# adwardlee/multitask-end-to-end-video-captioning

Measured on AMD Instinct MI355X. Metric: sampled caption tokens/sec (REINFORCE step), higher is better.
Workload: dtype f32

## Files before the change

include/s2vt.h:

```cpp
#ifndef S2VT_H
#define S2VT_H

#include <stddef.h>
#include <stdint.h>

#ifdef __cplusplus
extern "C" {
#endif

#define S2VT_OK 0
#define S2VT_E_BADARG (-1)
#define S2VT_E_ALIGN (-2)
#define S2VT_E_WORKSPACE (-3)
#define S2VT_E_HIP (-4)
#define S2VT_E_CHAIN_TIMEOUT (-5)

typedef void* s2vt_stream;

typedef struct s2vt_dims {
    int32_t dim_image;
    int32_t n_words;
    int32_t word_dim;
    int32_t lstm_dim;
    int32_t n_video_lstm_step;
// ... 138 lines not shown
size_t s2vt_train_workspace_bytes(const s2vt_dims* d, int32_t B, int32_t N);
int s2vt_teacher_forced_fwd(const s2vt_dims* d, const s2vt_params* p, const float* video, int32_t B, int32_t N,
                            const int32_t* caption, float keep, uint64_t seed, const int32_t* video_id,
                            const int32_t* sample_id, float* logits_out, void* workspace, size_t workspace_bytes,
                            s2vt_stream stream);

size_t s2vt_scheduled_scratch_bytes(const s2vt_dims* d, int32_t N);
int s2vt_scheduled_fwd(const s2vt_dims* d, const s2vt_params* p, const float* video, int32_t B, int32_t N, const int32_t* caption, float p_gt,
                       uint64_t coin_seed, float loss_weight, float keep, uint64_t seed, const int32_t* video_id, const int32_t* sample_id,
                       float* logits_out, int32_t* generated, int32_t* fed, float* mask, float* coef_tm, int32_t* target_tm, float* mask_sum,
                       float* mask_sum_copy, void* workspace, size_t workspace_bytes, void* scratch, size_t scratch_bytes, s2vt_stream stream);

int s2vt_teacher_forced_fwd_reuse(const s2vt_dims* d, const s2vt_params* p, const float* video, int32_t B, int32_t N,
                                  const int32_t* caption, float keep, uint64_t seed, const int32_t* video_id,
                                  const int32_t* sample_id, float* logits_out, void* workspace, size_t workspace_bytes,
                                  const void* sampler_workspace, size_t sampler_workspace_bytes, int32_t sampler_rows,
                                  s2vt_stream stream);

int s2vt_teacher_forced_fwd_steps(const s2vt_dims* d, const s2vt_params* p, const float* video, int32_t B, int32_t N,
                                  const int32_t* caption, int32_t caption_steps, float keep, uint64_t seed,
                                  const int32_t* video_id, const int32_t* sample_id, float* logits_out, void* workspace,
                                  size_t workspace_bytes, const void* sampler_workspace, size_t sampler_workspace_bytes,
                                  int32_t sampler_rows, s2vt_stream stream);

int s2vt_teacher_forced_fwd_live(const s2vt_dims* d, const s2vt_params* p, const float* video, int32_t B, int32_t N,
                                 const int32_t* caption, int32_t caption_steps, const int32_t* live_rows, int32_t n_live, float keep,
                                 uint64_t seed, const int32_t* video_id, const int32_t* sample_id, float* logits_out,
                                 void* workspace, size_t workspace_bytes, const void* sampler_workspace,
                                 size_t sampler_workspace_bytes, int32_t sampler_rows, s2vt_stream stream);

int s2vt_softmax_nll_fwd_bwd(float* logits, int32_t ld, int32_t R, int32_t V, const int32_t* target, const float* coef,
                             float smoothing, float* nll, float* lp_target, s2vt_stream stream);
int s2vt_softmax_nll_fwd_bwd_rows(float* logits, int32_t ld, int32_t R, int32_t V, const int32_t* target, const float* coef,
                                  const float* smoothing_rows, float* nll, float* lp_target, s2vt_stream stream);

int s2vt_bptt_bwd(const s2vt_dims* d, const s2vt_params* p, const s2vt_params* grads, const float* video, int32_t B,
                  int32_t N, const float* dlogits, float keep, uint64_t seed, const int32_t* video_id,
                  const int32_t* sample_id, void* workspace, size_t workspace_bytes, s2vt_stream stream);

int s2vt_bptt_bwd_phase(const s2vt_dims* d, const s2vt_params* p, const s2vt_params* grads, const float* video, int32_t B,
                        int32_t N, const float* dlogits, float keep, uint64_t seed, const int32_t* video_id,
                        const int32_t* sample_id, void* workspace, size_t workspace_bytes, int32_t phase, s2vt_stream stream);

int s2vt_bptt_bwd_steps(const s2vt_dims* d, const s2vt_params* p, const s2vt_params* grads, const float* video, int32_t B,
                        int32_t N, const float* dlogits, int32_t caption_steps, float keep, uint64_t seed,
                        const int32_t* video_id, const int32_t* sample_id, void* workspace, size_t workspace_bytes, int32_t phase,
                        s2vt_stream stream);

int s2vt_bptt_bwd_live(const s2vt_dims* d, const s2vt_params* p, const s2vt_params* grads, const float* video, int32_t B,
                       int32_t N, const float* dlogits, int32_t caption_steps, const int32_t* live_rows, int32_t n_live, float keep,
                       uint64_t seed, const int32_t* video_id, const int32_t* sample_id, void* workspace, size_t workspace_bytes,
                       int32_t phase, s2vt_stream stream);

size_t s2vt_bf16_grad_workspace_bytes(const s2vt_dims* d, int32_t B, int32_t N);
int s2vt_bptt_bwd_bf16(const s2vt_dims* d, const s2vt_params* p, const s2vt_params* grads, const float* video, int32_t B,
                       int32_t N, const float* dlogits, int32_t caption_steps, const int32_t* live_rows, int32_t n_live, float keep,
                       uint64_t seed, const int32_t* video_id, const int32_t* sample_id, void* workspace, size_t workspace_bytes,
                       int32_t phase, void* bf16_ws, size_t bf16_ws_bytes, s2vt_stream stream);

int s2vt_cast_bf16(const float* src, int32_t ld, const int32_t* rowidx, int32_t R, int32_t C, int32_t transpose, uint16_t* dst, int32_t ldd,
                   int32_t Rp, float* colsum, uint16_t* row_dst, int32_t row_ldd, void* scratch, size_t scratch_bytes, s2vt_stream stream);
int s2vt_gemm_bf16_nt(const uint16_t* A, int32_t lda, const uint16_t* B, int32_t ldb, float* C, int32_t ldc, int32_t M, int32_t N,
                      int32_t Kp, int32_t accumulate, int32_t mfma, s2vt_stream stream);

size_t s2vt_split_grad_workspace_bytes(const s2vt_dims* d, int32_t B, int32_t N);
int s2vt_bptt_bwd_split(const s2vt_dims* d, const s2vt_params* p, const s2vt_params* grads, const float* video, int32_t B,
                        int32_t N, const float* dlogits, int32_t caption_steps, const int32_t* live_rows, int32_t n_live, float keep,
                        uint64_t seed, const int32_t* video_id, const int32_t* sample_id, void* workspace, size_t workspace_bytes,
                        int32_t phase, void* split_ws, size_t split_ws_bytes, s2vt_stream stream);
int s2vt_cast_bf16_split(const float* src, int32_t ld, const int32_t* rowidx, int32_t R, int32_t C, int32_t transpose, uint16_t* dst,
                         uint16_t* dst_lo, int32_t ldd, int32_t Rp, float* colsum, uint16_t* row_dst, uint16_t* row_dst_lo, int32_t row_ldd,
                         void* scratch, size_t scratch_bytes, s2vt_stream stream);
int s2vt_gemm_bf16x3_nt(const uint16_t* Ah, const uint16_t* Al, int32_t lda, const uint16_t* Bh, const uint16_t* Bl, int32_t ldb, float* C,
                        int32_t ldc, int32_t M, int32_t N, int32_t Kp, int32_t accumulate, void* scratch, size_t scratch_bytes, s2vt_stream stream);

int s2vt_gemm_bf16x3_tn(const uint16_t* Ah, const uint16_t* Al, int32_t lda, const uint16_t* Bh, const uint16_t* Bl, int32_t ldb, float* C,
                        int32_t ldc, int32_t M, int32_t N, int32_t K, int32_t accumulate, float* bias, void* scratch, size_t scratch_bytes,
                        s2vt_stream stream);
int s2vt_split_grad_active(int32_t N);
int s2vt_split_grad_dlogits_planes(const s2vt_dims* d, int32_t B, int32_t N, size_t* hi_offset, size_t* lo_offset, int32_t* ld);
int s2vt_softmax_nll_fwd_bwd_split(float* logits, int32_t ld, int32_t R, int32_t V, const int32_t* target, const float* coef, float smoothing,
                                   const float* smoothing_rows, float* nll, float* lp_target, const s2vt_dims* d, int32_t B, int32_t N,
                                   void* split_ws, size_t split_ws_bytes, s2vt_stream stream);

int s2vt_bptt_dvideo(const s2vt_dims* d, const s2vt_params* p, int32_t B, int32_t N, float* d_video, void* workspace,
                      size_t workspace_bytes, s2vt_stream stream);

int s2vt_embed_scatter_add(const float* dE, int32_t ld, const int32_t* idx, int32_t R, int32_t E, float* dWemb,
                           s2vt_stream stream);

int s2vt_caption_mask(const int32_t* ids, int32_t N, int32_t Tc, float* mask, int32_t* target_tm, float* mask_sum, float* mask_sum_copy, s2vt_stream stream);
int s2vt_pg_coef(const float* mask, const float* rewards, const float* baseline, float scale, int32_t N, int32_t Tc, float* coef_tm,
                 s2vt_stream stream);
int s2vt_step_scalars(const float* coef, const float* nll, int64_t R, const float* mask_sum_local, const float* mask_sum_global, float* loss,
                      float* gscale, float* sumsq, s2vt_stream stream);

int s2vt_xe_prep(const float* mask, const int32_t* caption, int32_t N, int32_t Tc, float loss_weight, float n_global, int32_t q1, float* coef_tm,
                 int32_t* target_tm, float* mask_sum, s2vt_stream stream);
int s2vt_mixed_prep(const float* mask, const float* gt_mask, const float* rewards, const float* baseline, const int32_t* sampled,
                    const int32_t* gt_caption, int32_t Ns, int32_t B, int32_t Tc, double lambda_loss, float loss_weight, int32_t q1,
                    float smoothing, float n_global_b, float* coef_tm, float* smooth_tm, int32_t* caption_all, int32_t* target_tm, float* sums, s2vt_stream stream);
int s2vt_mixed_loss(const float* coef, const float* nll, const int32_t* live_rows, int64_t R, int32_t N, int32_t Ns, float* out3, s2vt_stream stream);

int s2vt_grad_finalize(float* g, const float* theta, int64_t n, const float* gscale, float weight_decay, float* sumsq,
                       s2vt_stream stream);
int s2vt_adam_tf(float* theta, const float* g, float* m, float* v, int64_t n, const float* sumsq, float clip_norm,
                 float lr, int64_t step, float beta1, float beta2, float eps, s2vt_stream stream);
int s2vt_adam_tf_guarded(float* theta, const float* g, float* m, float* v, int64_t n, const float* sumsq, float clip_norm,
                         float lr, int64_t step, float beta1, float beta2, float eps, int32_t* applied_step, s2vt_stream stream);

int s2vt_sgd_guarded(float* theta, const float* g, int64_t n, const float* sumsq, float clip_norm, float lr, int64_t step, int32_t* applied_step,
                     s2vt_stream stream);

int s2vt_attention_fwd(const float* hWa, const float* P, const float* Vt, const float* w, float* scores, float* alpha,
                       float* ctx, int32_t Tv, int32_t B, int32_t H, s2vt_stream stream);
int s2vt_attention_bwd(const float* hWa, const float* P, const float* Vt, const float* w, const float* alpha,
                       const float* dctx, float* de_scratch, float* dhWa, float* dP, float* dVt, float* dw, int32_t Tv,
                       int32_t B, int32_t H, s2vt_stream stream);

int s2vt_attention_fwd_rows(const float* hWa, const float* P, const float* Vt, const float* w, float* scores, float* alpha, float* ctx,
                            int32_t* row_video_scratch, int32_t Tv, int32_t n_video, int32_t samples, int32_t H, s2vt_stream stream);
int s2vt_attention_bwd_rows(const float* hWa, const float* P, const float* Vt, const float* w, const float* alpha, const float* dctx,
                            float* de_scratch, float* dhWa, float* dP, float* dVt, float* dw, int32_t Tv, int32_t n_video,
                            int32_t samples, int32_t H, int32_t acc, s2vt_stream stream);

typedef struct s2vt_attn_params {
    float* Wemb;
    float* encode_image_W;
    float* encode_image_b;
    float* embed_att_w;
    float* embed_att_Wa;
    float* embed_att_Ua;
    float* embed_att_ba;
    float* embed_word_W;
    float* embed_word_b;
    float* embed_nn_Wp;
    float* embed_nn_bp;
    float* lstm3_W;
    float* lstm3_b;
} s2vt_attn_params;

size_t s2vt_attn_workspace_bytes(const s2vt_dims* d, int32_t B);
int s2vt_attn_teacher_forced_fwd(const s2vt_dims* d, const s2vt_attn_params* p, const float* video, int32_t B, const int32_t* caption,
                                 int32_t caption_steps, float keep, uint64_t seed, const int32_t* video_id, const int32_t* sample_id,
                                 float* logits, float* alphas_out, void* workspace, size_t workspace_bytes, s2vt_stream stream);
int s2vt_attn_loss_inputs(const int32_t* caption, const float* mask, int32_t B, int32_t Tc, float beta, int32_t* target_tm, float* coef_tm,
                          float* reg_tm, float* mask_sum, s2vt_stream stream);
int s2vt_attn_step_scalars(const float* coef, const float* nll, int64_t R, const float* reg_coef, float reg_m, const float* mask_sum_local,
                           const float* mask_sum_global, float* loss, float* gscale, float* sumsq, const s2vt_dims* d, int32_t B,
                           void* workspace, size_t workspace_bytes, s2vt_stream stream);
int s2vt_attn_bptt_bwd(const s2vt_dims* d, const s2vt_attn_params* p, const s2vt_attn_params* grads, const float* video, int32_t B,
                       const float* dlogits, int32_t caption_steps, const float* reg_coef, float reg_m, float keep, uint64_t seed,
                       const int32_t* video_id, const int32_t* sample_id, void* workspace, size_t workspace_bytes, s2vt_stream stream);
int s2vt_attn_decode_greedy(const s2vt_dims* d, const s2vt_attn_params* p, const float* video, int32_t B, int32_t video_base, int32_t* ids_out,
                            float* alphas_out, void* workspace, size_t workspace_bytes, s2vt_stream stream);

size_t s2vt_attn_sample_workspace_bytes(const s2vt_dims* d, int32_t B, int32_t K, int32_t with_greedy);
int s2vt_attn_sample(const s2vt_dims* d, const s2vt_attn_params* p, const float* video, int32_t B, int32_t K, int32_t with_greedy, uint64_t seed,
                     int32_t video_base, int32_t* ids_out, int32_t* greedy_out, void* workspace, size_t workspace_bytes, s2vt_stream stream);
int s2vt_attn_sample_ex(const s2vt_dims* d, const s2vt_attn_params* p, const float* video, int32_t B, int32_t K, int32_t with_greedy, uint64_t seed,
                        int32_t video_base, int32_t flags, int32_t* ids_out, int32_t* greedy_out, void* workspace, size_t workspace_bytes,
                        s2vt_stream stream);
size_t s2vt_attn_rows_workspace_bytes(const s2vt_dims* d, int32_t n_video, int32_t samples);
int s2vt_attn_teacher_forced_fwd_rows(const s2vt_dims* d, const s2vt_attn_params* p, const float* video, int32_t n_video, int32_t samples,
                                      const int32_t* caption, int32_t caption_steps, float keep, uint64_t seed, const int32_t* video_id,
                                      const int32_t* sample_id, float* logits, float* alphas_out, void* workspace, size_t workspace_bytes,
// ... 141 lines not shown
```

multitask-end-to-end-video-captioning_amd/_lib.py:

```python
from __future__ import annotations

import ctypes as C
import os

_HERE = os.path.dirname(os.path.abspath(__file__))
_LIB = None


class S2VTLibraryError(RuntimeError):
    pass


class S2VTChainTimeout(S2VTLibraryError):
    """A persistent recurrence (csrc/chain.hip) was starved of CUs and gave up a grid-wide wait (S2VT_E_CHAIN_TIMEOUT):
    activations computed since are suspect, variable updates queued behind it were skipped on the device.  Recover with
    Video_Caption_Generator.recover() (synchronise, acknowledge, fall back to per-step launches) and repeat the step."""


MODEL_RESIDUAL = 1


class Dims(C.Structure):
    _fields_ = [(n, C.c_int32) for n in ("dim_image", "n_words", "word_dim", "lstm_dim", "n_video_lstm_step",
                                         "n_caption_lstm_step", "label_dim", "reserved")]
# ... 30 lines not shown

class Operand(C.Structure):
    _fields_ = [("ptr", C.c_void_p), ("rowidx", C.c_void_p), ("ld", C.c_int32), ("k", C.c_int32), ("rowmod", C.c_int32),
                ("reserved", C.c_int32)]


class LstmDir(C.Structure):
    _fields_ = [("W", C.c_void_p), ("kw0", C.c_int32), ("b", C.c_void_p), ("cinit", C.c_void_p), ("cinit_tstride", C.c_int64),
                ("ldcinit", C.c_int32), ("cinit_t0", C.c_int32), ("cinit_steps", C.c_int32), ("C_hist", C.c_void_p),
                ("H_hist", C.c_void_p), ("gates", C.c_void_p)]


BIDIR_PARAM_FIELDS = ("Wemb", "encode_image_W", "encode_image_b", "lstm1_fw_W", "lstm1_fw_b", "lstm1_bw_W", "lstm1_bw_b", "lstm2_W", "lstm2_b",
                      "embed_word_W", "embed_word_b")


class BidirParams(C.Structure):
    _fields_ = [(n, C.c_void_p) for n in BIDIR_PARAM_FIELDS]


def lib_path() -> str:
    return os.environ.get("S2VT_LIB") or os.path.join(_HERE, "libs2vt_hip.so")


_vp, _i32, _i64, _u32, _u64, _f32, _sz = C.c_void_p, C.c_int32, C.c_int64, C.c_uint32, C.c_uint64, C.c_float, C.c_size_t
_DP, _PP, _OP = C.POINTER(Dims), C.POINTER(Params), C.POINTER(Operand)
_AP = C.POINTER(AttnParams)
_LD = C.POINTER(LstmDir)
_BP = C.POINTER(BidirParams)

SIGNATURES = {
    "s2vt_version": (C.c_int, []),
    "s2vt_build_flags": (C.c_int, []),
    "s2vt_last_hip_error": (C.c_int, []),
    "s2vt_zero_regions": (C.c_int, [C.POINTER(C.c_void_p), C.POINTER(C.c_size_t), _i32, _vp]),
    "s2vt_error_string": (C.c_char_p, [C.c_int]),
    "s2vt_prof_enable": (C.c_int, [C.c_int]),
    "s2vt_prof_filter": (C.c_int, [C.c_int, C.c_int]),
    "s2vt_prof_collect": (C.c_int, [C.POINTER(ProfRow), C.c_int]),
    "s2vt_math_eval": (C.c_int, [C.c_int, _vp, _vp, _i64, _vp]),
    "s2vt_gumbel_eval": (C.c_int, [_u64, _i32, _i32, _i32, _vp, _i32, _vp]),
    "s2vt_gemm": (C.c_int, [_OP, _i32, _vp, _i32, _vp, _vp, _i32, _vp, _i32, _i32, _i32, _i32, _i32, _vp]),
    "s2vt_gemm_nt": (C.c_int, [_OP, _i32, _vp, _i32, _vp, _vp, _i32, _vp, _i32, _i32, _i32, _i32, _i32, _vp]),
    "s2vt_lstm_cell_fwd": (C.c_int, [_OP, _OP, _vp, _vp, _i32, _vp, _vp, _vp, _vp, _vp, _vp, _i32, _i32, _f32, _u64, _vp,
                                     _vp, _u32, _i32, _vp]),
    "s2vt_lstm_cell_fwd_res": (C.c_int, [_OP, _OP, _vp, _vp, _i32, _vp, _vp, _OP, _vp, _vp, _vp, _vp, _i32, _i32, _f32, _u64, _vp,
                                         _vp, _u32, _i32, _vp]),
    "s2vt_vocab_pick": (C.c_int, [_vp, _i32, _vp, _vp, _i32, _i32, _i32, _vp, _vp, _i32, _u64, _vp, _vp, _vp, _i32, _vp]),
    "s2vt_tile_count": (C.c_int, [C.c_int]),
    "s2vt_tile_info": (C.c_int, [C.c_int, C.c_int, C.POINTER(TileDesc)]),
    "s2vt_gemm_live": (C.c_int, [_OP, _i32, _vp, _i32, _vp, _vp, _i32, _vp, _i32, _i32, _i32, _i32, _vp, _vp, _i32, _vp]),
    "s2vt_lstm_cell_fwd_live": (C.c_int, [_OP, _OP, _vp, _vp, _i32, _vp, _vp, _OP, _vp, _vp, _vp, _vp, _i32, _i32, _f32, _u64, _vp,
                                          _vp, _u32, _vp, _vp, _i32, _vp]),
    "s2vt_lstm_cell_fwd_gather": (C.c_int, [_OP, _OP, _vp, _vp, _vp, _vp, _i32, _vp, _vp, _vp, _vp, _vp, _vp, _i32, _i32, _i32, _vp]),
    "s2vt_vocab_pick_live": (C.c_int, [_vp, _i32, _vp, _vp, _i32, _i32, _i32, _vp, _vp, _i32, _u64, _vp, _i32, _vp, _vp, _vp, _i32, _vp]),
    "s2vt_frame_embed_fwd": (C.c_int, [_DP, _PP, _vp, _i32, _vp, _vp]),
    "s2vt_sample_workspace_bytes": (_sz, [_DP, _i32, _i32, _i32]),
    "s2vt_sample": (C.c_int, [_DP, _PP, _vp, _i32, _i32, _i32, _u64, _i32, _vp, _vp, _sz, _vp]),
    "s2vt_sample_ex": (C.c_int, [_DP, _PP, _vp, _i32, _i32, _i32, _u64, _i32, _i32, _vp, _vp, _sz, _vp]),
    "s2vt_sample_screen_workspace_bytes": (_sz, [_DP, _i32, _i32, _i32]),
    "s2vt_sample_screened": (C.c_int, [_DP, _PP, _vp, _i32, _i32, _i32, _u64, _i32, _vp, _vp, _sz, _vp, _sz, _vp]),
    "s2vt_sample_mix_workspace_bytes": (_sz, [_DP, _i32, _i32]),
    "s2vt_sample_mix": (C.c_int, [_DP, _PP, _vp, _i32, _vp, _f32, _i32, _u64, _i32, _vp, _vp, _sz, _vp]),
    "s2vt_vocab_topk": (C.c_int, [_vp, _i32, _i32, _i32, _i32, _vp, _vp, _vp]),
    "s2vt_beam_workspace_bytes": (_sz, [_DP, _i32, _i32]),
    "s2vt_beam_encode": (C.c_int, [_DP, _PP, _vp, _i32, _i32, _vp, _sz, _vp]),
    "s2vt_beam_step": (C.c_int, [_DP, _PP, _i32, _i32, _i32, _i32, _vp, _vp, _vp, _i32, _vp, _vp, _vp, _vp, _sz, _vp]),
    "s2vt_train_workspace_bytes": (_sz, [_DP, _i32, _i32]),
    "s2vt_teacher_forced_fwd": (C.c_int, [_DP, _PP, _vp, _i32, _i32, _vp, _f32, _u64, _vp, _vp, _vp, _vp, _sz, _vp]),
    "s2vt_teacher_forced_fwd_reuse": (C.c_int, [_DP, _PP, _vp, _i32, _i32, _vp, _f32, _u64, _vp, _vp, _vp, _vp, _sz, _vp, _sz, _i32, _vp]),
    "s2vt_gemm_nt_splitk": (C.c_int, [_vp, _i32, _vp, _i32, _vp, _i32, _i32, _i32, _i32, _i32, _i32, _vp, _sz, _vp]),
    "s2vt_teacher_forced_fwd_steps": (C.c_int, [_DP, _PP, _vp, _i32, _i32, _vp, _i32, _f32, _u64, _vp, _vp, _vp, _vp, _sz, _vp, _sz, _i32, _vp]),
    "s2vt_teacher_forced_fwd_live": (C.c_int, [_DP, _PP, _vp, _i32, _i32, _vp, _i32, _vp, _i32, _f32, _u64, _vp, _vp, _vp, _vp, _sz, _vp, _sz, _i32, _vp]),
    "s2vt_bptt_bwd_live": (C.c_int, [_DP, _PP, _PP, _vp, _i32, _i32, _vp, _i32, _vp, _i32, _f32, _u64, _vp, _vp, _vp, _sz, _i32, _vp]),
    "s2vt_bf16_grad_workspace_bytes": (_sz, [_DP, _i32, _i32]),
    "s2vt_bptt_bwd_bf16": (C.c_int, [_DP, _PP, _PP, _vp, _i32, _i32, _vp, _i32, _vp, _i32, _f32, _u64, _vp, _vp, _vp, _sz, _i32, _vp, _sz, _vp]),
    "s2vt_cast_bf16": (C.c_int, [_vp, _i32, _vp, _i32, _i32, _i32, _vp, _i32, _i32, _vp, _vp, _i32, _vp, _sz, _vp]),
    "s2vt_gemm_bf16_nt": (C.c_int, [_vp, _i32, _vp, _i32, _vp, _i32, _i32, _i32, _i32, _i32, _i32, _vp]),
    "s2vt_split_grad_workspace_bytes": (_sz, [_DP, _i32, _i32]),
    "s2vt_bptt_bwd_split": (C.c_int, [_DP, _PP, _PP, _vp, _i32, _i32, _vp, _i32, _vp, _i32, _f32, _u64, _vp, _vp, _vp, _sz, _i32, _vp, _sz, _vp]),
    "s2vt_cast_bf16_split": (C.c_int, [_vp, _i32, _vp, _i32, _i32, _i32, _vp, _vp, _i32, _i32, _vp, _vp, _vp, _i32, _vp, _sz, _vp]),
    "s2vt_gemm_bf16x3_nt": (C.c_int, [_vp, _vp, _i32, _vp, _vp, _i32, _vp, _i32, _i32, _i32, _i32, _i32, _vp, _sz, _vp]),
    "s2vt_gemm_bf16x3_tn": (C.c_int, [_vp, _vp, _i32, _vp, _vp, _i32, _vp, _i32, _i32, _i32, _i32, _i32, _vp, _vp, _sz, _vp]),
    "s2vt_split_grad_active": (C.c_int, [_i32]),
    "s2vt_train_workspace_dz2": (C.c_int, [_DP, _i32, _i32, C.POINTER(_sz), C.POINTER(_sz)]),
    "s2vt_split_grad_dlogits_planes": (C.c_int, [_DP, _i32, _i32, C.POINTER(_sz), C.POINTER(_sz), C.POINTER(_i32)]),
    "s2vt_softmax_nll_fwd_bwd_split": (C.c_int, [_vp, _i32, _i32, _i32, _vp, _vp, _f32, _vp, _vp, _vp, _DP, _i32, _i32, _vp, _sz, _vp]),
    "s2vt_bptt_bwd_steps": (C.c_int, [_DP, _PP, _PP, _vp, _i32, _i32, _vp, _i32, _f32, _u64, _vp, _vp, _vp, _sz, _i32, _vp]),
    "s2vt_softmax_nll_fwd_bwd": (C.c_int, [_vp, _i32, _i32, _i32, _vp, _vp, _f32, _vp, _vp, _vp]),
    "s2vt_softmax_unshifted_argmax": (C.c_int, [_vp, _i32, _i32, _i32, _vp, _vp, _vp]),
    "s2vt_softmax_nll_fwd_bwd_rows": (C.c_int, [_vp, _i32, _i32, _i32, _vp, _vp, _vp, _vp, _vp, _vp]),
    "s2vt_bptt_bwd": (C.c_int, [_DP, _PP, _PP, _vp, _i32, _i32, _vp, _f32, _u64, _vp, _vp, _vp, _sz, _vp]),
    "s2vt_bptt_bwd_phase": (C.c_int, [_DP, _PP, _PP, _vp, _i32, _i32, _vp, _f32, _u64, _vp, _vp, _vp, _sz, _i32, _vp]),
    "s2vt_bptt_dvideo": (C.c_int, [_DP, _PP, _i32, _i32, _vp, _vp, _sz, _vp]),
    "s2vt_embed_scatter_add": (C.c_int, [_vp, _i32, _vp, _i32, _i32, _vp, _vp]),
    "s2vt_caption_mask": (C.c_int, [_vp, _i32, _i32, _vp, _vp, _vp, _vp, _vp]),
    "s2vt_pg_coef": (C.c_int, [_vp, _vp, _vp, _f32, _i32, _i32, _vp, _vp]),
    "s2vt_xe_prep": (C.c_int, [_vp, _vp, _i32, _i32, _f32, _f32, _i32, _vp, _vp, _vp, _vp]),
    "s2vt_mixed_prep": (C.c_int, [_vp, _vp, _vp, _vp, _vp, _vp, _i32, _i32, _i32, C.c_double, _f32, _i32, _f32, _f32, _vp, _vp, _vp, _vp, _vp, _vp]),
    "s2vt_mixed_loss": (C.c_int, [_vp, _vp, _vp, _i64, _i32, _i32, _vp, _vp]),
    "s2vt_step_scalars": (C.c_int, [_vp, _vp, _i64, _vp, _vp, _vp, _vp, _vp, _vp]),
    "s2vt_grad_finalize": (C.c_int, [_vp, _vp, _i64, _vp, _f32, _vp, _vp]),
    "s2vt_adam_tf": (C.c_int, [_vp, _vp, _vp, _vp, _i64, _vp, _f32, _f32, _i64, _f32, _f32, _f32, _vp]),
    "s2vt_attention_fwd": (C.c_int, [_vp, _vp, _vp, _vp, _vp, _vp, _vp, _i32, _i32, _i32, _vp]),
    "s2vt_attention_bwd": (C.c_int, [_vp, _vp, _vp, _vp, _vp, _vp, _vp, _vp, _vp, _vp, _vp, _i32, _i32, _i32, _vp]),
    "s2vt_attention_fwd_rows": (C.c_int, [_vp, _vp, _vp, _vp, _vp, _vp, _vp, _vp, _i32, _i32, _i32, _i32, _vp]),
    "s2vt_attention_bwd_rows": (C.c_int, [_vp, _vp, _vp, _vp, _vp, _vp, _vp, _vp, _vp, _vp, _vp, _i32, _i32, _i32, _i32, _i32, _vp]),
    "s2vt_attn_sample_workspace_bytes": (_sz, [_DP, _i32, _i32, _i32]),
    "s2vt_attn_sample": (C.c_int, [_DP, _AP, _vp, _i32, _i32, _i32, _u64, _i32, _vp, _vp, _vp, _sz, _vp]),
    "s2vt_attn_sample_ex": (C.c_int, [_DP, _AP, _vp, _i32, _i32, _i32, _u64, _i32, _i32, _vp, _vp, _vp, _sz, _vp]),
    "s2vt_attn_rows_workspace_bytes": (_sz, [_DP, _i32, _i32]),
    "s2vt_attn_teacher_forced_fwd_rows": (C.c_int, [_DP, _AP, _vp, _i32, _i32, _vp, _i32, _f32, _u64, _vp, _vp, _vp, _vp, _vp, _sz, _vp]),
    "s2vt_attn_step_scalars_rows": (C.c_int, [_vp, _vp, _i64, _vp, _f32, _vp, _vp, _vp, _vp, _vp, _DP, _i32, _i32, _vp, _sz, _vp]),
    "s2vt_attn_bptt_bwd_rows": (C.c_int, [_DP, _AP, _AP, _vp, _i32, _i32, _vp, _i32, _vp, _f32, _f32, _u64, _vp, _vp, _vp, _sz, _vp]),
    "s2vt_attn_workspace_bytes": (_sz, [_DP, _i32]),
    "s2vt_attn_teacher_forced_fwd": (C.c_int, [_DP, _AP, _vp, _i32, _vp, _i32, _f32, _u64, _vp, _vp, _vp, _vp, _vp, _sz, _vp]),
    "s2vt_attn_loss_inputs": (C.c_int, [_vp, _vp, _i32, _i32, _f32, _vp, _vp, _vp, _vp, _vp]),
    "s2vt_attn_step_scalars": (C.c_int, [_vp, _vp, _i64, _vp, _f32, _vp, _vp, _vp, _vp, _vp, _DP, _i32, _vp, _sz, _vp]),
    "s2vt_attn_bptt_bwd": (C.c_int, [_DP, _AP, _AP, _vp, _i32, _vp, _i32, _vp, _f32, _f32, _u64, _vp, _vp, _vp, _sz, _vp]),
    "s2vt_attn_decode_greedy": (C.c_int, [_DP, _AP, _vp, _i32, _i32, _vp, _vp, _vp, _sz, _vp]),
    "s2vt_attn_beam_workspace_bytes": (_sz, [_DP, _i32, _i32]),
    "s2vt_attn_beam_encode": (C.c_int, [_DP, _AP, _vp, _i32, _i32, _vp, _sz, _vp]),
    "s2vt_attn_beam_step": (C.c_int, [_DP, _AP, _i32, _i32, _i32, _i32, _vp, _vp, _vp, _i32, _vp, _vp, _vp, _vp, _vp, _sz, _vp]),
    "s2vt_attr_head_fwd": (C.c_int, [_vp, _i32, _i32, _i32, _vp, _vp, _i32, _vp, _vp, _vp, _vp, _vp]),
    "s2vt_attr_head_bwd": (C.c_int, [_vp, _vp, _vp, _i32, _i32, _i32, _f32, _vp, _vp, _vp, _vp]),
    "s2vt_attr_head_scores": (C.c_int, [_vp, _i32, _i32, _i32, _vp, _vp, _i32, _vp, _vp, _vp, _vp]),
    "s2vt_create": (C.c_int, [_DP, _i32, _i32, C.POINTER(_vp)]),
    "s2vt_destroy": (C.c_int, [_vp]),
    "s2vt_encode_fwd": (C.c_int, [_vp, _PP, _vp, _i32, _vp]),
    "s2vt_decode_greedy": (C.c_int, [_vp, _PP, _vp, _vp]),
    "s2vt_decode_multinomial": (C.c_int, [_vp, _PP, _i32, _u64, _i32, _vp, _vp]),
    "s2vt_pack_weights": (C.c_int, [_vp, _i32, _i32, _vp, _vp, _vp]),
    "s2vt_unpack_weights": (C.c_int, [_vp, _vp, _i32, _i32, _vp, _vp]),
    "s2vt_frame_embed_bwd": (C.c_int, [_DP, _vp, _vp, _i32, _vp, _vp, _vp]),
    "s2vt_lstm_cell_bwd": (C.c_int, [_vp, _vp, _vp, _vp, _vp, _vp, _vp, _i32, _i32, _vp]),
    "s2vt_xent_smooth_fwd_bwd": (C.c_int, [_vp, _i32, _i32, _i32, _vp, _vp, _f32, _vp, _vp]),
    "s2vt_pg_nll_fwd_bwd": (C.c_int, [_vp, _i32, _i32, _i32, _i32, _vp, _vp, _vp, _vp, _vp, _vp, _vp]),
    "s2vt_embed_gather": (C.c_int, [_vp, _i32, _vp, _i32, _i32, _vp, _i32, _vp]),
    "s2vt_global_norm_clip": (C.c_int, [_vp, _i64, _f32, _vp, _vp]),
    "s2vt_gemm_tn": (C.c_int, [_vp, _i32, _vp, _vp, _i32, _vp, _i32, _i32, _i32, _i32, _i32, _vp]),
    "s2vt_transpose": (C.c_int, [_vp, _i32, _vp, _i32, _i32, _i32, _vp]),
    "s2vt_colsum": (C.c_int, [_vp, _i32, _i32, _i32, _vp, _vp]),
    "s2vt_tanh_bwd": (C.c_int, [_vp, _vp, _vp, _i64, _vp]),
    "s2vt_dropout_bwd": (C.c_int, [_vp, _i32, _vp, _i32, _i32, _f32, _u64, _u32, _vp, _vp, _vp]),
    "s2vt_lstm_recurrence_scratch_bytes": (_sz, [_i32]),
    "s2vt_lstm_recurrence_fwd": (C.c_int, [_vp, _i32, _vp, _vp, _i64, _i32, _i32, _vp, _vp, _vp, _vp, _i32, _i32, _i32, _f32, _u64, _vp, _vp,
                                           _u32, _i32, _vp, _sz, _vp]),
    "s2vt_lstm_birecurrence_scratch_bytes": (_sz, [_i32]),
    "s2vt_lstm_birecurrence_fwd": (C.c_int, [_LD, _LD, _i32, _i32, _i32, _i32, _vp, _sz, _vp]),
    "s2vt_bidir_workspace_bytes": (_sz, [_DP, _i32]),
    "s2vt_bidir_teacher_forced_fwd": (C.c_int, [_DP, _BP, _vp, _i32, _vp, _f32, _u64, _vp, _vp, _i32, _vp, _vp, _sz, _vp]),
    "s2vt_bidir_bptt_bwd": (C.c_int, [_DP, _BP, _BP, _vp, _i32, _vp, _f32, _u64, _vp, _vp, _vp, _sz, _vp]),
    "s2vt_bidir_decode_workspace_bytes": (_sz, [_DP, _i32]),
    "s2vt_bidir_decode_greedy": (C.c_int, [_DP, _BP, _vp, _i32, _i32, _i32, _i32, _vp, _vp, _vp, _sz, _vp]),
    "s2vt_bidir_sample_workspace_bytes": (_sz, [_DP, _i32, _i32, _i32]),
    "s2vt_bidir_sample": (C.c_int, [_DP, _BP, _vp, _i32, _i32, _i32, _u64, _i32, _i32, _vp, _vp, _vp, _sz, _vp]),
    "s2vt_bidir_beam_workspace_bytes": (_sz, [_DP, _i32, _i32]),
    "s2vt_bidir_beam_encode": (C.c_int, [_DP, _BP, _vp, _i32, _i32, _i32, _vp, _sz, _vp]),
    "s2vt_bidir_beam_step": (C.c_int, [_DP, _BP, _i32, _i32, _i32, _i32, _vp, _vp, _vp, _i32, _vp, _vp, _vp, _vp, _sz, _vp]),
    "s2vt_bidir_sample_sum": (C.c_int, [_vp, _vp, _i32, _i32, _i32, _i32, _vp]),
    "s2vt_bidir_rows_workspace_bytes": (_sz, [_DP, _i32, _i32]),
    "s2vt_bidir_teacher_forced_fwd_rows": (C.c_int, [_DP, _BP, _vp, _i32, _i32, _vp, _f32, _u64, _vp, _vp, _i32, _vp, _vp, _sz, _vp]),
    "s2vt_bidir_bptt_bwd_rows": (C.c_int, [_DP, _BP, _BP, _vp, _i32, _i32, _vp, _f32, _u64, _vp, _vp, _vp, _sz, _vp]),
    "s2vt_lstm_recurrence_bwd_scratch_bytes": (_sz, [_i32, _i32]),
    "s2vt_lstm_recurrence_bwd": (C.c_int, [_vp, _i32, _vp, _vp, _vp, _i64, _i32, _i32, _vp, _i32, _i32, _i32, _f32, _u64, _vp, _vp, _u32, _i32,
                                           _vp, _sz, _vp]),
    "s2vt_lstm_recurrence_bwd_split": (C.c_int, [_vp, _i32, _vp, _vp, _vp, _i64, _i32, _i32, _vp, _i32, _i32, _i32, _f32, _u64, _vp, _vp, _u32,
# ... 47 lines not shown
```

multitask-end-to-end-video-captioning_amd/csrc/bwd_bf16.hip:

```cpp
#include <hip/hip_runtime.h>

#include <cstdlib>
#include <type_traits>

#include "internal.h"

namespace s2vt {
namespace {

typedef __bf16 bf16x8 __attribute__((ext_vector_type(8)));
typedef float f32x4 __attribute__((ext_vector_type(4)));
typedef float f32x16 __attribute__((ext_vector_type(16)));

template <bool SPLIT>
__global__ __launch_bounds__(256) void cast_rows_bf16_kernel(const float* __restrict__ src, int ld, const int32_t* __restrict__ rowidx,
                                                             int R, int K, uint16_t* __restrict__ dst, int ldd, int vec,
                                                             uint16_t* __restrict__ dst_lo, int ones)
{
    const int cpr = bf16_pad(K + ones) / 8;
    const long total = (long)R * cpr;
    for (long i = (long)blockIdx.x * 256 + threadIdx.x; i < total; i += (long)gridDim.x * 256) {
        const int r = (int)(i / cpr), k0 = (int)(i % cpr) * 8;
        const float* s = src + (size_t)(rowidx ? rowidx[r] : r) * ld + k0;
        float v[8];
        if (vec && k0 + 8 <= K) {
            const float4 a = *reinterpret_cast<const float4*>(s), b = *reinterpret_cast<const float4*>(s + 4);
            v[0] = a.x; v[1] = a.y; v[2] = a.z; v[3] = a.w; v[4] = b.x; v[5] = b.y; v[6] = b.z; v[7] = b.w;
        } else {
#pragma unroll
            for (int j = 0; j < 8; ++j) v[j] = k0 + j < K ? s[j] : ones && k0 + j == K ? 1.0f : 0.0f;
        }
        uint4 o;
        if constexpr (SPLIT) {
            uint4 l;
            split2(v[0], v[1], o.x, l.x); split2(v[2], v[3], o.y, l.y); split2(v[4], v[5], o.z, l.z); split2(v[6], v[7], o.w, l.w);
            *reinterpret_cast<uint4*>(dst_lo + (size_t)r * ldd + k0) = l;
        } else {
            o.x = pack2(v[0], v[1]); o.y = pack2(v[2], v[3]); o.z = pack2(v[4], v[5]); o.w = pack2(v[6], v[7]);
        }
        *reinterpret_cast<uint4*>(dst + (size_t)r * ldd + k0) = o;
    }
}

constexpr int kTrRows = 256;

template <bool SPLIT>
__global__ __launch_bounds__(256) void cast_tr_bf16_kernel(CastTrArgs a, int vec)
{
    __shared__ float t[64][65];
    __shared__ float cs[4][64];
    const int tid = threadIdx.x, c0 = blockIdx.x * 64;
    const int rbeg = blockIdx.y * kTrRows, rend = min(rbeg + kTrRows, a.Rp);
    float csum = 0.0f;
    for (int r0 = rbeg; r0 < rend; r0 += 64) {
#pragma unroll
        for (int p = 0; p < 4; ++p) {
            const int rr = p * 16 + (tid >> 4), cc = (tid & 15) * 4;
            const int r = r0 + rr, c = c0 + cc;
            float v[4] = {0.0f, 0.0f, 0.0f, 0.0f};
            if (r < a.R) {
                const float* s = a.src + (size_t)(a.rowidx ? a.rowidx[r] : r) * a.ld + c;
                if (vec && c + 4 <= a.C) {
                    const float4 x = *reinterpret_cast<const float4*>(s);
                    v[0] = x.x; v[1] = x.y; v[2] = x.z; v[3] = x.w;
                } else {
#pragma unroll
                    for (int j = 0; j < 4; ++j) v[j] = c + j < a.C ? s[j] : 0.0f;
                }
                if (a.rdst) {
                    uint2 o;
                    if constexpr (SPLIT) {
                        uint2 l;
                        split2(v[0], v[1], o.x, l.x); split2(v[2], v[3], o.y, l.y);
                        *reinterpret_cast<uint2*>(a.rdst_lo + (size_t)r * a.rldd + c) = l;
                    } else {
                        o.x = pack2(v[0], v[1]); o.y = pack2(v[2], v[3]);
                    }
                    *reinterpret_cast<uint2*>(a.rdst + (size_t)r * a.rldd + c) = o;
                }
            }
#pragma unroll
            for (int j = 0; j < 4; ++j) t[rr][cc + j] = v[j];
        }
        __syncthreads();
        for (int i = tid >> 6; i < 64; i += 4) csum += t[i][tid & 63];
#pragma unroll
        for (int p = 0; p < 2; ++p) {
            const int cc = p * 32 + (tid >> 3), rr = (tid & 7) * 8;
            if (c0 + cc < a.C) {
                uint4 o;
                if constexpr (SPLIT) {
                    uint4 l;
                    split2(t[rr][cc], t[rr + 1][cc], o.x, l.x); split2(t[rr + 2][cc], t[rr + 3][cc], o.y, l.y);
                    split2(t[rr + 4][cc], t[rr + 5][cc], o.z, l.z); split2(t[rr + 6][cc], t[rr + 7][cc], o.w, l.w);
                    *reinterpret_cast<uint4*>(a.dst_lo + (size_t)(c0 + cc) * a.ldd + r0 + rr) = l;
                } else {
                    o.x = pack2(t[rr][cc], t[rr + 1][cc]); o.y = pack2(t[rr + 2][cc], t[rr + 3][cc]);
                    o.z = pack2(t[rr + 4][cc], t[rr + 5][cc]); o.w = pack2(t[rr + 6][cc], t[rr + 7][cc]);
                }
                *reinterpret_cast<uint4*>(a.dst + (size_t)(c0 + cc) * a.ldd + r0 + rr) = o;
            }
        }
// ... 57 lines not shown
    constexpr int RM = MF == 16 ? 4 : 2;
    typedef typename std::conditional<MF == 16, f32x4, f32x16>::type acc_t;
    constexpr int NACC = MF == 16 ? 4 : 16;
    acc_t acc[RM][RM];
#pragma unroll
    for (int i = 0; i < RM; ++i)
#pragma unroll
        for (int j = 0; j < RM; ++j)
#pragma unroll
            for (int e = 0; e < NACC; ++e) acc[i][j][e] = 0.0f;

    const int nk = g.Kp / kBK;
    if (nk > 0) { load(0); store(0); }
    __syncthreads();
    for (int kt = 0; kt < nk; ++kt) {
        const int cur = kt & 1;
        if (kt + 1 < nk) load((kt + 1) * kBK);
        const uint16_t* As = lds[cur][0];
        const uint16_t* Bs = lds[cur][1];
        if constexpr (MF == 16) {
#pragma unroll
            for (int kk = 0; kk < 2; ++kk) {
                const int ch = kk * 4 + (lane >> 4);
                bf16x8 af[4], bfr[4];
#pragma unroll
                for (int i = 0; i < 4; ++i) {
                    const int ra_ = wr * 64 + i * 16 + (lane & 15), rb_ = wc * 64 + i * 16 + (lane & 15);
                    af[i] = *reinterpret_cast<const bf16x8*>(As + swz(ra_, ch));
                    bfr[i] = *reinterpret_cast<const bf16x8*>(Bs + swz(rb_, ch));
                }
#pragma unroll
                for (int i = 0; i < 4; ++i)
#pragma unroll
                    for (int j = 0; j < 4; ++j) acc[i][j] = __builtin_amdgcn_mfma_f32_16x16x32_bf16(af[i], bfr[j], acc[i][j], 0, 0, 0);
            }
        } else {
#pragma unroll
            for (int kk = 0; kk < 4; ++kk) {
                const int ch = kk * 2 + (lane >> 5);
                bf16x8 af[2], bfr[2];
#pragma unroll
                for (int i = 0; i < 2; ++i) {
                    const int ra_ = wr * 64 + i * 32 + (lane & 31), rb_ = wc * 64 + i * 32 + (lane & 31);
                    af[i] = *reinterpret_cast<const bf16x8*>(As + swz(ra_, ch));
                    bfr[i] = *reinterpret_cast<const bf16x8*>(Bs + swz(rb_, ch));
                }
#pragma unroll
                for (int i = 0; i < 2; ++i)
#pragma unroll
                    for (int j = 0; j < 2; ++j) acc[i][j] = __builtin_amdgcn_mfma_f32_32x32x16_bf16(af[i], bfr[j], acc[i][j], 0, 0, 0);
            }
        }
        if (kt + 1 < nk) store(cur ^ 1);
        __syncthreads();
    }
#pragma unroll
    for (int i = 0; i < RM; ++i)
#pragma unroll
        for (int j = 0; j < RM; ++j)
#pragma unroll
            for (int e = 0; e < NACC; ++e) {
                int row, col;
                if constexpr (MF == 16) {
                    row = m0 + wr * 64 + i * 16 + (lane >> 4) * 4 + e;
                    col = n0 + wc * 64 + j * 16 + (lane & 15);
                } else {
                    row = m0 + wr * 64 + i * 32 + (e & 3) + 8 * (e >> 2) + 4 * (lane >> 5);
                    col = n0 + wc * 64 + j * 32 + (lane & 31);
                }
                if (row < g.M && col < g.N) {
                    float* c = g.C + (size_t)row * g.ldc + col;
                    *c = g.accumulate ? *c + acc[i][j][e] : acc[i][j][e];
                }
            }
}


struct GemmX3Args {
    const uint16_t *Ah, *Al; int lda; const uint16_t *Bh, *Bl; int ldb; float* C; int ldc;
    int M, N, nk, nk_slab, accumulate, tiles_m, tiles_n;
    float* part;
    int K;
    float* bias; int Mo;
};

constexpr int kX3BK = 32, kX3Slots = 4, kX3Plane = kTile * kX3BK;
constexpr int kX3Lds = kX3Slots * 4 * kX3Plane * 2;
constexpr int kX3Dma = kTile / 16;
typedef __attribute__((address_space(3))) void* x3_lds_ptr;
typedef short i16x4 __attribute__((ext_vector_type(4)));
typedef __attribute__((address_space(3))) i16x4* x3_tr_ptr;

template <bool TN>
__global__ __launch_bounds__(512) void gemm_bf16x3_kernel(GemmX3Args g)
{
    extern __shared__ __attribute__((aligned(16))) uint16_t x3lds[];
    const int nwg = g.tiles_m * g.tiles_n, orig = blockIdx.x;
    const int xcd = orig & 7, q = nwg >> 3, rem = nwg & 7;
    const int wgid = (xcd < rem ? xcd * (q + 1) : rem * (q + 1) + (xcd - rem) * q) + (orig >> 3);
    const int tm = wgid % g.tiles_m, tn = wgid / g.tiles_m;
    const int m0 = tm * kTile, n0 = tn * kTile;
    const int kbeg = blockIdx.y * g.nk_slab, nk = min(g.nk_slab, g.nk - kbeg);
    const int tid = threadIdx.x, lane = tid & 63, w = __builtin_amdgcn_readfirstlane(tid >> 6);

    if (w >= 4) {
        const int p = w - 4;
        const uint16_t* const plane = p == 0 ? g.Ah : p == 1 ? g.Al : p == 2 ? g.Bh : g.Bl;
        const int r0 = p < 2 ? m0 : n0, rows = p < 2 ? g.M : g.N, ld = p < 2 ? g.lda : g.ldb;
        const __amdgpu_buffer_rsrc_t rs = __builtin_amdgcn_make_buffer_rsrc(const_cast<uint16_t*>(plane + (TN ? (size_t)r0 : (size_t)r0 * ld)), 0,
                                                                            TN ? (int)(((uint32_t)g.K * (uint32_t)ld - (uint32_t)r0) * 2u) : (int)kOob, 0x00020000);
        uint32_t voff[kX3Dma];
        if constexpr (TN) {
            const int kr = lane >> 4, s = lane & 15;
#pragma unroll
            for (int b = 0; b < kX3Dma; ++b)
                voff[b] = (uint32_t)((b * 4 + kr) * ld + ((((s >> 1) ^ (kr | ((b & 2) << 1))) << 1) | (s & 1)) * 8) * 2u;
        } else {
            const int rr = lane >> 2, kg = (lane & 3) ^ ((rr >> 2) & 3);
#pragma unroll
            for (int b = 0; b < kX3Dma; ++b) {
                const int r = b * 16 + rr;
                voff[b] = r0 + r < rows ? (uint32_t)(r * ld + kg * 8) * 2u : kOob;
            }
        }
        auto issue = [&](int ks) __attribute__((always_inline)) {
            uint16_t* const dst = x3lds + ((ks % kX3Slots) * 4 + p) * kX3Plane;
            if constexpr (TN) {
                const uint32_t koff = (uint32_t)(kbeg + ks) * kX3BK * (uint32_t)ld * 2u;
#pragma unroll
                for (int b = 0; b < kX3Dma; ++b)
                    __builtin_amdgcn_raw_ptr_buffer_load_lds(rs, (x3_lds_ptr)(dst + b * 4 * kTile), 16, voff[b] + koff, 0, 0, 0);
            } else {
                const uint32_t soff = (uint32_t)(kbeg + ks) * kX3BK * 2u;
#pragma unroll
                for (int b = 0; b < kX3Dma; ++b)
                    __builtin_amdgcn_raw_ptr_buffer_load_lds(rs, (x3_lds_ptr)(dst + b * 16 * kX3BK), 16, voff[b], soff, 0, 0);
            }
        };
        auto wait_younger = [](int n) __attribute__((always_inline)) {
            if (n >= 2) wait_vmcnt<2 * kX3Dma>();
            else if (n == 1) wait_vmcnt<kX3Dma>();
            else wait_vmcnt<0>();
        };
        const int pro = min(kX3Slots, nk);
        for (int ks = 0; ks < pro; ++ks) issue(ks);
        if (pro - 1 >= 3) wait_vmcnt<3 * kX3Dma>();
        else wait_younger(pro - 1);
        asm volatile("" ::: "memory");
        __builtin_amdgcn_s_barrier();
        asm volatile("" ::: "memory");
        for (int k = 0; k < nk; ++k) {
            wait_younger(min(k + 3, nk - 1) - (k + 1));
            asm volatile("" ::: "memory");
            __builtin_amdgcn_s_barrier();
            asm volatile("" ::: "memory");
            if (k + kX3Slots < nk) issue(k + kX3Slots);
        }
        return;
    }

    const int wr = w >> 1, wc = w & 1;
    const int fofs = (lane & 15) * kX3BK + (((lane >> 4) ^ ((lane >> 2) & 3)) << 3);
    const int gq = lane >> 4, tq = (lane >> 2) & 3, tswz = tq | ((gq & 1) << 2);
    const int tofs = (gq * 8 + tq) * kTile + (lane & 3) * 4;
    f32x4 acc[4][4];
#pragma unroll
    for (int i = 0; i < 4; ++i)
#pragma unroll
        for (int j = 0; j < 4; ++j) acc[i][j] = f32x4{0.0f, 0.0f, 0.0f, 0.0f};
    auto read = [&](int ks, bf16x8 (&f)[4][4]) __attribute__((always_inline)) {
        const uint16_t* const s = x3lds + (ks % kX3Slots) * 4 * kX3Plane;
#pragma unroll
        for (int pl = 0; pl < 4; ++pl)
#pragma unroll
            for (int i = 0; i < 4; ++i)
                if constexpr (TN) {
                    const uint16_t* const a = s + pl * kX3Plane + tofs + ((((pl < 2 ? wr : wc) * 4 + i) ^ tswz) << 4);
                    const i16x4 lo4 = __builtin_amdgcn_ds_read_tr16_b64_v4i16((x3_tr_ptr)a);
                    const i16x4 hi4 = __builtin_amdgcn_ds_read_tr16_b64_v4i16((x3_tr_ptr)(a + 4 * kTile));
                    f[pl][i] = __builtin_bit_cast(bf16x8, __builtin_shufflevector(lo4, hi4, 0, 1, 2, 3, 4, 5, 6, 7));
                } else {
                    f[pl][i] = *reinterpret_cast<const bf16x8*>(s + pl * kX3Plane + ((pl < 2 ? wr : wc) * 64 + i * 16) * kX3BK + fofs);
                }
    };
    auto mul = [&](const bf16x8 (&f)[4][4]) __attribute__((always_inline)) {
#pragma unroll
        for (int i = 0; i < 4; ++i)
#pragma unroll
            for (int j = 0; j < 4; ++j) acc[i][j] = __builtin_amdgcn_mfma_f32_16x16x32_bf16(f[0][i], f[3][j], acc[i][j], 0, 0, 0);
#pragma unroll
        for (int i = 0; i < 4; ++i)
#pragma unroll
            for (int j = 0; j < 4; ++j) acc[i][j] = __builtin_amdgcn_mfma_f32_16x16x32_bf16(f[1][i], f[2][j], acc[i][j], 0, 0, 0);
#pragma unroll
        for (int i = 0; i < 4; ++i)
#pragma unroll
            for (int j = 0; j < 4; ++j) acc[i][j] = __builtin_amdgcn_mfma_f32_16x16x32_bf16(f[0][i], f[2][j], acc[i][j], 0, 0, 0);
    };
    bf16x8 fa[4][4], fb[4][4];
    __syncthreads();
    if (nk > 0) read(0, fa);
    auto step = [&](int k, bf16x8 (&cur)[4][4], bf16x8 (&nxt)[4][4]) __attribute__((always_inline)) {
        asm volatile("s_waitcnt lgkmcnt(0)" ::: "memory");
        __syncthreads();
        if (k + 1 < nk) read(k + 1, nxt);
        mul(cur);
    };
    for (int k = 0; k < nk; k += 2) {
        step(k, fa, fb);
        step(k + 1, fb, fa);
    }
    float* const out = g.part ? g.part + (size_t)blockIdx.y * g.Mo * g.N : g.C;
    const int ldo = g.part ? g.N : g.ldc;
    const bool add = !g.part && g.accumulate;
#pragma unroll
    for (int i = 0; i < 4; ++i)
#pragma unroll
        for (int j = 0; j < 4; ++j)
#pragma unroll
            for (int e = 0; e < 4; ++e) {
                const int row = m0 + wr * 64 + i * 16 + (lane >> 4) * 4 + e, col = n0 + wc * 64 + j * 16 + (lane & 15);
                if (row < g.M && col < g.N) {
                    float* c = out + (size_t)row * ldo + col;
                    *c = add ? *c + acc[i][j][e] : acc[i][j][e];
                } else if (TN && row == g.M && g.bias && col < g.N) {
                    if (g.part) out[(size_t)row * ldo + col] = acc[i][j][e];
                    else g.bias[col] += acc[i][j][e];
                }
            }
}

__global__ __launch_bounds__(256) void reduce_slabs_kernel(const float* __restrict__ part, int slabs, int M, int N, float* __restrict__ C, int ldc,
                                                           int accumulate, int Mo, float* __restrict__ bias)
{
    const size_t MN = (size_t)Mo * N;
    for (size_t i = (size_t)blockIdx.x * 256 + threadIdx.x; i < MN; i += (size_t)gridDim.x * 256) {
        float s = part[i];
        for (int k = 1; k < slabs; ++k) s += part[(size_t)k * MN + i];
        const size_t r = i / N;
        if (r < (size_t)M) {
            float* c = C + r * ldc + i % N;
            *c = accumulate ? *c + s : s;
        } else {
            bias[i % N] += s;
        }
    }
}
}

hipError_t launch_cast_rows_bf16(const float* src, int ld, const int32_t* rowidx, int R, int K, uint16_t* dst, int ldd, hipStream_t st,
                                 uint16_t* dst_lo, int ones)
{
    if (R <= 0 || K <= 0) return hipSuccess;
    ones = ones ? 1 : 0;
    const int vec = !((reinterpret_cast<uintptr_t>(src) & 15) || (ld & 3));
    const long chunks = (long)R * (bf16_pad(K + ones) / 8);
    const long blocks = (chunks + 255) / 256;
    const dim3 grid((unsigned)(blocks < 8192 ? blocks : 8192));
    if (dst_lo) hipLaunchKernelGGL(cast_rows_bf16_kernel<true>, grid, dim3(256), 0, st, src, ld, rowidx, R, K, dst, ldd, vec, dst_lo, ones);
    else hipLaunchKernelGGL(cast_rows_bf16_kernel<false>, grid, dim3(256), 0, st, src, ld, rowidx, R, K, dst, ldd, vec, dst_lo, ones);
    return hipGetLastError();
}

size_t cast_tr_part_floats(int Rp, int C)
{
    return (size_t)((Rp + kTrRows - 1) / kTrRows) * (size_t)C;
}

hipError_t launch_cast_tr_bf16(const CastTrArgs& a, hipStream_t st)
{
    if (a.C <= 0 || a.Rp <= 0) return hipSuccess;
    const int vec = !((reinterpret_cast<uintptr_t>(a.src) & 15) || (a.ld & 3));
    const int ny = (a.Rp + kTrRows - 1) / kTrRows;
    if (a.dst_lo) hipLaunchKernelGGL(cast_tr_bf16_kernel<true>, dim3((a.C + 63) / 64, ny), dim3(256), 0, st, a, vec);
    else hipLaunchKernelGGL(cast_tr_bf16_kernel<false>, dim3((a.C + 63) / 64, ny), dim3(256), 0, st, a, vec);
    hipError_t e = hipGetLastError();
    if (e != hipSuccess || !a.colsum) return e;
    hipLaunchKernelGGL(colsum_parts_kernel, dim3((a.C + 255) / 256), dim3(256), 0, st, (const float*)a.part, ny, a.C, a.colsum);
    return hipGetLastError();
}

int gemm_bf16_default_mfma()
{
    static const int v = [] { const char* e = getenv("S2VT_BF16_MFMA"); const int x = e ? atoi(e) : 16; return x == 32 ? 32 : 16; }();
    return v;
}

hipError_t launch_gemm_bf16_nt(const uint16_t* A, int lda, const uint16_t* B, int ldb, float* C, int ldc, int M, int N, int Kp, int accumulate,
                               int mfma, hipStream_t st)
{
    if (M <= 0 || N <= 0) return hipSuccess;
    GemmBf16Args g;
    g.A = A; g.lda = lda; g.B = B; g.ldb = ldb; g.C = C; g.ldc = ldc; g.M = M; g.N = N; g.Kp = Kp; g.accumulate = accumulate;
    g.tiles_m = (M + kTile - 1) / kTile; g.tiles_n = (N + kTile - 1) / kTile;
    const dim3 grid((unsigned)(g.tiles_m * g.tiles_n));
    if ((mfma ? mfma : gemm_bf16_default_mfma()) == 32) hipLaunchKernelGGL(gemm_bf16_nt_kernel<32>, grid, dim3(256), 0, st, g);
    else hipLaunchKernelGGL(gemm_bf16_nt_kernel<16>, grid, dim3(256), 0, st, g);
    return hipGetLastError();
}

int gemm_bf16x3_slabs(int M, int N, int Kp)
{
    const int tiles = ((M + kTile - 1) / kTile) * ((N + kTile - 1) / kTile), nk = Kp / kX3BK;
    static const int cus = [] {
        int dev = 0, n = 256;
        if (hipGetDevice(&dev) == hipSuccess) (void)hipDeviceGetAttribute(&n, hipDeviceAttributeMultiprocessorCount, dev);
        return n > 0 ? n : 256;
    }();
    int s = 1;
    while (s < 8 && tiles * (s * 2) <= cus && nk / (s * 2) >= 16) s *= 2;
    return s;
}

size_t gemm_bf16x3_part_floats(int M, int N, int Kp)
{
    const int s = gemm_bf16x3_slabs(M, N, Kp);
    return s > 1 ? (size_t)s * M * N : 0;
}

namespace {
template <bool TN>
hipError_t launch_x3(const uint16_t* Ah, const uint16_t* Al, int lda, const uint16_t* Bh, const uint16_t* Bl, int ldb, float* C, int ldc, int M, int N,
                     int Kp, int accumulate, float* bias, float* part, size_t part_floats, int cls, hipStream_t st)
{
    if (M <= 0 || N <= 0) return hipSuccess;
    static const hipError_t attr = hipFuncSetAttribute(reinterpret_cast<const void*>(gemm_bf16x3_kernel<TN>), hipFuncAttributeMaxDynamicSharedMemorySize, kX3Lds);
    if (attr != hipSuccess) return attr;
    GemmX3Args g;
    g.Ah = Ah; g.Al = Al; g.lda = lda; g.Bh = Bh; g.Bl = Bl; g.ldb = ldb; g.C = C; g.ldc = ldc; g.M = M; g.N = N;
    g.K = Kp; g.bias = bias; g.Mo = M + (bias ? 1 : 0);
    const int Kr = bf16_pad(Kp);
    g.nk = Kr / kX3BK; g.accumulate = accumulate;
    g.tiles_m = (g.Mo + kTile - 1) / kTile; g.tiles_n = (N + kTile - 1) / kTile;
    int slabs = part ? gemm_bf16x3_slabs(g.Mo, N, Kr) : 1;
    if ((size_t)slabs * g.Mo * N > part_floats) slabs = 1;
    g.nk_slab = ((g.nk + slabs - 1) / slabs + 1) & ~1;
    slabs = g.nk_slab ? (g.nk + g.nk_slab - 1) / g.nk_slab : 1;
    g.part = slabs > 1 ? part : nullptr;
    const dim3 grid((unsigned)(g.tiles_m * g.tiles_n), (unsigned)slabs);
    const bool prof = prof_wants(cls, 16);
    hipEvent_t e0 = nullptr, e1 = nullptr;
    if (prof) {
        hipError_t pe = prof_events(&e0, &e1);
        if (pe != hipSuccess) return pe;
        (void)hipEventRecord(e0, st);
    }
    hipLaunchKernelGGL(gemm_bf16x3_kernel<TN>, grid, dim3(512), kX3Lds, st, g);
    if (slabs > 1) {
        const size_t MN = (size_t)g.Mo * N, blocks = (MN + 255) / 256;
        hipLaunchKernelGGL(reduce_slabs_kernel, dim3((unsigned)(blocks < 4096 ? blocks : 4096)), dim3(256), 0, st, (const float*)part, slabs, M, N, C, ldc,
                           accumulate, g.Mo, bias);
    }
    if (prof) {
        (void)hipEventRecord(e1, st);
        prof_record(cls, 16, cls == 2 ? "x3_128x128(dma) pick screen" : cls == 3 ? "x3_128x128(dma) wgrad" : "x3_128x128(dma) dgrad",
                    2.0 * M * (double)N * Kp, e0, e1);
    }
    return hipGetLastError();
}
}

hipError_t launch_gemm_bf16x3_nt(const uint16_t* Ah, const uint16_t* Al, int lda, const uint16_t* Bh, const uint16_t* Bl, int ldb, float* C, int ldc,
                                 int M, int N, int Kp, int accumulate, float* part, size_t part_floats, int cls, hipStream_t st)
{
    return launch_x3<false>(Ah, Al, lda, Bh, Bl, ldb, C, ldc, M, N, Kp, accumulate, nullptr, part, part_floats, cls, st);
}

bool gemm_bf16x3_tn_ok(int lda, int ldb, int K)
{
    const unsigned long long ld = (unsigned long long)(lda > ldb ? lda : ldb);
    return K >= 0 && lda > 0 && ldb > 0 && ((unsigned long long)bf16_pad(K) + 1) * ld * 2ull + 512ull < (1ull << 31);
}

hipError_t launch_gemm_bf16x3_tn(const uint16_t* Ah, const uint16_t* Al, int lda, const uint16_t* Bh, const uint16_t* Bl, int ldb, float* C, int ldc,
                                 int M, int N, int K, int accumulate, float* bias, float* part, size_t part_floats, int cls, hipStream_t st)
{
    if (!gemm_bf16x3_tn_ok(lda, ldb, K)) return hipErrorInvalidValue;
    return launch_x3<true>(Ah, Al, lda, Bh, Bl, ldb, C, ldc, M, N, K, accumulate, bias, part, part_floats, cls, st);
}

}
```

multitask-end-to-end-video-captioning_amd/csrc/internal.h:

```cpp
#pragma once
#include <hip/hip_runtime.h>
#include <stdint.h>

#include "gemm_mfma.h"

namespace s2vt {

hipError_t launch_gemm(const GemmArgs& a, int epi, int cfg, hipStream_t st);

struct ProfRow { int cls, cfg; long launches; double ms, flops; const char* name; };
void prof_enable(bool on);
bool prof_on();
bool prof_wants(int cls, int cfg);
void prof_filter(int cls, int cfg);
void prof_record(int cls, int cfg, const char* name, double flops, hipEvent_t e0, hipEvent_t e1);
hipError_t prof_events(hipEvent_t* e0, hipEvent_t* e1);
int prof_collect(ProfRow* rows, int max_rows);
int gemm_num_cfgs(int epi);
const char* gemm_cfg_name(int epi, int cfg);
struct GemmCfgInfo { const char* name; int BM, CG, fallback; bool has_scalar, has_live; };
bool gemm_cfg_info(int epi, int cfg, GemmCfgInfo* out);

struct TnArgs {
    const float* A; const int* rowidx; int lda;
// ... 166 lines not shown
    int n_video;
    const int32_t* live;
    const int32_t* n_live;
};
hipError_t launch_attn_fwd(const AttnFwdArgs& a, hipStream_t st);
struct AttnBwdArgs {
    const float* hWa; const float* P; const float* Vt; const float* w; const float* alpha;
    const float* dctx; int ld_dctx;
    const float* slabs; int nslab; size_t slab_stride; int ld_slab;
    int ctx_col0, emb_col0;
    const float* demb_dense; int ld_demb; float* demb_out;
    const float* reg_coef;
    const float* asum; float reg_m;
    float* dhWa;
    float* dP; float* dVt; int acc;
    float* dw;
    int Tv, B, H;
    int vec;
};
hipError_t launch_attn_bwd(const AttnBwdArgs& a, hipStream_t st);
struct AttnBwdRowsArgs {
    AttnBwdArgs a;
    int n_video, samples;
    float* de_rows;
    float* dctx_rows;
};
hipError_t launch_attn_bwd_rows(const AttnBwdRowsArgs& r, hipStream_t st);
hipError_t launch_attn_row_video(int32_t* row_video, int rows, int n_video, hipStream_t st);

hipError_t launch_vocab_topk(const float* logits, int ld, int R, int V, int k, int32_t* ids, float* logp, hipStream_t st);

struct AttnChainLaunch {
    const float* W3; int ldw; const float* b3;
    const float* cinit; size_t cinit_tstride; int ldcinit;
    float* C; float* Hh; float* Out; size_t state_tstride;
    float* gates; size_t gates_tstride;
    const float* Wa; int ldwa; const float* P; const float* Vt; const float* w;
    float* hWa; size_t hwa_tstride;
    float* alpha; float* asum; float* ctx;
    int B, H, T, Tv;
    float keep; uint32_t seed_lo, seed_hi, drop_code0; const int32_t* video_id; const int32_t* sample_id;
    float* img;
    unsigned* sync;
};
constexpr size_t kAttnChainSyncBytes = 3 * kChainSyncBytes;
bool attn_chain_eligible(int B, int H, int Tv);
size_t attn_chain_scratch_floats(int H);
hipError_t launch_attn_chain(const AttnChainLaunch& a, hipStream_t st);

struct AttnBwdChainLaunch {
    const float* W3; int ldw; const float* Wa; int ldwa;
    const float* gates; size_t gates_tstride; const float* C; size_t state_tstride;
    float* dcat; size_t dcat_tstride; int ld_cat;
    float* deh;
    float* dZ; size_t dz_tstride;
    const float* hWa; size_t hwa_tstride; const float* P; const float* Vt; const float* w; const float* alpha;
    const float* reg_coef; const float* asum; float reg_m;
    float* dhWa; size_t dhwa_tstride;
    float* dP; float* dVt; float* dw;
    int B, H, T, Tv;
    float keep; uint32_t seed_lo, seed_hi, drop_code0; const int32_t* video_id; const int32_t* sample_id;
    float* img; float* ex; float* dctxs; unsigned* sync;
};
bool attn_bwd_chain_eligible(int B, int H, int Tv);
void attn_bwd_chain_scratch(int H, size_t* img_floats, size_t* ex_floats, size_t* row_floats, size_t* sync_bytes);
hipError_t launch_attn_bwd_chain(const AttnBwdChainLaunch& a, hipStream_t st);

constexpr int kBf16K = 64;
__host__ __device__ inline int bf16_pad(int k) { return (k + kBf16K - 1) / kBf16K * kBf16K; }
typedef float f32x2 __attribute__((ext_vector_type(2)));
typedef __bf16 bf16x2 __attribute__((ext_vector_type(2)));
__device__ __forceinline__ uint32_t pack2(float a, float b)
{
    const f32x2 v = {a, b};
    return __builtin_bit_cast(uint32_t, __builtin_convertvector(v, bf16x2));
}

__device__ __forceinline__ void split2(float a, float b, uint32_t& hi, uint32_t& lo)
{
    hi = pack2(a, b);
    lo = pack2(a - __uint_as_float(hi << 16), b - __uint_as_float(hi & 0xffff0000u));
}
hipError_t launch_cast_rows_bf16(const float* src, int ld, const int32_t* rowidx, int R, int K, uint16_t* dst, int ldd, hipStream_t st,
                                 uint16_t* dst_lo = nullptr, int ones = 0);
struct CastTrArgs {
    const float* src; int ld; const int32_t* rowidx; int R, C;
    uint16_t* dst; int ldd; int Rp;
    float* colsum; float* part;
    uint16_t* rdst; int rldd;
    uint16_t* dst_lo; uint16_t* rdst_lo;
};
hipError_t launch_cast_tr_bf16(const CastTrArgs& a, hipStream_t st);
size_t cast_tr_part_floats(int Rp, int C);
hipError_t launch_gemm_bf16_nt(const uint16_t* A, int lda, const uint16_t* B, int ldb, float* C, int ldc, int M, int N, int Kp, int accumulate,
                               int mfma, hipStream_t st);
hipError_t launch_gemm_bf16x3_nt(const uint16_t* Ah, const uint16_t* Al, int lda, const uint16_t* Bh, const uint16_t* Bl, int ldb, float* C, int ldc,
                                 int M, int N, int Kp, int accumulate, float* part, size_t part_floats, int cls, hipStream_t st);
size_t gemm_bf16x3_part_floats(int M, int N, int Kp);
bool gemm_bf16x3_tn_ok(int lda, int ldb, int K);
hipError_t launch_gemm_bf16x3_tn(const uint16_t* Ah, const uint16_t* Al, int lda, const uint16_t* Bh, const uint16_t* Bl, int ldb, float* C, int ldc,
                                 int M, int N, int K, int accumulate, float* bias, float* part, size_t part_floats, int cls, hipStream_t st);
bool softmax_nll_split_ok(const float* logits, int ld, int V, const uint16_t* hi, const uint16_t* lo, int ldp);
hipError_t launch_softmax_nll_split(const float* logits, int ld, int R, int V, const int32_t* target, const float* coef, float smoothing, float* nll,
                                    float* lp_t, uint16_t* hi, uint16_t* lo, int ldp, hipStream_t st, const float* smooth_rows = nullptr);

constexpr int kPickScreenMaxH = 2048;
constexpr size_t kPickScreenHeadBytes = 256;
struct PickScreenWs {
    unsigned long long* counters;
    float* nwmax;
    uint16_t *Wh, *Wl;
    float* Wt;
    uint16_t *hh, *hl;
    float* L;
    int Hp, ldl, ldt;
};
hipError_t launch_pick_screen_prepare(const float* W, int H, int V, const PickScreenWs& s, hipStream_t st);
hipError_t launch_pick_screen_step(const float* h, int ldh, const float* W, const float* bias, int R, int H, int V, const int32_t* vid,
                                   const int32_t* sid, uint64_t seed, int step, unsigned long long* pick, int pick_stride, const PickScreenWs& s,
                                   hipStream_t st);

struct NnBwdArgs {
    const float* A; int lda;
    const float* W; int ldw;
    float* C; int ldc;
    int M, N, K;
    int splits; size_t slab_stride;
};
hipError_t launch_gemm_nn_bwd(const NnBwdArgs& a, hipStream_t st);

}
```

multitask-end-to-end-video-captioning_amd/csrc/train.hip:

```cpp
#include <hip/hip_runtime.h>

#include <mutex>

#include <cstdlib>

#include "api_util.h"

using namespace s2vt_api;

namespace s2vt_api {
SideStream& side_stream()
{
    constexpr int kMaxDev = 32;
    static SideStream table[kMaxDev];
    static bool made[kMaxDev] = {};
    static SideStream none;
    static const int mode = [] {
        const char* on = getenv("S2VT_OVERLAP");
        const int m = on ? atoi(on) : 2;
        return (m < 1 || m > 2) ? 0 : m;
    }();
    int dev = -1;
    if (mode == 0 || hipGetDevice(&dev) != hipSuccess || dev < 0 || dev >= kMaxDev) return none;
    std::lock_guard<std::mutex> lk(side_stream_mutex());
// ... 157 lines not shown
    const size_t ke1 = bf16_pad((int)(Tv * B)), K1 = ke1 + bf16_pad((int)(Tc * B));
    auto mx = [](std::initializer_list<size_t> l) { size_t m = 0; for (size_t v : l) m = v > m ? v : m; return m; };
    Bf16Ws w;
    const size_t off0 = c.off;
    w.L = c.take<uint16_t>(mx({Tc * N * Kv, T * N * K4, Tv * B * K4}));
    w.W = c.take<uint16_t>(mx({H * Kv, (H + E) * K4, E * K4}));
    const bool fused = split && split_fused();
    const size_t Hp1 = bf16_pad((int)H + 1), Ep = bf16_pad((int)E);
    w.BT = c.take<uint16_t>(mx({V * Kr, 4 * H * Kt, 4 * H * K1, E * ke1}));
    w.AT = c.take<uint16_t>(mx({H * Kr, H * Kt, E * Kr, E * ke1, H * K1, D * ke1, fused ? T * N * Hp1 : 0, fused ? Tc * N * Ep : 0}));
    w.lo_delta = 0; w.kpart = nullptr; w.kpart_floats = 0;
    if (split) {
        const size_t hi_bytes = c.off - off0;
        c.take<char>(hi_bytes);
        w.lo_delta = hi_bytes / sizeof(uint16_t);
        const int Re = (int)(Tv * N), Rr = (int)(Tc * N), Re1 = (int)(Tv * B);
        if (fused)
            w.kpart_floats = mx({gemm_bf16x3_part_floats((int)H + 1, (int)V, (int)Kr), gemm_bf16x3_part_floats(Rr, (int)H, (int)Kv),
                                 gemm_bf16x3_part_floats((int)H + 1, (int)(4 * H), bf16_pad((int)(T * N))),
                                 gemm_bf16x3_part_floats((int)E, (int)(4 * H), (int)Kr),
                                 gemm_bf16x3_part_floats((int)(T * N), (int)(H + E), (int)K4), gemm_bf16x3_part_floats(Re, (int)(H + E), (int)K4),
                                 gemm_bf16x3_part_floats(Rr, (int)(H + E), (int)K4)});
        else
        w.kpart_floats = mx({gemm_bf16x3_part_floats((int)H, (int)V, (int)Kr), gemm_bf16x3_part_floats(Rr, (int)H, (int)Kv),
                             gemm_bf16x3_part_floats((int)H, (int)(4 * H), (int)Kt), gemm_bf16x3_part_floats((int)E, (int)(4 * H), (int)Kr),
                             gemm_bf16x3_part_floats((int)(T * N), (int)(H + E), (int)K4), gemm_bf16x3_part_floats(Re, (int)(H + E), (int)K4),
                             gemm_bf16x3_part_floats(Rr, (int)(H + E), (int)K4), gemm_bf16x3_part_floats(Re1, (int)E, (int)K4),
                             gemm_bf16x3_part_floats((int)E, (int)(4 * H), (int)ke1), gemm_bf16x3_part_floats((int)H, (int)(4 * H), (int)K1),
                             gemm_bf16x3_part_floats((int)D, (int)E, (int)ke1)});
        w.kpart = c.take<float>(w.kpart_floats);
    }
    w.part = c.take<float>(mx({cast_tr_part_floats((int)Kr, (int)V), cast_tr_part_floats((int)(ke > Kr ? ke : Kr), (int)(4 * H)),
                               cast_tr_part_floats((int)(K1 - ke1 > ke1 ? K1 - ke1 : ke1), (int)(4 * H)), cast_tr_part_floats((int)ke1, (int)E)}));
    if (out) *out = w;
    return c.off;
}

bool params_ok(const s2vt_params* p)
{
    return p && p->Wemb && p->encode_image_W && p->encode_image_b && p->lstm1_W && p->lstm1_b && p->lstm2_W && p->lstm2_b &&
           p->embed_word_W && p->embed_word_b;
}

struct BwdScratch { float* slab; float* dc; float* bimg; float* bex; unsigned* bsync; };
hipError_t lstm_recurrence_bwd(const float* W, int kw0, const float* gates, const float* C, const float* dext, size_t dext_tstride,
                               int ld_ext, int dext_t0, float* dZ, int M, int H, int T, float keep, uint64_t seed, uint32_t drop_code0,
                               const int32_t* video_id, const int32_t* sample_id, const BwdScratch& sc, int persistent, hipStream_t st,
                               const int32_t* perm = nullptr, const int32_t* nlive = nullptr, bool split = false)
{
    const size_t MH = (size_t)M * H;
    const bool can = sc.bimg && sc.bex && sc.bsync && bwd_chain_eligible(M, H) && !(reinterpret_cast<uintptr_t>(W) & 15);
    if (persistent == 1 && !can) return hipErrorInvalidValue;
    if (persistent == 1 || (persistent == -1 && can && bwd_chain_auto(M, H))) {
        BwdChainLaunch a;
        std::memset(&a, 0, sizeof(a));
        a.W = W; a.ldw = 4 * H; a.kw0 = kw0; a.gates = gates; a.gates_tstride = 4 * MH; a.C = C; a.state_tstride = MH;
        a.dext = dext; a.dext_tstride = dext_tstride; a.ld_ext = ld_ext; a.dext_t0 = dext_t0;
        a.dZ = dZ; a.dz_tstride = 4 * MH; a.M = M; a.H = H; a.T = T;
        a.keep = keep; a.seed_lo = (uint32_t)seed; a.seed_hi = (uint32_t)(seed >> 32); a.drop_code0 = drop_code0;
        a.video_id = video_id; a.sample_id = sample_id;
        a.img = sc.bimg; a.ex = sc.bex; a.sync = sc.bsync;
        a.perm = perm; a.nlive = nlive;
        a.split = split && bwd_chain_split_serves(M, H);
        return launch_lstm_bwd_chain(a, st);
    }
    const SlabPlan sp = slab_plan(M, H);
    for (int t = T - 1; t >= 0; --t) {
        hipError_t e = launch_lstm_bwd_pointwise(gates + (size_t)t * 4 * MH, C + (t + 1) * MH, C + t * MH, t == T - 1 ? nullptr : sc.slab, sp.nslab, MH,
                                                 (dext && t >= dext_t0) ? dext + (size_t)(t - dext_t0) * dext_tstride : nullptr, ld_ext,
                                                 t == T - 1 ? nullptr : sc.dc, sc.dc, dZ + (size_t)t * 4 * MH, M, H, keep, seed, drop_code0 + (uint32_t)t,
                                                 video_id, sample_id, st);
        if (e != hipSuccess) return e;
        if (t > 0) {
            e = nn_bwd(dZ + (size_t)t * 4 * MH, 4 * H, W + (size_t)kw0 * 4 * H, 4 * H, sc.slab, H, M, H, 4 * H, sp.splits, MH, st);
            if (e != hipSuccess) return e;
        }
    }
    return hipSuccess;
}


int unroll_front(const s2vt_dims* d, const s2vt_params* p, const float* video, int B, int N, int T, float keep, uint64_t seed,
                 const int32_t* video_id, const int32_t* sample_id, const TrainWs& w, const void* sampler_workspace,
                 size_t sampler_workspace_bytes, int sampler_rows, s2vt_stream stream)
{
    const int H = d->lstm_dim, E = d->word_dim, Tv = d->n_video_lstm_step;
    const size_t NH = (size_t)N * H, BH = (size_t)B * H;
    hipStream_t st = S(stream);
    hipLaunchKernelGGL(enc_index_kernel, dim3((B * Tv + 255) / 256), dim3(256), 0, st, w.encidx, B, Tv);
    HIP_TRY(hipGetLastError());
    {
        ZeroList z;
        if (!sampler_workspace) { z.add(w.C1, BH * 4); z.add(w.H1, BH * 4); }
        z.add(w.C2, NH * 4); z.add(w.H2, NH * 4);
        HIP_TRY(launch_zero_regions(z, st));
    }
    if (!sampler_workspace) {
        int rc = s2vt_frame_embed_fwd(d, p, video, B, w.emb, stream);
        if (rc != S2VT_OK) return rc;
    }

    NoiseIds none{nullptr, nullptr, 0};
    if (sampler_workspace) {
        Carver sc(const_cast<void*>(sampler_workspace), sampler_workspace_bytes);
        SampleWs sw;
        carve_sample(sc, d, B, sampler_rows, &sw);
        if (!sc.ok() || sampler_rows <= 0) return S2VT_E_WORKSPACE;
        CopyList cl;
        if (cl.add(w.C1, sw.c1, (size_t)(T + 1) * BH * 4) && cl.add(w.H1, sw.h1, (size_t)(T + 1) * BH * 4) && cl.add(w.G1, sw.G1, (size_t)T * 4 * BH * 4) &&
            cl.add(w.emb, sw.emb, (size_t)B * Tv * E * 4)) {
            HIP_TRY(launch_copy_regions(cl, st));
        } else {
            HIP_TRY(hipMemcpyAsync(w.emb, sw.emb, (size_t)B * Tv * E * 4, hipMemcpyDeviceToDevice, st));
            HIP_TRY(hipMemcpyAsync(w.C1, sw.c1, (size_t)(T + 1) * BH * 4, hipMemcpyDeviceToDevice, st));
            HIP_TRY(hipMemcpyAsync(w.H1, sw.h1, (size_t)(T + 1) * BH * 4, hipMemcpyDeviceToDevice, st));
            HIP_TRY(hipMemcpyAsync(w.G1, sw.G1, (size_t)T * 4 * BH * 4, hipMemcpyDeviceToDevice, st));
        }
    } else {
        {
            ASeg sx = make_seg(w.emb, E, E, 0);
            HIP_TRY(store_call(&sx, 1, p->lstm1_W, 4 * H, nullptr, w.Xp1, 4 * H, B * Tv, 4 * H, 0, -1, st));
        }
        HIP_TRY(lstm_recurrence(p->lstm1_W, E, p->lstm1_b, w.Xp1, (size_t)4 * H, Tv * 4 * H, Tv, w.C1, w.H1, BH, w.G1, (size_t)4 * BH,
                                nullptr, 0, B, H, T, 1.0f, none, 0, w.chain_abuf, w.chain_sync, st));
    }
    HIP_TRY(launch_expand_dropout(w.H1 + BH, w.O1, T, B, N, H, keep, seed, 256u, video_id, sample_id, st));
    {
        ASeg se = make_seg(w.O1, H, H, 0);
        HIP_TRY(store_call(&se, 1, p->lstm2_W, 4 * H, nullptr, w.G2, 4 * H, Tv * N, 4 * H, 0, -1, st));
    }
    return S2VT_OK;
}

__device__ __forceinline__ int32_t clamp_word(int32_t c, int V) { return c < 0 ? 0 : c >= V ? V - 1 : c; }

__global__ __launch_bounds__(256) void sched_open_kernel(const int32_t* caption, int N, int Tc, int V, int32_t* prev, int32_t* tgt, int32_t* fed,
                                                         int32_t* argmax_sid)
{
    const int i = blockIdx.x * 256 + threadIdx.x;
    if (i >= N * Tc) return;
    const int t = i / N, n = i - t * N;
    tgt[i] = clamp_word(caption[(size_t)n * Tc + t], V);
    if (t == 0) { prev[n] = 1; fed[(size_t)n * Tc] = 1; argmax_sid[n] = -1; }
}

__global__ __launch_bounds__(256) void sched_step_kernel(const unsigned long long* picked, int stride, const int32_t* caption, int N, int Tc, int t,
                                                         int V, const int32_t* video_id, const int32_t* sample_id, uint32_t seed_lo,
                                                         uint32_t seed_hi, float p_gt, float loss_weight, float* running, int32_t* generated,
                                                         int32_t* fed, float* mask, float* coef_tm, int32_t* target_tm, int32_t* prev)
{
    const int n = blockIdx.x * 256 + threadIdx.x;
    if (n >= N) return;
    const unsigned long long w = picked[(size_t)n * stride];
    const int32_t g = w ? (int32_t)(~(uint32_t)w) : 0;
    const float m = (t == 0 ? 1.0f : running[n]) * (g != 0 ? 1.0f : 0.0f);
    running[n] = m;
    const int32_t truth = clamp_word(caption[(size_t)n * Tc + t], V);
    generated[(size_t)n * Tc + t] = g;
    mask[(size_t)n * Tc + t] = m;
    coef_tm[(size_t)t * N + n] = loss_weight * m;
    target_tm[(size_t)t * N + n] = truth;
    if (t + 1 < Tc) {
        const int32_t word = mix_feeds_truth(seed_lo, seed_hi, (uint32_t)video_id[n], (uint32_t)sample_id[n], (uint32_t)(t + 1), p_gt) ? truth : g;
        fed[(size_t)n * Tc + t + 1] = word;
        prev[(size_t)(t + 1) * N + n] = word;
    }
}

__global__ __launch_bounds__(256) void sched_mask_sum_kernel(const float* mask, int n, float* mask_sum, float* mask_sum_copy)
{
    __shared__ float sh[4];
    float local = 0.f;
    for (int i = threadIdx.x; i < n; i += 256) local += mask[i];
    for (int off = 32; off > 0; off >>= 1) local += __shfl_down(local, off, 64);
    if ((threadIdx.x & 63) == 0) sh[threadIdx.x >> 6] = local;
    __syncthreads();
    if (threadIdx.x == 0) {
        const float total = (sh[0] + sh[1]) + (sh[2] + sh[3]);
        if (mask_sum) *mask_sum = total;
        if (mask_sum_copy) *mask_sum_copy = total;
    }
}

struct SchedScratch { unsigned long long* packed; float* running; int32_t* argmax_sid; };
size_t carve_sched(Carver& c, const s2vt_dims* d, int N, SchedScratch* out)
{
    SchedScratch s;
    s.packed = c.take<unsigned long long>((size_t)d->n_caption_lstm_step * N * kPickStride);
    s.running = c.take<float>(N);
    s.argmax_sid = c.take<int32_t>(N);
    if (out) *out = s;
    return c.off;
}

#define HIP_CHECK(expr) do { const hipError_t _e = (expr); if (_e != hipSuccess) return _e; } while (0)

struct SchedDecode {
    const s2vt_params* p; const TrainWs& w; const SchedScratch& x;
    int N, H, E, V, Tv, Tc; float keep; NoiseIds ids; hipStream_t st;
    const int32_t* caption; float p_gt, loss_weight; uint64_t coin_seed;
    float* logits; int32_t *generated, *fed; float *mask, *coef_tm; int32_t* target_tm;
    size_t NH;

    unsigned long long* picks(int t) const { return x.packed + (size_t)t * N * kPickStride; }

    hipError_t open()
    {
        ZeroList z;
        z.add(x.packed, (size_t)Tc * N * kPickStride * 8);
        HIP_CHECK(launch_zero_regions(z, st));
// ... 57 lines not shown
    if (reinterpret_cast<uintptr_t>(scratch) & 255u) return S2VT_E_ALIGN;
    if (chain_fault()) return S2VT_E_CHAIN_TIMEOUT;
    Carver c(scratch, scratch_bytes);
    size_t imgf, exf, syncb;
    bwd_scratch_max(H, M, &imgf, &exf, &syncb);
    BwdScratch sc;
    sc.slab = c.take<float>((size_t)kMaxSlabs * M * H); sc.dc = c.take<float>((size_t)M * H);
    sc.bimg = c.take<float>(imgf); sc.bex = c.take<float>(exf); sc.bsync = c.take<unsigned>(syncb / 4);
    if (!c.ok()) return S2VT_E_WORKSPACE;
    if (persistent == 1 && !bwd_chain_eligible(M, H)) return S2VT_E_BADARG;
    if (split && (persistent != 1 || !bwd_chain_split_serves(M, H) || (reinterpret_cast<uintptr_t>(W) & 15))) return S2VT_E_BADARG;
    HIP_TRY(lstm_recurrence_bwd(W, kw0, gates, C_hist, dext, (size_t)dext_tstride, ld_ext, dext_t0, dZ, M, H, T, keep, seed, drop_code0, video_id,
                                sample_id, sc, persistent, S(stream), nullptr, nullptr, split));
    return S2VT_OK;
}

int s2vt_lstm_recurrence_bwd(const float* W, int32_t kw0, const float* gates, const float* C_hist, const float* dext, int64_t dext_tstride,
                             int32_t ld_ext, int32_t dext_t0, float* dZ, int32_t M, int32_t H, int32_t T, float keep, uint64_t seed,
                             const int32_t* video_id, const int32_t* sample_id, uint32_t drop_code0, int32_t persistent, void* scratch,
                             size_t scratch_bytes, s2vt_stream stream)
{
    return recurrence_bwd_entry(W, kw0, gates, C_hist, dext, dext_tstride, ld_ext, dext_t0, dZ, M, H, T, keep, seed, video_id, sample_id, drop_code0,
                                persistent, scratch, scratch_bytes, stream, false);
}

int s2vt_lstm_recurrence_bwd_split(const float* W, int32_t kw0, const float* gates, const float* C_hist, const float* dext, int64_t dext_tstride,
                                   int32_t ld_ext, int32_t dext_t0, float* dZ, int32_t M, int32_t H, int32_t T, float keep, uint64_t seed,
                                   const int32_t* video_id, const int32_t* sample_id, uint32_t drop_code0, int32_t persistent, void* scratch,
                                   size_t scratch_bytes, s2vt_stream stream)
{
    return recurrence_bwd_entry(W, kw0, gates, C_hist, dext, dext_tstride, ld_ext, dext_t0, dZ, M, H, T, keep, seed, video_id, sample_id, drop_code0,
                                persistent, scratch, scratch_bytes, stream, true);
}

size_t s2vt_train_workspace_bytes(const s2vt_dims* d, int32_t B, int32_t N)
{
    if (!dims_ok_res(d) || B <= 0 || N <= 0 || N % B) return 0;
    Carver c(nullptr, 0);
    return carve_train(c, d, B, N, nullptr);
}

int s2vt_train_workspace_dz2(const s2vt_dims* d, int32_t B, int32_t N, size_t* offset, size_t* floats)
{
    if (!dims_ok_res(d) || B <= 0 || N <= 0 || N % B || !offset || !floats) return S2VT_E_BADARG;
    alignas(256) static char origin[256];
    Carver c(origin, 0);
    TrainWs w;
    carve_train(c, d, B, N, &w);
    *offset = (size_t)(reinterpret_cast<const char*>(w.dZ2) - origin);
    *floats = (size_t)(d->n_video_lstm_step + d->n_caption_lstm_step) * N * 4 * d->lstm_dim;
    return S2VT_OK;
}

int s2vt_teacher_forced_fwd(const s2vt_dims* d, const s2vt_params* p, const float* video, int32_t B, int32_t N,
                            const int32_t* caption, float keep, uint64_t seed, const int32_t* video_id,
                            const int32_t* sample_id, float* logits, void* workspace, size_t workspace_bytes,
                            s2vt_stream stream)
{
    return s2vt_teacher_forced_fwd_reuse(d, p, video, B, N, caption, keep, seed, video_id, sample_id, logits, workspace,
                                         workspace_bytes, nullptr, 0, 0, stream);
}

int s2vt_teacher_forced_fwd_reuse(const s2vt_dims* d, const s2vt_params* p, const float* video, int32_t B, int32_t N,
                                  const int32_t* caption, float keep, uint64_t seed, const int32_t* video_id,
                                  const int32_t* sample_id, float* logits, void* workspace, size_t workspace_bytes,
                                  const void* sampler_workspace, size_t sampler_workspace_bytes, int32_t sampler_rows,
                                  s2vt_stream stream)
{
    return s2vt_teacher_forced_fwd_steps(d, p, video, B, N, caption, d ? d->n_caption_lstm_step : 0, keep, seed, video_id, sample_id,
                                         logits, workspace, workspace_bytes, sampler_workspace, sampler_workspace_bytes, sampler_rows,
                                         stream);
}

int s2vt_teacher_forced_fwd_steps(const s2vt_dims* d, const s2vt_params* p, const float* video, int32_t B, int32_t N,
                                  const int32_t* caption, int32_t caption_steps, float keep, uint64_t seed,
                                  const int32_t* video_id, const int32_t* sample_id, float* logits, void* workspace,
                                  size_t workspace_bytes, const void* sampler_workspace, size_t sampler_workspace_bytes,
                                  int32_t sampler_rows, s2vt_stream stream)
{
    return s2vt_teacher_forced_fwd_live(d, p, video, B, N, caption, caption_steps, nullptr, 0, keep, seed, video_id, sample_id, logits,
                                        workspace, workspace_bytes, sampler_workspace, sampler_workspace_bytes, sampler_rows, stream);
}

int s2vt_teacher_forced_fwd_live(const s2vt_dims* d, const s2vt_params* p, const float* video, int32_t B, int32_t N,
                                 const int32_t* caption, int32_t caption_steps, const int32_t* live_rows, int32_t n_live, float keep,
                                 uint64_t seed, const int32_t* video_id, const int32_t* sample_id, float* logits, void* workspace,
                                 size_t workspace_bytes, const void* sampler_workspace, size_t sampler_workspace_bytes,
                                 int32_t sampler_rows, s2vt_stream stream)
{
    if ((live_rows == nullptr) != (n_live == 0) || n_live < 0) return S2VT_E_BADARG;
    if (!dims_ok_res(d) || !params_ok(p) || !video || !caption || !logits || !workspace || B <= 0 || N <= 0 || N % B)
        return S2VT_E_BADARG;
    if (!(keep > 0.0f) || (keep < 1.0f && (!video_id || !sample_id))) return S2VT_E_BADARG;
    if (reinterpret_cast<uintptr_t>(workspace) & 255u) return S2VT_E_ALIGN;
    if (chain_fault()) return S2VT_E_CHAIN_TIMEOUT;
    if (caption_steps < 1 || caption_steps > d->n_caption_lstm_step) return S2VT_E_BADARG;
    if (live_rows && (n_live > caption_steps * N || ((d->lstm_dim | d->word_dim) & 3))) return S2VT_E_BADARG;
    const int H = d->lstm_dim, E = d->word_dim, V = d->n_words, Tv = d->n_video_lstm_step, Tc = caption_steps;
    const int T = Tv + Tc;
    Carver c(workspace, workspace_bytes);
    TrainWs w;
    carve_train(c, d, B, N, &w);
    if (!c.ok()) return S2VT_E_WORKSPACE;
    hipStream_t st = S(stream);

    HIP_TRY(launch_prep_caption(caption, w.prev, w.tgt, N, d->n_caption_lstm_step, st));
    {
        const int rc = unroll_front(d, p, video, B, N, T, keep, seed, video_id, sample_id, w, sampler_workspace, sampler_workspace_bytes,
                                    sampler_rows, stream);
        if (rc != S2VT_OK) return rc;
    }
    const size_t NH = (size_t)N * H;
    NoiseIds ids{video_id, sample_id, seed};
    {
        if (!live_rows) {
            ASeg sd[2] = {make_seg(w.O1 + (size_t)Tv * NH, H, H, 0), make_seg(p->Wemb, E, E, H, 0, w.prev)};
            HIP_TRY(store_call(sd, 2, p->lstm2_W, 4 * H, nullptr, w.G2 + (size_t)Tv * 4 * NH, 4 * H, Tc * N, 4 * H, 0, -1, st));
        } else {
            HIP_TRY(launch_gather_i32(w.prev, live_rows, n_live, w.prevp, st));
            ASeg sd[2] = {make_seg(w.O1 + (size_t)Tv * NH, H, H, 0, 0, live_rows), make_seg(p->Wemb, E, E, H, 0, w.prevp)};
            HIP_TRY(store_call(sd, 2, p->lstm2_W, 4 * H, nullptr, w.dZ2p, 4 * H, n_live, 4 * H, 0, -1, st));
            float* const dec = w.G2 + (size_t)Tv * 4 * NH;
            ZeroList z;
            z.add(dec, (size_t)Tc * N * 4 * H * 4);
            if (live_rows && Tc <= 128 && chain_live_capable(N, H)) z.add(w.C2 + (size_t)(Tv + 1) * NH, (size_t)Tc * NH * 4);
            HIP_TRY(launch_zero_regions(z, st));
            HIP_TRY(launch_scatter_rows(w.dZ2p, 4 * H, live_rows, n_live, 4 * H, dec, 4 * H, st));
        }
    }
    const bool rec_live = live_rows && Tc <= 128 && chain_live_capable(N, H);
    if (live_rows && Tc <= 128 && N <= 1024) HIP_TRY(launch_row_order(live_rows, n_live, N, Tv, Tc, w.perm, w.nlive, st));
    HIP_TRY(lstm_recurrence(p->lstm2_W, H + E, p->lstm2_b, w.G2, (size_t)4 * NH, 4 * H, T, w.C2, w.H2, NH, w.G2, (size_t)4 * NH,
                            w.O2, NH, N, H, T, keep, ids, 512u, w.chain_abuf, w.chain_sync, st, rec_live ? w.perm : nullptr,
                            rec_live ? w.nlive : nullptr));
    if (is_residual(d)) HIP_TRY(launch_add_inplace(w.O2 + (size_t)Tv * NH, w.O1 + (size_t)Tv * NH, (size_t)Tc * NH, st));
    ASeg so = make_seg(w.O2 + (size_t)Tv * NH, H, H, 0, 0, live_rows);
    HIP_TRY(store_call(&so, 1, p->embed_word_W, V, p->embed_word_b, logits, V, live_rows ? n_live : Tc * N, V, 0, -1, st));
    return S2VT_OK;
}

size_t s2vt_scheduled_scratch_bytes(const s2vt_dims* d, int32_t N)
{
    if (!dims_ok(d) || N <= 0) return 0;
    Carver c(nullptr, 0);
    return carve_sched(c, d, N, nullptr);
}

int s2vt_scheduled_fwd(const s2vt_dims* d, const s2vt_params* p, const float* video, int32_t B, int32_t N, const int32_t* caption, float p_gt,
                       uint64_t coin_seed, float loss_weight, float keep, uint64_t seed, const int32_t* video_id, const int32_t* sample_id,
                       float* logits_out, int32_t* generated, int32_t* fed, float* mask, float* coef_tm, int32_t* target_tm, float* mask_sum,
                       float* mask_sum_copy, void* workspace, size_t workspace_bytes, void* scratch, size_t scratch_bytes, s2vt_stream stream)
{
    if (!dims_ok(d) || !params_ok(p) || !video || !caption || !video_id || !sample_id || !logits_out || !generated || !fed || !mask || !coef_tm ||
        !target_tm || !workspace || !scratch || B <= 0 || N <= 0 || N % B)
        return S2VT_E_BADARG;
    if (!(p_gt >= 0.0f && p_gt <= 1.0f) || !(keep > 0.0f)) return S2VT_E_BADARG;
    if ((reinterpret_cast<uintptr_t>(workspace) | reinterpret_cast<uintptr_t>(scratch)) & 255u) return S2VT_E_ALIGN;
    if (chain_fault()) return S2VT_E_CHAIN_TIMEOUT;
    const int H = d->lstm_dim, E = d->word_dim, V = d->n_words, Tv = d->n_video_lstm_step, Tc = d->n_caption_lstm_step;
    Carver c(workspace, workspace_bytes);
    TrainWs w;
    carve_train(c, d, B, N, &w);
    Carver cs(scratch, scratch_bytes);
    SchedScratch x;
    carve_sched(cs, d, N, &x);
    if (!c.ok() || !cs.ok()) return S2VT_E_WORKSPACE;
    hipStream_t st = S(stream);
    SchedDecode s{p, w, x, N, H, E, V, Tv, Tc, keep, NoiseIds{video_id, sample_id, seed}, st, caption, p_gt, loss_weight, coin_seed,
                  logits_out, generated, fed, mask, coef_tm, target_tm, (size_t)N * H};
    HIP_TRY(s.open());
    {
        const int rc = unroll_front(d, p, video, B, N, Tv + Tc, keep, seed, video_id, sample_id, w, nullptr, 0, 0, stream);
        if (rc != S2VT_OK) return rc;
    }
    HIP_TRY(s.decode_partials());
    HIP_TRY(s.encode());
    for (int t = 0; t < Tc; ++t) HIP_TRY(s.step(t));
    HIP_TRY(s.close(mask_sum, mask_sum_copy));
    return S2VT_OK;
}

int s2vt_caption_mask(const int32_t* ids, int32_t N, int32_t Tc, float* mask, int32_t* target_tm, float* mask_sum, float* mask_sum_copy, s2vt_stream stream)
{
    if (!ids || N <= 0 || Tc <= 0) return S2VT_E_BADARG;
    HIP_TRY(launch_caption_mask(ids, N, Tc, mask, target_tm, mask_sum, mask_sum_copy, S(stream)));
    return S2VT_OK;
}

int s2vt_pg_coef(const float* mask, const float* rewards, const float* baseline, float scale, int32_t N, int32_t Tc, float* coef_tm,
                 s2vt_stream stream)
{
    if (!mask || !coef_tm || N <= 0 || Tc <= 0) return S2VT_E_BADARG;
    HIP_TRY(launch_pg_coef(mask, rewards, baseline, scale, N, Tc, coef_tm, S(stream)));
    return S2VT_OK;
}

int s2vt_xe_prep(const float* mask, const int32_t* caption, int32_t N, int32_t Tc, float loss_weight, float n_global, int32_t q1, float* coef_tm,
                 int32_t* target_tm, float* mask_sum, s2vt_stream stream)
{
    if (!mask || !coef_tm || (target_tm && !caption) || N <= 0 || Tc <= 0 || Tc > 128 || !(n_global > 0.0f)) return S2VT_E_BADARG;
    HIP_TRY(launch_xe_prep(mask, caption, N, Tc, loss_weight, n_global, q1, coef_tm, target_tm, mask_sum, S(stream)));
    return S2VT_OK;
}

int s2vt_mixed_prep(const float* mask, const float* gt_mask, const float* rewards, const float* baseline, const int32_t* sampled,
                    const int32_t* gt_caption, int32_t Ns, int32_t B, int32_t Tc, double lambda_loss, float loss_weight, int32_t q1,
                    float smoothing, float n_global_b, float* coef_tm, float* smooth_tm, int32_t* caption_all, int32_t* target_tm, float* sums, s2vt_stream stream)
{
    if (!mask || !gt_mask || !rewards || !baseline || !sampled || !gt_caption || !coef_tm || !smooth_tm || !caption_all || !target_tm || !sums) return S2VT_E_BADARG;
    if (Ns <= 0 || B <= 0 || Tc <= 0 || Tc > 128 || !(n_global_b > 0.0f)) return S2VT_E_BADARG;
    HIP_TRY(launch_mixed_prep(mask, gt_mask, rewards, baseline, sampled, gt_caption, Ns, B, Tc, (float)(1.0 - lambda_loss), (float)lambda_loss,
                              loss_weight, q1, smoothing, n_global_b, coef_tm, smooth_tm, caption_all, target_tm, sums, S(stream)));
    return S2VT_OK;
}

int s2vt_mixed_loss(const float* coef, const float* nll, const int32_t* live_rows, int64_t R, int32_t N, int32_t Ns, float* out3, s2vt_stream stream)
{
    if (!coef || !nll || !out3 || R < 0 || R > 0x7fffffff || N <= 0 || Ns < 0 || Ns > N) return S2VT_E_BADARG;
    HIP_TRY(launch_mixed_loss(coef, nll, live_rows, (int)R, N, Ns, out3, S(stream)));
    return S2VT_OK;
}

int s2vt_gemm_nt_splitk(const float* A, int32_t lda, const float* Wt, int32_t ldw, float* C, int32_t ldc, int32_t M, int32_t N,
                        int32_t K, int32_t splits, int32_t tile_cfg, float* slabs, size_t slab_floats, s2vt_stream stream)
{
    if (!A || !Wt || !C || M < 0 || N <= 0 || K <= 0 || lda < K || ldw < K || ldc < N || splits < 0 || splits > 64) return S2VT_E_BADARG;
    if (M == 0) return S2VT_OK;
    hipStream_t st = S(stream);
    int s = splits == 0 ? dx_splits(M, N, K) : splits;
    if (s > 1 && (ldc != N || !slabs)) { if (splits) return S2VT_E_BADARG; s = 1; }
    if (s <= 1) { HIP_TRY(nn_bwd(A, lda, Wt, ldw, C, ldc, M, N, K, 1, 0, st, tile_cfg)); return S2VT_OK; }
    const size_t stride = (size_t)M * N;
    const int kper = ((K + s - 1) / s + BK - 1) / BK * BK, nslab = (K + kper - 1) / kper;
    if ((size_t)nslab * stride > slab_floats) return S2VT_E_WORKSPACE;
    HIP_TRY(nn_bwd(A, lda, Wt, ldw, slabs, N, M, N, K, s, stride, st, tile_cfg >= 0 ? tile_cfg : kSlabTileCfg));
    HIP_TRY(launch_sum_slabs(C, slabs, nslab, stride, stride, st));
    return S2VT_OK;
}

int s2vt_step_scalars(const float* coef, const float* nll, int64_t R, const float* mask_sum_local, const float* mask_sum_global, float* loss,
                      float* gscale, float* sumsq, s2vt_stream stream)
{
    if (R < 0 || ((coef == nullptr) != (nll == nullptr))) return S2VT_E_BADARG;
    HIP_TRY(launch_step_scalars(coef, nll, R, mask_sum_local, mask_sum_global, loss, gscale, sumsq, S(stream)));
    return S2VT_OK;
}

int s2vt_softmax_nll_fwd_bwd(float* logits, int32_t ld, int32_t R, int32_t V, const int32_t* target, const float* coef,
                             float smoothing, float* nll, float* lp_target, s2vt_stream stream)
{
    if (!logits || !target || !coef || R < 0 || V <= 0 || ld < V) return S2VT_E_BADARG;
    HIP_TRY(launch_softmax_nll(logits, ld, R, V, target, coef, smoothing, nll, lp_target, S(stream)));
    return S2VT_OK;
}

int s2vt_softmax_unshifted_argmax(const float* logits, int32_t ld, int32_t R, int32_t V, int32_t* ids, float* probs,
                                  s2vt_stream stream)
{
    if (!logits || !ids || R < 0 || V <= 0 || ld < V) return S2VT_E_BADARG;
    HIP_TRY(launch_softmax_unshifted_argmax(logits, ld, R, V, ids, probs, S(stream)));
    return S2VT_OK;
}

int s2vt_softmax_nll_fwd_bwd_rows(float* logits, int32_t ld, int32_t R, int32_t V, const int32_t* target, const float* coef,
                                  const float* smoothing_rows, float* nll, float* lp_target, s2vt_stream stream)
{
    if (!logits || !target || !coef || !smoothing_rows || R < 0 || V <= 0 || ld < V) return S2VT_E_BADARG;
    HIP_TRY(launch_softmax_nll(logits, ld, R, V, target, coef, 0.0f, nll, lp_target, S(stream), smoothing_rows));
    return S2VT_OK;
}

int s2vt_bptt_bwd(const s2vt_dims* d, const s2vt_params* p, const s2vt_params* grads, const float* video, int32_t B,
                  int32_t N, const float* dlogits, float keep, uint64_t seed, const int32_t* video_id,
                  const int32_t* sample_id, void* workspace, size_t workspace_bytes, s2vt_stream stream)
{
    return s2vt_bptt_bwd_phase(d, p, grads, video, B, N, dlogits, keep, seed, video_id, sample_id, workspace, workspace_bytes, 0,
                               stream);
}

int s2vt_bptt_bwd_phase(const s2vt_dims* d, const s2vt_params* p, const s2vt_params* grads, const float* video, int32_t B,
                        int32_t N, const float* dlogits, float keep, uint64_t seed, const int32_t* video_id,
                        const int32_t* sample_id, void* workspace, size_t workspace_bytes, int32_t phase, s2vt_stream stream)
{
    return s2vt_bptt_bwd_steps(d, p, grads, video, B, N, dlogits, d ? d->n_caption_lstm_step : 0, keep, seed, video_id, sample_id,
                               workspace, workspace_bytes, phase, stream);
}

int s2vt_bptt_bwd_steps(const s2vt_dims* d, const s2vt_params* p, const s2vt_params* grads, const float* video, int32_t B,
                        int32_t N, const float* dlogits, int32_t caption_steps, float keep, uint64_t seed,
                        const int32_t* video_id, const int32_t* sample_id, void* workspace, size_t workspace_bytes, int32_t phase,
                        s2vt_stream stream)
{
    return s2vt_bptt_bwd_live(d, p, grads, video, B, N, dlogits, caption_steps, nullptr, 0, keep, seed, video_id, sample_id, workspace,
                              workspace_bytes, phase, stream);
}

enum GradMode { kGradFp32 = 0, kGradBf16 = 1, kGradSplit = 2 };

static int split_grad_mode(int N)
{
    static const int on = [] { const char* e = getenv("S2VT_SPLIT_GRADS"); return e ? atoi(e) : 1; }();
    return on && N > 256 ? kGradSplit : kGradFp32;
}
static bool split_recurrence()
{
    static const bool on = [] { const char* e = getenv("S2VT_BCHAIN_SPLIT"); return !(e && e[0] == '0'); }();
    return on;
}

enum BwdPhase { kAll = 0, kVocab = 1, kLstm2AndRest = 2, kLstm2 = 3, kRest = 4 };

static TnArgs tn(const float* A, const int32_t* idx, int gather_rows, int lda, const float* B, int ldb, float* C, int ldc, int rows, int M, int N,
                 float* colsum = nullptr)
{
    return TnArgs{A, idx, lda, B, ldb, C, ldc, rows, M, N, 1, colsum, gather_rows};
}

struct BpttBwd {
    SideStream& ss;
    int H, E, V, D, Tv, Tc, T, B, N;
    int K4, Re, Rd;
    size_t NH; TrainWs w; Bf16Ws bw;
    const s2vt_params *p, *grads; const float *video, *dlogits; const int32_t* live_rows; int n_live;
    float keep; uint64_t seed; const int32_t *video_id, *sample_id;
    bool bf16, split, fused;
    hipStream_t st, sd, sv;
    bool gate1, gate2;

    const float* dzd() const { return live_rows ? w.dZ2p : w.dZ2 + (size_t)Tv * 4 * NH; }

    uint16_t* lo(uint16_t* hi) const { return split && hi ? hi + bw.lo_delta : nullptr; }
    hipError_t tr(const float* src, int ld, const int32_t* idx, int R, int C, uint16_t* dst, int ldd, float* colsum = nullptr,
                  uint16_t* rdst = nullptr, int rldd = 0) const
    {
        CastTrArgs a{src, ld, idx, R, C, dst, ldd, bf16_pad(R), colsum, bw.part, rdst, rldd, lo(dst), lo(rdst)};
        return launch_cast_tr_bf16(a, st);
    }
    hipError_t rows(const float* src, int ld, const int32_t* idx, int R, int K, uint16_t* dst, int ldd) const
    {
        return launch_cast_rows_bf16(src, ld, idx, R, K, dst, ldd, st, lo(dst));
    }
    hipError_t mm(uint16_t* A, int lda, uint16_t* Bm, int ldb, float* Cm, int ldc, int M, int Nn, int Kp, int acc) const
    {
        if (split)
            return launch_gemm_bf16x3_nt(A, lo(A), lda, Bm, lo(Bm), ldb, Cm, ldc, M, Nn, Kp, acc, bw.kpart, bw.kpart_floats, acc ? 3 : 4, st);
        return launch_gemm_bf16_nt(A, lda, Bm, ldb, Cm, ldc, M, Nn, Kp, acc, 0, st);
    }
    hipError_t rows1(const float* src, int ld, const int32_t* idx, int R, int K, uint16_t* dst, int ldd) const
    {
        return launch_cast_rows_bf16(src, ld, idx, R, K, dst, ldd, st, lo(dst), 1);
    }
    hipError_t mmt(uint16_t* A, int lda, uint16_t* Bm, int ldb, float* Cm, int ldc, int M, int Nn, int K, float* bias) const
    {
        return launch_gemm_bf16x3_tn(A, lo(A), lda, Bm, lo(Bm), ldb, Cm, ldc, M, Nn, K, 1, bias, bw.kpart, bw.kpart_floats, 3, st);
    }

    hipError_t scatter_into_zeroed(const float* packed, int ld, int n, float* dst, size_t bytes) const
    {
        ZeroList z;
        z.add(dst, bytes);
        const hipError_t e = launch_zero_regions(z, st);
        return e != hipSuccess ? e : launch_scatter_rows(packed, ld, live_rows, n, ld, dst, ld, st);
    }
    hipError_t wemb_scatter_add() const
    {
        if (live_rows) return launch_scatter_add_rows(w.dX2p + H, H + E, w.prevp, n_live, E, grads->Wemb, E, st);
        return launch_scatter_add_rows(w.dX2 + (size_t)Tv * N * (H + E) + H, H + E, w.prev, Tc * N, E, grads->Wemb, E, st);
    }
    hipError_t cast_dz2_rows() const
    {
        HIP_CHECK(rows(w.dZ2, 4 * H, nullptr, Re, 4 * H, bw.L, K4));
        return rows(dzd(), 4 * H, nullptr, Rd, 4 * H, bw.L + (size_t)Re * K4, K4);
    }

    hipError_t vocab_fused(int R, float* dO2t) const
    {
        const int Kv = bf16_pad(V), Hp1 = bf16_pad(H + 1);
        if (dlogits) HIP_CHECK(rows(dlogits, V, nullptr, R, V, bw.L, Kv));
        HIP_CHECK(rows1(w.O2 + (size_t)Tv * NH, H, live_rows, R, H, bw.AT, Hp1));
        HIP_CHECK(mmt(bw.AT, Hp1, bw.L, Kv, grads->embed_word_W, V, H, V, R, grads->embed_word_b));
        HIP_CHECK(rows(p->embed_word_W, V, nullptr, H, V, bw.W, Kv));
        return mm(bw.L, Kv, bw.W, Kv, dO2t, H, R, H, Kv, 0);
    }
    hipError_t vocab_tr(int R, float* dO2t) const
    {
        const int Kr = bf16_pad(R), Kv = bf16_pad(V);
// ... 254 lines not shown
{
    return split_grad_mode(N) == kGradSplit && split_fused();
}

int s2vt_softmax_nll_fwd_bwd_split(float* logits, int32_t ld, int32_t R, int32_t V, const int32_t* target, const float* coef, float smoothing,
                                   const float* smoothing_rows, float* nll, float* lp_target, const s2vt_dims* d, int32_t B, int32_t N,
                                   void* split_ws, size_t split_ws_bytes, s2vt_stream stream)
{
    if (!logits || !target || !coef || R < 0 || V <= 0 || ld < V || !dims_ok_res(d) || B <= 0 || N <= 0 || N % B || !split_ws) return S2VT_E_BADARG;
    if (V != d->n_words || (size_t)R > (size_t)d->n_caption_lstm_step * N || !s2vt_split_grad_active(N)) return S2VT_E_BADARG;
    if (reinterpret_cast<uintptr_t>(split_ws) & 255u) return S2VT_E_ALIGN;
    Carver cb(split_ws, split_ws_bytes);
    Bf16Ws bw{};
    carve_bf16(cb, d, B, N, &bw, true);
    if (!cb.ok()) return S2VT_E_WORKSPACE;
    const int Kv = bf16_pad(V);
    if (!softmax_nll_split_ok(logits, ld, V, bw.L, bw.L + bw.lo_delta, Kv) || !gemm_bf16x3_tn_ok(bf16_pad(d->lstm_dim + 1), Kv, R)) {
        HIP_TRY(launch_softmax_nll(logits, ld, R, V, target, coef, smoothing_rows ? 0.0f : smoothing, nll, lp_target, S(stream), smoothing_rows));
        return 1;
    }
    HIP_TRY(launch_softmax_nll_split(logits, ld, R, V, target, coef, smoothing_rows ? 0.0f : smoothing, nll, lp_target, bw.L, bw.L + bw.lo_delta, Kv,
                                     S(stream), smoothing_rows));
    return S2VT_OK;
}

int s2vt_split_grad_dlogits_planes(const s2vt_dims* d, int32_t B, int32_t N, size_t* hi_offset, size_t* lo_offset, int32_t* ld)
{
    if (!dims_ok_res(d) || B <= 0 || N <= 0 || N % B || !hi_offset || !lo_offset || !ld) return S2VT_E_BADARG;
    Carver cb(nullptr, 0);
    Bf16Ws bw{};
    carve_bf16(cb, d, B, N, &bw, true);
    *hi_offset = 0;
    *lo_offset = bw.lo_delta * sizeof(uint16_t);
    *ld = bf16_pad(d->n_words);
    return S2VT_OK;
}

int s2vt_gemm_bf16x3_tn(const uint16_t* Ah, const uint16_t* Al, int32_t lda, const uint16_t* Bh, const uint16_t* Bl, int32_t ldb, float* C,
                        int32_t ldc, int32_t M, int32_t N, int32_t K, int32_t accumulate, float* bias, void* scratch, size_t scratch_bytes,
                        s2vt_stream stream)
{
    if (!Ah || !Al || !Bh || !Bl || !C || M < 0 || N < 0 || K < 0 || lda < M + (bias ? 1 : 0) || ldb < N || ldc < N || (lda & 7) || (ldb & 7))
        return S2VT_E_BADARG;
    if (accumulate < 0 || accumulate > 1 || (scratch_bytes && !scratch) || !gemm_bf16x3_tn_ok(lda, ldb, K)) return S2VT_E_BADARG;
    if ((reinterpret_cast<uintptr_t>(Ah) | reinterpret_cast<uintptr_t>(Al) | reinterpret_cast<uintptr_t>(Bh) | reinterpret_cast<uintptr_t>(Bl)) & 15)
        return S2VT_E_ALIGN;
    HIP_TRY(launch_gemm_bf16x3_tn(Ah, Al, lda, Bh, Bl, ldb, C, ldc, M, N, K, accumulate, bias, static_cast<float*>(scratch), scratch_bytes / 4, 3, S(stream)));
    return S2VT_OK;
}

int s2vt_cast_bf16_split(const float* src, int32_t ld, const int32_t* rowidx, int32_t R, int32_t C, int32_t transpose, uint16_t* dst,
                         uint16_t* dst_lo, int32_t ldd, int32_t Rp, float* colsum, uint16_t* row_dst, uint16_t* row_dst_lo, int32_t row_ldd,
                         void* scratch, size_t scratch_bytes, s2vt_stream stream)
{
    if (!src || !dst || !dst_lo || R < 0 || C <= 0 || ld < C || transpose < 0 || transpose > 1) return S2VT_E_BADARG;
    if ((reinterpret_cast<uintptr_t>(dst) | reinterpret_cast<uintptr_t>(dst_lo)) & 15) return S2VT_E_ALIGN;
    if (!transpose) {
        if (colsum || row_dst || row_dst_lo || ldd < bf16_pad(C) || (ldd & 7)) return S2VT_E_BADARG;
        HIP_TRY(launch_cast_rows_bf16(src, ld, rowidx, R, C, dst, ldd, S(stream), dst_lo));
        return S2VT_OK;
    }
    if (Rp < R || Rp % kBf16K || ldd < Rp || (ldd & 7)) return S2VT_E_BADARG;
    if (!row_dst != !row_dst_lo) return S2VT_E_BADARG;
    if (row_dst && (row_ldd < bf16_pad(C) || (row_ldd & 3))) return S2VT_E_BADARG;
    if (row_dst && ((reinterpret_cast<uintptr_t>(row_dst) | reinterpret_cast<uintptr_t>(row_dst_lo)) & 7)) return S2VT_E_ALIGN;
    if (colsum && (!scratch || scratch_bytes < cast_tr_part_floats(Rp, C) * 4)) return S2VT_E_WORKSPACE;
    CastTrArgs a{src, ld, rowidx, R, C, dst, ldd, Rp, colsum, static_cast<float*>(scratch), row_dst, row_ldd, dst_lo, row_dst_lo};
    HIP_TRY(launch_cast_tr_bf16(a, S(stream)));
    return S2VT_OK;
}

int s2vt_gemm_bf16x3_nt(const uint16_t* Ah, const uint16_t* Al, int32_t lda, const uint16_t* Bh, const uint16_t* Bl, int32_t ldb, float* C,
                        int32_t ldc, int32_t M, int32_t N, int32_t Kp, int32_t accumulate, void* scratch, size_t scratch_bytes, s2vt_stream stream)
{
    if (!Ah || !Al || !Bh || !Bl || !C || M < 0 || N < 0 || Kp < 0 || Kp % kBf16K || lda < Kp || ldb < Kp || ldc < N || (lda & 7) || (ldb & 7))
        return S2VT_E_BADARG;
    if (accumulate < 0 || accumulate > 1 || (scratch_bytes && !scratch)) return S2VT_E_BADARG;
    if ((reinterpret_cast<uintptr_t>(Ah) | reinterpret_cast<uintptr_t>(Al) | reinterpret_cast<uintptr_t>(Bh) | reinterpret_cast<uintptr_t>(Bl)) & 15)
        return S2VT_E_ALIGN;
    HIP_TRY(launch_gemm_bf16x3_nt(Ah, Al, lda, Bh, Bl, ldb, C, ldc, M, N, Kp, accumulate, static_cast<float*>(scratch), scratch_bytes / 4, 3, S(stream)));
    return S2VT_OK;
}

int s2vt_cast_bf16(const float* src, int32_t ld, const int32_t* rowidx, int32_t R, int32_t C, int32_t transpose, uint16_t* dst, int32_t ldd,
                   int32_t Rp, float* colsum, uint16_t* row_dst, int32_t row_ldd, void* scratch, size_t scratch_bytes, s2vt_stream stream)
{
    if (!src || !dst || R < 0 || C <= 0 || ld < C || transpose < 0 || transpose > 1) return S2VT_E_BADARG;
    if (reinterpret_cast<uintptr_t>(dst) & 15) return S2VT_E_ALIGN;
    if (!transpose) {
        if (colsum || row_dst || ldd < bf16_pad(C) || (ldd & 7)) return S2VT_E_BADARG;
        HIP_TRY(launch_cast_rows_bf16(src, ld, rowidx, R, C, dst, ldd, S(stream)));
        return S2VT_OK;
    }
    if (Rp < R || Rp % kBf16K || ldd < Rp || (ldd & 7)) return S2VT_E_BADARG;
    if (row_dst && (row_ldd < bf16_pad(C) || (row_ldd & 3))) return S2VT_E_BADARG;
    if (row_dst && (reinterpret_cast<uintptr_t>(row_dst) & 7)) return S2VT_E_ALIGN;
    if (colsum && (!scratch || scratch_bytes < cast_tr_part_floats(Rp, C) * 4)) return S2VT_E_WORKSPACE;
    CastTrArgs a{src, ld, rowidx, R, C, dst, ldd, Rp, colsum, static_cast<float*>(scratch), row_dst, row_ldd};
    HIP_TRY(launch_cast_tr_bf16(a, S(stream)));
    return S2VT_OK;
}

int s2vt_gemm_bf16_nt(const uint16_t* A, int32_t lda, const uint16_t* Bm, int32_t ldb, float* C, int32_t ldc, int32_t M, int32_t N, int32_t Kp,
                      int32_t accumulate, int32_t mfma, s2vt_stream stream)
{
    if (!A || !Bm || !C || M < 0 || N < 0 || Kp < 0 || Kp % kBf16K || lda < Kp || ldb < Kp || ldc < N || (lda & 7) || (ldb & 7)) return S2VT_E_BADARG;
    if (accumulate < 0 || accumulate > 1 || (mfma != 0 && mfma != 16 && mfma != 32)) return S2VT_E_BADARG;
    if ((reinterpret_cast<uintptr_t>(A) | reinterpret_cast<uintptr_t>(Bm)) & 15) return S2VT_E_ALIGN;
    HIP_TRY(launch_gemm_bf16_nt(A, lda, Bm, ldb, C, ldc, M, N, Kp, accumulate, mfma, S(stream)));
    return S2VT_OK;
}

int s2vt_bptt_dvideo(const s2vt_dims* d, const s2vt_params* p, int32_t B, int32_t N, float* d_video, void* workspace,
                      size_t workspace_bytes, s2vt_stream stream)
{
    if (!dims_ok_res(d) || !p || !p->encode_image_W || !d_video || !workspace || B <= 0 || N <= 0 || N % B) return S2VT_E_BADARG;
    Carver c(workspace, workspace_bytes);
    TrainWs w;
    carve_train(c, d, B, N, &w);
    if (!c.ok()) return S2VT_E_WORKSPACE;
    hipStream_t st = S(stream);
    const int E = d->word_dim, D = d->dim_image, Tv = d->n_video_lstm_step;
    hipLaunchKernelGGL(enc_index_kernel, dim3((B * Tv + 255) / 256), dim3(256), 0, st, w.decidx, Tv, B);
    HIP_TRY(hipGetLastError());
    GemmArgs a;
    std::memset(&a, 0, sizeof(a));
    a.seg[0] = make_seg(w.dX1, E, E, 0, 0, w.decidx);
    a.nseg = 1;
    a.W = p->encode_image_W; a.ldw = E; a.M = B * Tv; a.N = D; a.C = d_video; a.ldc = D;
    HIP_TRY(launch_gemm(a, EPI_STORE_NT, -1, st));
    return S2VT_OK;
}

int s2vt_embed_scatter_add(const float* dE, int32_t ld, const int32_t* idx, int32_t R, int32_t E, float* dWemb,
                           s2vt_stream stream)
{
    if (!dE || !idx || !dWemb || R < 0 || E <= 0 || ld < E) return S2VT_E_BADARG;
    HIP_TRY(launch_scatter_add_rows(dE, ld, idx, R, E, dWemb, E, S(stream)));
    return S2VT_OK;
}

int s2vt_grad_finalize(float* g, const float* theta, int64_t n, const float* gscale, float weight_decay, float* sumsq,
                       s2vt_stream stream)
{
    if (!g || !sumsq || n < 0 || (weight_decay != 0.0f && !theta)) return S2VT_E_BADARG;
    HIP_TRY(launch_grad_finalize(g, theta, n, gscale, weight_decay, sumsq, S(stream)));
    return S2VT_OK;
}

int s2vt_adam_tf(float* theta, const float* g, float* m, float* v, int64_t n, const float* sumsq, float clip_norm,
                 float lr, int64_t step, float beta1, float beta2, float eps, s2vt_stream stream)
{
    return s2vt_adam_tf_guarded(theta, g, m, v, n, sumsq, clip_norm, lr, step, beta1, beta2, eps, nullptr, stream);
}

int s2vt_adam_tf_guarded(float* theta, const float* g, float* m, float* v, int64_t n, const float* sumsq, float clip_norm,
                         float lr, int64_t step, float beta1, float beta2, float eps, int32_t* applied_step, s2vt_stream stream)
{
    if (!theta || !g || !m || !v || n < 0 || step < 1) return S2VT_E_BADARG;
    if (chain_fault()) return S2VT_E_CHAIN_TIMEOUT;
    const double lr_t = (double)lr * sqrt(1.0 - pow((double)beta2, (double)step)) / (1.0 - pow((double)beta1, (double)step));
    HIP_TRY(launch_adam_tf(theta, g, m, v, n, sumsq, clip_norm, (float)lr_t, beta1, beta2, eps, S(stream), chain_fault_word(), applied_step,
                           (int32_t)step));
    return S2VT_OK;
}

// ... 11 lines not shown
```

multitask-end-to-end-video-captioning_amd/model.py:

```python
from __future__ import annotations

import math
from dataclasses import dataclass

import numpy as np
import torch

from . import dist as dp
from . import ops
from ._lib import PARAM_FIELDS

TF_NAMES = {
    "Wemb": "Wemb", "encode_image_W": "encode_image_W", "encode_image_b": "encode_image_b",
    "embed_word_W": "embed_word_W", "embed_word_b": "embed_word_b",
    "lstm1_W": "s2vt/LSTM1/basic_lstm_cell/weights", "lstm1_b": "s2vt/LSTM1/basic_lstm_cell/biases",
    "lstm2_W": "s2vt/LSTM2/basic_lstm_cell/weights", "lstm2_b": "s2vt/LSTM2/basic_lstm_cell/biases",
    "attr_W": "attr_W", "attr_b": "attr_b",
}
DECAYED = ("Wemb", "encode_image_W", "encode_image_b", "lstm1_W", "lstm2_W", "embed_word_W", "embed_word_b", "attr_W", "attr_b")
UNDECAYED = ("lstm1_b", "lstm2_b")


def param_shapes(dim_image, n_words, word_dim, lstm_dim, label_dim=0):
    E, H, V, D = word_dim, lstm_dim, n_words, dim_image
# ... 413 lines not shown
                ids[:len(sent)] = sent[:Tc]
            elif unshifted_softmax:
                from .beam_generator import BeamSearchGenerator
                ids = BeamSearchGenerator(self, 1).generate_unshifted_softmax(v)
            else:
                _, g = self.sample(v, 0, True)
                ids = g.cpu().numpy().astype(np.int64)[0]
            return {f"word_{t}": ids[t] for t in range(Tc)}
        sentence = [Output(f"word_{t}", fn, [video]) for t in range(Tc)]
        return video, sentence, []

    def _beam_decoder(self, B, beam):
        return ops.BeamDecoder(self.dims, B, beam, self.device)

    def beam_search(self, video, beam_size=3, length_normalization_factor=0.0, batch_size=64):
        from .beam_generator import BatchedBeamSearch
        gen = BatchedBeamSearch(self, beam_size, length_normalization_factor)
        n = video.shape[0] if hasattr(video, "shape") else len(video)
        out = []
        for a in range(0, n, batch_size):
            out += gen.generate(self._features(video[a:a + batch_size]))
        return out

    @staticmethod
    def active_steps(mask):
        if isinstance(mask, torch.Tensor):
            if mask.is_cuda:
                return None
            mask = mask.numpy()
        m = np.asarray(mask)
        if m.ndim != 2 or m.size == 0:
            return None
        live = np.flatnonzero(np.asarray(m != 0).any(axis=0))
        return int(live[-1]) + 1 if live.size else 1

    def live_rows(self, mask, steps):
        if isinstance(mask, torch.Tensor):
            if mask.is_cuda:
                return None
            mask = mask.numpy()
        if mask is None or ((self.dims.lstm_dim | self.dims.word_dim) & 3):
            return None
        m = np.asarray(mask)
        if m.ndim != 2 or m.size == 0:
            return None
        on = m[:, :steps] != 0
        if (on[:, 1:] & ~on[:, :-1]).any():
            return None
        tm = np.ascontiguousarray(on.T).reshape(-1)
        live = np.flatnonzero(tm).astype(np.int32)
        if live.size == 0 or live.size > 0.85 * tm.size:
            return None
        return torch.as_tensor(live).to(self.device)

    def _steps(self, active_steps, mask, local_ok=True):
        Tc = self.n_caption_lstm_step
        if active_steps is None or active_steps == 0:
            return Tc
        if isinstance(active_steps, str):
            if active_steps != "auto":
                raise ValueError("active_steps: an int, None or 'auto'")
            s = self.active_steps(mask) if (local_ok or self.world_size == 1) else None
            return Tc if s is None else max(1, min(Tc, s))
        return max(1, min(Tc, int(active_steps)))

    def _forward_loss(self, video, caption, coef_tm, smoothing, rep, video_base, keep, reuse_sampler_state=False, target_tm=None,
                      steps=None, live=None, row_ids=None):
        B = video.shape[0]
        N = caption.shape[0]
        steps = self.n_caption_lstm_step if steps is None else int(steps)
        R = steps * N
        vid, sid = self._row_ids(B, rep, video_base) if row_ids is None else row_ids
        seed = self.dropout_seed + 104729 * self.global_step
        state = None
        if reuse_sampler_state:
            ls = getattr(self, "_sampler_state", None)
            ok = (ls is not None and ls[2] is video and ls[3] == video._version and ls[4] == B and ls[5] == self.global_step
                  and ops.sample.last_state is not None and ops.sample.last_state[4] == ls[6])
            if not ok:
                raise RuntimeError("reuse_sampler_state needs model.sample() on this very video tensor, with the current "
                                   "weights, as the last sampler call before the update")
            state = (ls[0], ls[1])
        logits, ws = ops.teacher_forced_fwd(self.dims, self.store.params, video, caption, N, keep, seed, vid, sid,
                                            sampler_state=state, steps=steps, live=live)
        if callable(coef_tm):
            coef_tm = coef_tm()
        target = caption.t().contiguous().view(-1) if target_tm is None else target_tm
        if isinstance(smoothing, torch.Tensor):
            smoothing = smoothing[:R]
        target, coef = target[:R], coef_tm[:R]
        if live is not None:
            ix = live.long()
            target, coef = target[ix].contiguous(), coef[ix].contiguous()
            if isinstance(smoothing, torch.Tensor):
                smoothing = smoothing[ix].contiguous()
        dlogits = logits
        if self.grad_precision == "fp32" and ops.split_grad_active(N):
            nll, lp, in_planes = ops.softmax_nll_fwd_bwd_split(logits, target, coef, smoothing, self.dims, B, N)
            if in_planes:
                dlogits = _PlanesDlogits(logits, target, coef, smoothing)
        else:
            nll, lp = ops.softmax_nll_fwd_bwd(logits, target, coef, smoothing)
        self._coef_used = coef
        self._ctx = (video, N, dlogits, ws, keep, seed, vid, sid, steps, live)
        return nll, lp

    def backward(self, accumulate=False, overlap=None, keep_tail=False):
        if overlap is None:
            overlap = self.dp_overlap
        video, N, dlogits, ws, keep, seed, vid, sid, steps, live = self._ctx
        if isinstance(dlogits, _PlanesDlogits):
            dlogits = None
        st = self.store
        if not accumulate:
            ops.zero_(st.grad[:st.numel] if keep_tail else st.grad)
        self._pending = []
        self._early = None
        if dp.active() and overlap:
            def span(first, last):
                return st.offsets[first], st.offsets[last] + (int(np.prod(st.shapes[last])) + 63) // 64 * 64
            args = (self.dims, st.params, st.grads, video, N, dlogits, ws, keep, seed, vid, sid)
            ops.bptt_bwd(*args, phase=1, steps=steps, live=live, precision=self.grad_precision)
            lo1, hi1 = span("embed_word_W", "embed_word_b")
            self._pending.append(dp.allreduce_async(st.grad[lo1:hi1]))
            with ops.chain_hold():
                ops.bptt_bwd(*args, phase=3, steps=steps, live=live, precision=self.grad_precision)
                lo2, hi2 = span("lstm2_W", "lstm2_W")
                assert hi2 == lo1, "bucket layout: lstm2_W sits right below embed_word_W"
                self._pending.append(dp.allreduce_async(st.grad[lo2:hi2]))
                self._early = (lo2, hi1)
                ops.bptt_bwd(*args, phase=4, steps=steps, live=live, precision=self.grad_precision)
        else:
            ops.bptt_bwd(self.dims, st.params, st.grads, video, N, dlogits, ws, keep, seed, vid, sid, steps=steps, live=live,
                         precision=self.grad_precision)

    def video_grad(self):
        video, N, _, ws, *_ = self._ctx
        return ops.bptt_dvideo(self.dims, self.store.params, video.shape[0], N, ws)

    def apply_gradients(self, mask_sum, lr, clip_norm, weight_decay=0.0, attr_scale=None, extra_sumsq=None, decay_all=False, loss_terms=None,
                        optimizer="adam"):
        if optimizer not in ("adam", "sgd"):
            raise ValueError(f"optimizer must be 'adam' or 'sgd', got {optimizer!r}")
        st = self.store
        early = getattr(self, "_early", None)
        if early is not None and dp.active():
            lo, hi = early
            if mask_sum is not None:
                st.grad[st.numel] = mask_sum
            pend = getattr(self, "_pending", [])
            pend.append(dp.allreduce_async(st.grad[:lo]))
            pend.append(dp.allreduce_async(st.grad[hi:]))
            dp.wait_all(pend, st.grad)
            self._pending, self._early = [], None
            gsum = st.grad[st.numel:st.numel + 1]
        else:
            gsum = dp.allreduce_bucket(st.grad, st.numel, mask_sum)
        self._sumsq = torch.empty(1, dtype=torch.float32, device=self.device)
        self._loss = torch.empty(1, dtype=torch.float32, device=self.device) if loss_terms is not None else None
        coef_, nll_, msum_ = loss_terms if loss_terms is not None else (None, None, None)
        ops.step_scalars(coef_, nll_, msum_, gsum, self._loss, self._gscale, self._sumsq)
        nd = st.n_decayed
        a0 = st.offsets.get("attr_W", nd)
        ops.grad_finalize(st.grad[:a0], st.theta[:a0], self._gscale, weight_decay, self._sumsq)
        if a0 < nd:
            want = 1.0 if attr_scale is None else float(attr_scale)
            if getattr(self, "_ascale_val", None) != want:
# ... 518 lines not shown
```

multitask-end-to-end-video-captioning_amd/ops.py:

```python
from __future__ import annotations

import ctypes as C

import torch

from . import _lib
from ._lib import AttnParams, Dims, Operand, Params, check, lib


def _stream():
    return C.c_void_p(torch.cuda.current_stream().cuda_stream)


def _ptr(t):
    return None if t is None else C.c_void_p(t.data_ptr())


def _chk_f32(*ts):
    for t in ts:
        if t is not None:
            assert t.is_cuda and t.dtype == torch.float32, "expected a CUDA float32 tensor"


def make_dims(dim_image, n_words, word_dim, lstm_dim, n_video_lstm_step, n_caption_lstm_step, label_dim=0, residual=False) -> Dims:
# ... 366 lines not shown
    emb = torch.empty((B * dims.n_video_lstm_step, dims.word_dim), dtype=torch.float32, device=video.device)
    check(lib().s2vt_frame_embed_fwd(C.byref(dims), C.byref(params), _ptr(video), B, _ptr(emb), _stream()),
          "s2vt_frame_embed_fwd")
    return emb


def zero_(*tensors):
    ts = [t for t in tensors if t is not None and t.numel()]
    for i in range(0, len(ts), 8):
        grp = ts[i:i + 8]
        for t in grp:
            assert t.is_cuda and t.is_contiguous() and (t.numel() * t.element_size()) % 4 == 0
        ptrs = (C.c_void_p * len(grp))(*[t.data_ptr() for t in grp])
        nb = (C.c_size_t * len(grp))(*[t.numel() * t.element_size() for t in grp])
        check(lib().s2vt_zero_regions(ptrs, nb, len(grp), _stream()), "s2vt_zero_regions")


_ws_cache = {}


def workspace(nbytes: int, device, tag="default"):
    key = (tag, str(device))
    t = _ws_cache.get(key)
    if t is None or t.numel() < nbytes:
        t = torch.empty(max(nbytes, 256), dtype=torch.uint8, device=device)
        assert t.data_ptr() % 256 == 0
        _ws_cache[key] = t
    return t


def sample(dims: Dims, params: Params, video, K: int, seed: int, video_base: int = 0, with_greedy: bool = True, stop_at_eos: bool = False):
    _chk_f32(video)
    assert video.is_contiguous()
    B = video.shape[0]
    g = 1 if with_greedy else 0
    L = lib()
    nbytes = L.s2vt_sample_workspace_bytes(C.byref(dims), B, K, g)
    ws = workspace(nbytes, video.device, "sample")
    ids = torch.empty(((K + g) * B, dims.n_caption_lstm_step), dtype=torch.int32, device=video.device)
    if stop_at_eos:
        check(L.s2vt_sample_ex(C.byref(dims), C.byref(params), _ptr(video), B, K, g, seed, video_base, 1, _ptr(ids), _ptr(ws),
                               ws.numel(), _stream()), "s2vt_sample_ex")
    else:
        sbytes = L.s2vt_sample_screen_workspace_bytes(C.byref(dims), B, K, g)
        if sbytes > 0:
            sws = workspace(sbytes, video.device, "sample_screen")
            check(L.s2vt_sample_screened(C.byref(dims), C.byref(params), _ptr(video), B, K, g, seed, video_base, _ptr(ids), _ptr(ws),
                                         ws.numel(), _ptr(sws), sws.numel(), _stream()), "s2vt_sample_screened")
        else:
            check(L.s2vt_sample(C.byref(dims), C.byref(params), _ptr(video), B, K, g, seed, video_base, _ptr(ids), _ptr(ws),
                                ws.numel(), _stream()), "s2vt_sample")
    sample.serial += 1
    sample.last_state = (ws, (K + g) * B, video.data_ptr(), B, sample.serial)
    return ids[:K * B], (ids[K * B:] if with_greedy else None)


sample.last_state = None
sample.serial = 0


def sample_mix(dims: Dims, params: Params, video, caption, p_gt: float, seed: int, video_base: int = 0, with_greedy: bool = True):
    _chk_f32(video)
    assert video.is_contiguous()
    B = video.shape[0]
    assert caption.is_cuda and caption.dtype == torch.int32 and caption.is_contiguous()
    assert tuple(caption.shape) == (B, dims.n_caption_lstm_step)
    g = 1 if with_greedy else 0
    L = lib()
    nbytes = L.s2vt_sample_mix_workspace_bytes(C.byref(dims), B, g)
    ws = workspace(nbytes, video.device, "sample_mix")
    ids = torch.empty(((1 + g) * B, dims.n_caption_lstm_step), dtype=torch.int32, device=video.device)
    check(L.s2vt_sample_mix(C.byref(dims), C.byref(params), _ptr(video), B, _ptr(caption), float(p_gt), g, seed, video_base, _ptr(ids),
                            _ptr(ws), ws.numel(), _stream()), "s2vt_sample_mix")
    return ids[:B], (ids[B:] if with_greedy else None)


def train_workspace(dims: Dims, B: int, N: int, device):
    nbytes = lib().s2vt_train_workspace_bytes(C.byref(dims), B, N)
    assert nbytes > 0, "bad dims / B / N (N must be a multiple of B)"
    return workspace(nbytes, device, "train")


def teacher_forced_fwd(dims: Dims, params: Params, video, caption, N: int, keep=1.0, seed=0, video_id=None,
                       sample_id=None, ws=None, logits=None, sampler_state=None, steps=None, live=None):
    _chk_f32(video)
    assert caption.is_cuda and caption.dtype == torch.int32 and caption.is_contiguous() and caption.shape[0] == N
    assert caption.shape[1] == dims.n_caption_lstm_step
    B = video.shape[0]
    steps = dims.n_caption_lstm_step if steps is None else int(steps)
    if ws is None:
        ws = train_workspace(dims, B, N, video.device)
    R = steps * N
    if live is not None:
        assert live.is_cuda and live.dtype == torch.int32 and live.is_contiguous() and live.dim() == 1
        R = live.numel()
    if logits is None:
        logits = torch.empty((R, dims.n_words), dtype=torch.float32, device=video.device)
    assert logits.shape[0] == R
    sws, srows = sampler_state if sampler_state is not None else (None, 0)
    check(lib().s2vt_teacher_forced_fwd_live(C.byref(dims), C.byref(params), _ptr(video), B, N, _ptr(caption), steps,
                                             _ptr(live), 0 if live is None else live.numel(), float(keep), seed,
                                              _ptr(video_id), _ptr(sample_id), _ptr(logits), _ptr(ws), ws.numel(), _ptr(sws),
                                              0 if sws is None else sws.numel(), srows, _stream()),
          "s2vt_teacher_forced_fwd")
    return logits, ws


def scheduled_fwd(dims: Dims, params: Params, video, caption, N: int, p_gt: float, coin_seed: int, loss_weight=1.0, keep=1.0, seed=0,
                  video_id=None, sample_id=None, ws=None, mask_sum=None, mask_sum_copy=None):
    _chk_f32(video, mask_sum, mask_sum_copy)
    assert video.is_contiguous()
    assert caption.is_cuda and caption.dtype == torch.int32 and caption.is_contiguous()
    Tc = dims.n_caption_lstm_step
    assert tuple(caption.shape) == (N, Tc)
    for t in (video_id, sample_id):
        assert t is not None and t.is_cuda and t.dtype == torch.int32 and t.is_contiguous() and t.numel() == N, "video_id / sample_id: int32 [N]"
    B = video.shape[0]
    dev = video.device
    L = lib()
    if ws is None:
        ws = train_workspace(dims, B, N, dev)
    nb = L.s2vt_scheduled_scratch_bytes(C.byref(dims), N)
    assert nb > 0, "bad dims / N"
    scratch = workspace(nb, dev, "scheduled")
    out = dict(logits=torch.empty((Tc * N, dims.n_words), dtype=torch.float32, device=dev),
               generated=torch.empty((N, Tc), dtype=torch.int32, device=dev), fed=torch.empty((N, Tc), dtype=torch.int32, device=dev),
               mask=torch.empty((N, Tc), dtype=torch.float32, device=dev), coef_tm=torch.empty(Tc * N, dtype=torch.float32, device=dev),
               target_tm=torch.empty(Tc * N, dtype=torch.int32, device=dev),
               mask_sum=torch.empty(1, dtype=torch.float32, device=dev) if mask_sum is None else mask_sum, ws=ws)
    check(L.s2vt_scheduled_fwd(C.byref(dims), C.byref(params), _ptr(video), B, N, _ptr(caption), float(p_gt), int(coin_seed) & (2 ** 64 - 1),
                               float(loss_weight), float(keep), seed, _ptr(video_id), _ptr(sample_id), _ptr(out["logits"]), _ptr(out["generated"]),
                               _ptr(out["fed"]), _ptr(out["mask"]), _ptr(out["coef_tm"]), _ptr(out["target_tm"]), _ptr(out["mask_sum"]),
                               _ptr(mask_sum_copy), _ptr(ws), ws.numel(), _ptr(scratch), scratch.numel(), _stream()), "s2vt_scheduled_fwd")
    return out


def softmax_nll_fwd_bwd(logits, target, coef, smoothing=0.0):
    _chk_f32(logits, coef)
    R, V = logits.shape
    assert target.dtype == torch.int32 and target.is_cuda and target.numel() == R and coef.numel() == R
    nll = torch.empty(R, dtype=torch.float32, device=logits.device)
    lp = torch.empty_like(nll)
    if isinstance(smoothing, torch.Tensor):
        _chk_f32(smoothing)
        assert smoothing.numel() == R and smoothing.is_contiguous()
        check(lib().s2vt_softmax_nll_fwd_bwd_rows(_ptr(logits), logits.stride(0), R, V, _ptr(target), _ptr(coef), _ptr(smoothing),
                                                  _ptr(nll), _ptr(lp), _stream()), "s2vt_softmax_nll_fwd_bwd_rows")
        return nll, lp
    check(lib().s2vt_softmax_nll_fwd_bwd(_ptr(logits), logits.stride(0), R, V, _ptr(target), _ptr(coef), float(smoothing),
                                         _ptr(nll), _ptr(lp), _stream()), "s2vt_softmax_nll_fwd_bwd")
    return nll, lp


def split_grad_active(N: int) -> bool:
    return bool(lib().s2vt_split_grad_active(int(N)))


def softmax_nll_fwd_bwd_split(logits, target, coef, smoothing, dims: Dims, B: int, N: int):
    _chk_f32(logits, coef)
    R, V = logits.shape
    assert target.dtype == torch.int32 and target.is_cuda and target.numel() == R and coef.numel() == R
    nll = torch.empty(R, dtype=torch.float32, device=logits.device)
    lp = torch.empty_like(nll)
    rows = None
    if isinstance(smoothing, torch.Tensor):
        _chk_f32(smoothing)
        assert smoothing.numel() == R and smoothing.is_contiguous()
        rows, smoothing = smoothing, 0.0
    sws = split_grad_workspace(dims, B, N, logits.device)
    rc = lib().s2vt_softmax_nll_fwd_bwd_split(_ptr(logits), logits.stride(0), R, V, _ptr(target), _ptr(coef), float(smoothing), _ptr(rows),
                                              _ptr(nll), _ptr(lp), C.byref(dims), B, N, _ptr(sws), sws.numel(), _stream())
    if rc != 1:
        check(rc, "s2vt_softmax_nll_fwd_bwd_split")
    return nll, lp, rc == 0


def train_workspace_dz2(dims: Dims, B: int, N: int, ws):
    off, n = C.c_size_t(), C.c_size_t()
    check(lib().s2vt_train_workspace_dz2(C.byref(dims), B, N, C.byref(off), C.byref(n)), "s2vt_train_workspace_dz2")
    return ws[off.value:off.value + 4 * n.value].view(torch.float32).view(-1, N, 4 * dims.lstm_dim)


def split_grad_dlogits_planes(dims: Dims, B: int, N: int, R: int, device):
    hi_off, lo_off, ld = C.c_size_t(), C.c_size_t(), C.c_int32()
    check(lib().s2vt_split_grad_dlogits_planes(C.byref(dims), B, N, C.byref(hi_off), C.byref(lo_off), C.byref(ld)), "s2vt_split_grad_dlogits_planes")
    sws = split_grad_workspace(dims, B, N, device)
    n = R * ld.value * 2
    return tuple(sws[o.value:o.value + n].view(torch.bfloat16).view(R, ld.value) for o in (hi_off, lo_off))


def softmax_unshifted_argmax(logits, want_probs=False):
    _chk_f32(logits)
    R, V = logits.shape
    ids = torch.empty(R, dtype=torch.int32, device=logits.device)
    probs = torch.empty((R, V), dtype=torch.float32, device=logits.device) if want_probs else None
    check(lib().s2vt_softmax_unshifted_argmax(_ptr(logits), logits.stride(0), R, V, _ptr(ids), _ptr(probs), _stream()),
          "s2vt_softmax_unshifted_argmax")
    return ids, probs


GRAD_PRECISIONS = ("fp32", "bf16")


def bf16_grad_workspace(dims: Dims, B: int, N: int, device):
    nbytes = lib().s2vt_bf16_grad_workspace_bytes(C.byref(dims), B, N)
    assert nbytes > 0, "bad dims / B / N (N must be a multiple of B)"
    return workspace(nbytes, device, "bf16_grad")


def split_grad_workspace(dims: Dims, B: int, N: int, device):
    nbytes = lib().s2vt_split_grad_workspace_bytes(C.byref(dims), B, N)
    assert nbytes > 0, "bad dims / B / N (N must be a multiple of B)"
    return workspace(nbytes, device, "split_grad")


def bptt_bwd(dims: Dims, params: Params, grads: Params, video, N: int, dlogits, ws, keep=1.0, seed=0, video_id=None,
             sample_id=None, phase=0, steps=None, live=None, precision="fp32"):
    _chk_f32(video, dlogits)
    if precision not in GRAD_PRECISIONS:
        raise ValueError(f"precision must be one of {GRAD_PRECISIONS}, got {precision!r}")
    steps = dims.n_caption_lstm_step if steps is None else int(steps)
    assert dlogits is None or dlogits.shape[0] == (steps * N if live is None else live.numel())
    assert dlogits is not None or precision == "fp32"
    if precision == "bf16":
        bws = bf16_grad_workspace(dims, video.shape[0], N, video.device)
        check(lib().s2vt_bptt_bwd_bf16(C.byref(dims), C.byref(params), C.byref(grads), _ptr(video), video.shape[0], N, _ptr(dlogits),
                                       steps, _ptr(live), 0 if live is None else live.numel(), float(keep), seed, _ptr(video_id),
                                       _ptr(sample_id), _ptr(ws), ws.numel(), phase, _ptr(bws), bws.numel(), _stream()),
              "s2vt_bptt_bwd_bf16")
        return
    sws = split_grad_workspace(dims, video.shape[0], N, video.device)
    check(lib().s2vt_bptt_bwd_split(C.byref(dims), C.byref(params), C.byref(grads), _ptr(video), video.shape[0], N, _ptr(dlogits),
                                    steps, _ptr(live), 0 if live is None else live.numel(), float(keep), seed, _ptr(video_id),
                                    _ptr(sample_id), _ptr(ws), ws.numel(), phase, _ptr(sws), sws.numel(), _stream()),
          "s2vt_bptt_bwd_split")


def cast_bf16(src, rowidx=None, transpose=False, pad_rows=None, colsum=None, row_copy=False):
    _chk_f32(src, colsum)
    assert src.dim() == 2 and src.stride(1) == 1
    if rowidx is not None:
        assert rowidx.is_cuda and rowidx.dtype == torch.int32 and rowidx.is_contiguous()
    R = src.shape[0] if rowidx is None else rowidx.numel()
    Cc = src.shape[1]
    Kp = (Cc + 63) // 64 * 64
    dev = src.device
    if not transpose:
        out = torch.empty((R, Kp), dtype=torch.bfloat16, device=dev)
        check(lib().s2vt_cast_bf16(_ptr(src), src.stride(0), _ptr(rowidx), R, Cc, 0, _ptr(out), Kp, 0, None, None, 0, None, 0, _stream()),
              "s2vt_cast_bf16")
        return out
    Rp = (R + 63) // 64 * 64 if pad_rows is None else int(pad_rows)
    out = torch.empty((Cc, Rp), dtype=torch.bfloat16, device=dev)
    rows = torch.empty((R, Kp), dtype=torch.bfloat16, device=dev) if row_copy else None
    scratch = workspace(4 * ((Rp + 255) // 256) * Cc, dev, "cast_bf16") if colsum is not None else None
    check(lib().s2vt_cast_bf16(_ptr(src), src.stride(0), _ptr(rowidx), R, Cc, 1, _ptr(out), Rp, Rp, _ptr(colsum), _ptr(rows), Kp,
                               _ptr(scratch), 0 if scratch is None else scratch.numel(), _stream()), "s2vt_cast_bf16")
    return (out, rows) if row_copy else out


def gemm_bf16x3_tn(Ah, Al, Bh, Bl, M=None, N=None, out=None, accumulate=False, split_k=True, bias=None):
    for t in (Ah, Al, Bh, Bl):
        assert t.is_cuda and t.dtype == torch.bfloat16 and t.stride(1) == 1
    assert Ah.shape == Al.shape and Bh.shape == Bl.shape and Ah.stride(0) == Al.stride(0) and Bh.stride(0) == Bl.stride(0)
    K = Ah.shape[0]
    assert Bh.shape[0] == K
    M = Ah.shape[1] if M is None else int(M)
    N = Bh.shape[1] if N is None else int(N)
    if out is None:
        assert not accumulate
        out = torch.empty((M, N), dtype=torch.float32, device=Ah.device)
    _chk_f32(out, bias)
    assert out.shape[0] == M and out.shape[1] == N and out.stride(1) == 1
    scratch = workspace(32 * (M + 1) * N, Ah.device, "gemm_bf16x3") if split_k and M * N else None
    check(lib().s2vt_gemm_bf16x3_tn(_ptr(Ah), _ptr(Al), Ah.stride(0), _ptr(Bh), _ptr(Bl), Bh.stride(0), _ptr(out), out.stride(0), M, N, K,
                                    int(bool(accumulate)), _ptr(bias), _ptr(scratch), 0 if scratch is None else scratch.numel(), _stream()),
          "s2vt_gemm_bf16x3_tn")
    return out


def cast_bf16_split(src, rowidx=None, transpose=False, pad_rows=None, colsum=None, row_copy=False):
    _chk_f32(src, colsum)
    assert src.dim() == 2 and src.stride(1) == 1
    if rowidx is not None:
        assert rowidx.is_cuda and rowidx.dtype == torch.int32 and rowidx.is_contiguous()
    R = src.shape[0] if rowidx is None else rowidx.numel()
    Cc = src.shape[1]
    Kp = (Cc + 63) // 64 * 64
    dev = src.device
    if not transpose:
        hi = torch.empty((R, Kp), dtype=torch.bfloat16, device=dev)
        lo = torch.empty_like(hi)
        check(lib().s2vt_cast_bf16_split(_ptr(src), src.stride(0), _ptr(rowidx), R, Cc, 0, _ptr(hi), _ptr(lo), Kp, 0, None, None, None, 0,
                                         None, 0, _stream()), "s2vt_cast_bf16_split")
        return hi, lo
    Rp = (R + 63) // 64 * 64 if pad_rows is None else int(pad_rows)
    hi = torch.empty((Cc, Rp), dtype=torch.bfloat16, device=dev)
    lo = torch.empty_like(hi)
    rh = torch.empty((R, Kp), dtype=torch.bfloat16, device=dev) if row_copy else None
    rl = torch.empty((R, Kp), dtype=torch.bfloat16, device=dev) if row_copy else None
    scratch = workspace(4 * ((Rp + 255) // 256) * Cc, dev, "cast_bf16") if colsum is not None else None
    check(lib().s2vt_cast_bf16_split(_ptr(src), src.stride(0), _ptr(rowidx), R, Cc, 1, _ptr(hi), _ptr(lo), Rp, Rp, _ptr(colsum), _ptr(rh),
                                     _ptr(rl), Kp, _ptr(scratch), 0 if scratch is None else scratch.numel(), _stream()), "s2vt_cast_bf16_split")
    return ((hi, lo), (rh, rl)) if row_copy else (hi, lo)


def gemm_bf16x3_nt(Ah, Al, Bh, Bl, out=None, accumulate=False, split_k=True):
    for t in (Ah, Al, Bh, Bl):
        assert t.is_cuda and t.dtype == torch.bfloat16 and t.stride(1) == 1
    assert Ah.shape == Al.shape and Bh.shape == Bl.shape and Ah.stride(0) == Al.stride(0) and Bh.stride(0) == Bl.stride(0)
    M, Kp = Ah.shape
    N = Bh.shape[0]
    if out is None:
        assert not accumulate
        out = torch.empty((M, N), dtype=torch.float32, device=Ah.device)
    _chk_f32(out)
    assert out.shape[0] == M and out.shape[1] == N and out.stride(1) == 1
    scratch = workspace(32 * M * N, Ah.device, "gemm_bf16x3") if split_k and M * N else None
    check(lib().s2vt_gemm_bf16x3_nt(_ptr(Ah), _ptr(Al), Ah.stride(0), _ptr(Bh), _ptr(Bl), Bh.stride(0), _ptr(out), out.stride(0), M, N, Kp,
                                    int(bool(accumulate)), _ptr(scratch), 0 if scratch is None else scratch.numel(), _stream()),
          "s2vt_gemm_bf16x3_nt")
    return out


def gemm_bf16_nt(A, B, out=None, accumulate=False, mfma=0, n=None):
    assert A.is_cuda and B.is_cuda and A.dtype == torch.bfloat16 and B.dtype == torch.bfloat16
    assert A.stride(1) == 1 and B.stride(1) == 1 and A.shape[1] == B.shape[1]
    M, Kp = A.shape
    N = B.shape[0] if n is None else int(n)
    if out is None:
        assert not accumulate
        out = torch.empty((M, N), dtype=torch.float32, device=A.device)
    _chk_f32(out)
    assert out.shape[0] == M and out.shape[1] == N and out.stride(1) == 1
    check(lib().s2vt_gemm_bf16_nt(_ptr(A), A.stride(0), _ptr(B), B.stride(0), _ptr(out), out.stride(0), M, N, Kp, int(bool(accumulate)),
                                  int(mfma), _stream()), "s2vt_gemm_bf16_nt")
    return out


def bptt_dvideo(dims: Dims, params: Params, B: int, N: int, ws):
    import torch
    out = torch.empty(B, dims.n_video_lstm_step, dims.dim_image, device=ws.device, dtype=torch.float32)
    check(lib().s2vt_bptt_dvideo(C.byref(dims), C.byref(params), B, N, _ptr(out), _ptr(ws), ws.numel(), _stream()), "s2vt_bptt_dvideo")
    return out


def caption_mask(ids, mask_sum=None, want_mask=True, want_target=True, mask_sum_copy=None):
    assert ids.is_cuda and ids.dtype == torch.int32 and ids.is_contiguous()
    N, Tc = ids.shape
    mask = torch.empty((N, Tc), dtype=torch.float32, device=ids.device) if want_mask else None
    tgt = torch.empty(N * Tc, dtype=torch.int32, device=ids.device) if want_target else None
    if mask_sum is None:
        mask_sum = torch.empty(1, dtype=torch.float32, device=ids.device)
    check(lib().s2vt_caption_mask(_ptr(ids), N, Tc, _ptr(mask), _ptr(tgt), _ptr(mask_sum), _ptr(mask_sum_copy), _stream()), "s2vt_caption_mask")
    return mask, tgt, mask_sum


def pg_coef(mask, rewards, baseline, scale=1.0):
    _chk_f32(mask, rewards, baseline)
    N, Tc = mask.shape
# ... 599 lines not shown
```

Baseline: 679,700.

## Route teacher-forced forward GEMMs through split-bf16x3 matrix kernels with fused bias

Adds an NN form of the bf16x3 (hi/lo split) GEMM kernel, with mixed transpose handling in the LDS reads and a column-bias epilogue in both the direct-store and split-K reduce paths. Adds a split teacher-forced forward entry point that casts activations to hi/lo bf16 planes and runs the vocabulary projection on matrix cores instead of the fp32 path. The Python model enables it when grad precision is fp32 and split mode is active for the batch size, staged by an environment variable. The intent is to replace the fp32 forward logits GEMM with emulated-fp32 bf16 matrix-core work, at the cost of extra cast passes and a small precision difference.

New measurement: 714,900, median of 6. 5.2% higher.

```diff
diff --git a/include/s2vt.h b/include/s2vt.h
--- a/include/s2vt.h
+++ b/include/s2vt.h
@@ -244,6 +244,19 @@
 int s2vt_softmax_nll_fwd_bwd_split(float* logits, int32_t ld, int32_t R, int32_t V, const int32_t* target, const float* coef, float smoothing,
                                    const float* smoothing_rows, float* nll, float* lp_target, const s2vt_dims* d, int32_t B, int32_t N,
                                    void* split_ws, size_t split_ws_bytes, s2vt_stream stream);
+
+int s2vt_gemm_bf16x3_nn(const uint16_t* Ah, const uint16_t* Al, int32_t lda, const uint16_t* Bh, const uint16_t* Bl, int32_t ldb, float* C,
+                        int32_t ldc, int32_t M, int32_t N, int32_t K, int32_t accumulate, const float* bias, void* scratch, size_t scratch_bytes,
+                        s2vt_stream stream);
+
+int s2vt_split_fwd_stage(void);
+int s2vt_split_fwd_active(int32_t N);
+int s2vt_teacher_forced_fwd_split(const s2vt_dims* d, const s2vt_params* p, const float* video, int32_t B, int32_t N,
+                                  const int32_t* caption, int32_t caption_steps, const int32_t* live_rows, int32_t n_live, float keep,
+                                  uint64_t seed, const int32_t* video_id, const int32_t* sample_id, float* logits_out,
+                                  void* workspace, size_t workspace_bytes, const void* sampler_workspace,
+                                  size_t sampler_workspace_bytes, int32_t sampler_rows, void* split_ws, size_t split_ws_bytes,
+                                  s2vt_stream stream);
 
 int s2vt_bptt_dvideo(const s2vt_dims* d, const s2vt_params* p, int32_t B, int32_t N, float* d_video, void* workspace,
                       size_t workspace_bytes, s2vt_stream stream);
diff --git a/multitask-end-to-end-video-captioning_amd/_lib.py b/multitask-end-to-end-video-captioning_amd/_lib.py
--- a/multitask-end-to-end-video-captioning_amd/_lib.py
+++ b/multitask-end-to-end-video-captioning_amd/_lib.py
@@ -136,7 +136,12 @@
     "s2vt_cast_bf16_split": (C.c_int, [_vp, _i32, _vp, _i32, _i32, _i32, _vp, _vp, _i32, _i32, _vp, _vp, _vp, _i32, _vp, _sz, _vp]),
     "s2vt_gemm_bf16x3_nt": (C.c_int, [_vp, _vp, _i32, _vp, _vp, _i32, _vp, _i32, _i32, _i32, _i32, _i32, _vp, _sz, _vp]),
     "s2vt_gemm_bf16x3_tn": (C.c_int, [_vp, _vp, _i32, _vp, _vp, _i32, _vp, _i32, _i32, _i32, _i32, _i32, _vp, _vp, _sz, _vp]),
+    "s2vt_gemm_bf16x3_nn": (C.c_int, [_vp, _vp, _i32, _vp, _vp, _i32, _vp, _i32, _i32, _i32, _i32, _i32, _vp, _vp, _sz, _vp]),
     "s2vt_split_grad_active": (C.c_int, [_i32]),
+    "s2vt_split_fwd_stage": (C.c_int, []),
+    "s2vt_split_fwd_active": (C.c_int, [_i32]),
+    "s2vt_teacher_forced_fwd_split": (C.c_int, [_DP, _PP, _vp, _i32, _i32, _vp, _i32, _vp, _i32, _f32, _u64, _vp, _vp, _vp, _vp, _sz, _vp, _sz, _i32,
+                                                _vp, _sz, _vp]),
     "s2vt_train_workspace_dz2": (C.c_int, [_DP, _i32, _i32, C.POINTER(_sz), C.POINTER(_sz)]),
     "s2vt_split_grad_dlogits_planes": (C.c_int, [_DP, _i32, _i32, C.POINTER(_sz), C.POINTER(_sz), C.POINTER(_i32)]),
     "s2vt_softmax_nll_fwd_bwd_split": (C.c_int, [_vp, _i32, _i32, _i32, _vp, _vp, _f32, _vp, _vp, _vp, _DP, _i32, _i32, _vp, _sz, _vp]),
diff --git a/multitask-end-to-end-video-captioning_amd/csrc/bwd_bf16.hip b/multitask-end-to-end-video-captioning_amd/csrc/bwd_bf16.hip
--- a/multitask-end-to-end-video-captioning_amd/csrc/bwd_bf16.hip
+++ b/multitask-end-to-end-video-captioning_amd/csrc/bwd_bf16.hip
@@ -15,9 +15,9 @@
 template <bool SPLIT>
 __global__ __launch_bounds__(256) void cast_rows_bf16_kernel(const float* __restrict__ src, int ld, const int32_t* __restrict__ rowidx,
                                                              int R, int K, uint16_t* __restrict__ dst, int ldd, int vec,
-                                                             uint16_t* __restrict__ dst_lo, int ones)
-{
-    const int cpr = bf16_pad(K + ones) / 8;
+                                                             uint16_t* __restrict__ dst_lo, int ones, int width)
+{
+    const int cpr = width / 8;
     const long total = (long)R * cpr;
     for (long i = (long)blockIdx.x * 256 + threadIdx.x; i < total; i += (long)gridDim.x * 256) {
         const int r = (int)(i / cpr), k0 = (int)(i % cpr) * 8;
@@ -241,7 +241,10 @@
     float* part;
     int K;
     float* bias; int Mo;
+    const float* cbias;
 };
+
+enum : int { kX3NT = 0, kX3TN = 1, kX3NN = 2 };
 
 constexpr int kX3BK = 32, kX3Slots = 4, kX3Plane = kTile * kX3BK;
 constexpr int kX3Lds = kX3Slots * 4 * kX3Plane * 2;
@@ -250,9 +253,10 @@
 typedef short i16x4 __attribute__((ext_vector_type(4)));
 typedef __attribute__((address_space(3))) i16x4* x3_tr_ptr;
 
-template <bool TN>
+template <int FORM>
 __global__ __launch_bounds__(512) void gemm_bf16x3_kernel(GemmX3Args g)
 {
+    constexpr bool ATN = FORM == kX3TN, BTN = FORM != kX3NT;
     extern __shared__ __attribute__((aligned(16))) uint16_t x3lds[];
     const int nwg = g.tiles_m * g.tiles_n, orig = blockIdx.x;
     const int xcd = orig & 7, q = nwg >> 3, rem = nwg & 7;
@@ -264,12 +268,13 @@
 
     if (w >= 4) {
         const int p = w - 4;
+        const bool TN = ATN == BTN ? ATN : p >= 2;
         const uint16_t* const plane = p == 0 ? g.Ah : p == 1 ? g.Al : p == 2 ? g.Bh : g.Bl;
         const int r0 = p < 2 ? m0 : n0, rows = p < 2 ? g.M : g.N, ld = p < 2 ? g.lda : g.ldb;
         const __amdgpu_buffer_rsrc_t rs = __builtin_amdgcn_make_buffer_rsrc(const_cast<uint16_t*>(plane + (TN ? (size_t)r0 : (size_t)r0 * ld)), 0,
                                                                             TN ? (int)(((uint32_t)g.K * (uint32_t)ld - (uint32_t)r0) * 2u) : (int)kOob, 0x00020000);
         uint32_t voff[kX3Dma];
-        if constexpr (TN) {
+        if (TN) {
             const int kr = lane >> 4, s = lane & 15;
 #pragma unroll
             for (int b = 0; b < kX3Dma; ++b)
@@ -284,7 +289,7 @@
         }
         auto issue = [&](int ks) __attribute__((always_inline)) {
             uint16_t* const dst = x3lds + ((ks % kX3Slots) * 4 + p) * kX3Plane;
-            if constexpr (TN) {
+            if (TN) {
                 const uint32_t koff = (uint32_t)(kbeg + ks) * kX3BK * (uint32_t)ld * 2u;
 #pragma unroll
                 for (int b = 0; b < kX3Dma; ++b)
@@ -333,7 +338,16 @@
         for (int pl = 0; pl < 4; ++pl)
 #pragma unroll
             for (int i = 0; i < 4; ++i)
-                if constexpr (TN) {
+                if constexpr (ATN != BTN) {
+                    if (pl < 2) {
+                        f[pl][i] = *reinterpret_cast<const bf16x8*>(s + pl * kX3Plane + (wr * 64 + i * 16) * kX3BK + fofs);
+                    } else {
+                        const uint16_t* const a = s + pl * kX3Plane + tofs + (((wc * 4 + i) ^ tswz) << 4);
+                        const i16x4 lo4 = __builtin_amdgcn_ds_read_tr16_b64_v4i16((x3_tr_ptr)a);
+                        const i16x4 hi4 = __builtin_amdgcn_ds_read_tr16_b64_v4i16((x3_tr_ptr)(a + 4 * kTile));
+                        f[pl][i] = __builtin_bit_cast(bf16x8, __builtin_shufflevector(lo4, hi4, 0, 1, 2, 3, 4, 5, 6, 7));
+                    }
+                } else if constexpr (ATN) {
                     const uint16_t* const a = s + pl * kX3Plane + tofs + ((((pl < 2 ? wr : wc) * 4 + i) ^ tswz) << 4);
                     const i16x4 lo4 = __builtin_amdgcn_ds_read_tr16_b64_v4i16((x3_tr_ptr)a);
                     const i16x4 hi4 = __builtin_amdgcn_ds_read_tr16_b64_v4i16((x3_tr_ptr)(a + 4 * kTile));
@@ -381,8 +395,13 @@
                 const int row = m0 + wr * 64 + i * 16 + (lane >> 4) * 4 + e, col = n0 + wc * 64 + j * 16 + (lane & 15);
                 if (row < g.M && col < g.N) {
                     float* c = out + (size_t)row * ldo + col;
-                    *c = add ? *c + acc[i][j][e] : acc[i][j][e];
-                } else if (TN && row == g.M && g.bias && col < g.N) {
+                    if constexpr (FORM == kX3NN) {
+                        const float v = !g.part && g.cbias ? acc[i][j][e] + g.cbias[col] : acc[i][j][e];
+                        *c = add ? *c + v : v;
+                    } else {
+                        *c = add ? *c + acc[i][j][e] : acc[i][j][e];
+                    }
+                } else if (FORM == kX3TN && row == g.M && g.bias && col < g.N) {
                     if (g.part) out[(size_t)row * ldo + col] = acc[i][j][e];
                     else g.bias[col] += acc[i][j][e];
                 }
@@ -390,7 +409,7 @@
 }
 
 __global__ __launch_bounds__(256) void reduce_slabs_kernel(const float* __restrict__ part, int slabs, int M, int N, float* __restrict__ C, int ldc,
-                                                           int accumulate, int Mo, float* __restrict__ bias)
+                                                           int accumulate, int Mo, float* __restrict__ bias, const float* __restrict__ cbias)
 {
     const size_t MN = (size_t)Mo * N;
     for (size_t i = (size_t)blockIdx.x * 256 + threadIdx.x; i < MN; i += (size_t)gridDim.x * 256) {
@@ -399,6 +418,7 @@
         const size_t r = i / N;
         if (r < (size_t)M) {
             float* c = C + r * ldc + i % N;
+            if (cbias) s = s + cbias[i % N];
             *c = accumulate ? *c + s : s;
         } else {
             bias[i % N] += s;
@@ -408,16 +428,18 @@
 }
 
 hipError_t launch_cast_rows_bf16(const float* src, int ld, const int32_t* rowidx, int R, int K, uint16_t* dst, int ldd, hipStream_t st,
-                                 uint16_t* dst_lo, int ones)
+                                 uint16_t* dst_lo, int ones, int width)
 {
     if (R <= 0 || K <= 0) return hipSuccess;
     ones = ones ? 1 : 0;
+    if (width <= 0) width = bf16_pad(K + ones);
+    if ((width & 7) || width < K + ones) return hipErrorInvalidValue;
     const int vec = !((reinterpret_cast<uintptr_t>(src) & 15) || (ld & 3));
-    const long chunks = (long)R * (bf16_pad(K + ones) / 8);
+    const long chunks = (long)R * (width / 8);
     const long blocks = (chunks + 255) / 256;
     const dim3 grid((unsigned)(blocks < 8192 ? blocks : 8192));
-    if (dst_lo) hipLaunchKernelGGL(cast_rows_bf16_kernel<true>, grid, dim3(256), 0, st, src, ld, rowidx, R, K, dst, ldd, vec, dst_lo, ones);
-    else hipLaunchKernelGGL(cast_rows_bf16_kernel<false>, grid, dim3(256), 0, st, src, ld, rowidx, R, K, dst, ldd, vec, dst_lo, ones);
+    if (dst_lo) hipLaunchKernelGGL(cast_rows_bf16_kernel<true>, grid, dim3(256), 0, st, src, ld, rowidx, R, K, dst, ldd, vec, dst_lo, ones, width);
+    else hipLaunchKernelGGL(cast_rows_bf16_kernel<false>, grid, dim3(256), 0, st, src, ld, rowidx, R, K, dst, ldd, vec, dst_lo, ones, width);
     return hipGetLastError();
 }
 
@@ -478,16 +500,16 @@
 }
 
 namespace {
-template <bool TN>
+template <int FORM>
 hipError_t launch_x3(const uint16_t* Ah, const uint16_t* Al, int lda, const uint16_t* Bh, const uint16_t* Bl, int ldb, float* C, int ldc, int M, int N,
-                     int Kp, int accumulate, float* bias, float* part, size_t part_floats, int cls, hipStream_t st)
+                     int Kp, int accumulate, float* bias, float* part, size_t part_floats, int cls, hipStream_t st, const float* cbias = nullptr)
 {
     if (M <= 0 || N <= 0) return hipSuccess;
-    static const hipError_t attr = hipFuncSetAttribute(reinterpret_cast<const void*>(gemm_bf16x3_kernel<TN>), hipFuncAttributeMaxDynamicSharedMemorySize, kX3Lds);
+    static const hipError_t attr = hipFuncSetAttribute(reinterpret_cast<const void*>(gemm_bf16x3_kernel<FORM>), hipFuncAttributeMaxDynamicSharedMemorySize, kX3Lds);
     if (attr != hipSuccess) return attr;
     GemmX3Args g;
     g.Ah = Ah; g.Al = Al; g.lda = lda; g.Bh = Bh; g.Bl = Bl; g.ldb = ldb; g.C = C; g.ldc = ldc; g.M = M; g.N = N;
-    g.K = Kp; g.bias = bias; g.Mo = M + (bias ? 1 : 0);
+    g.K = Kp; g.bias = bias; g.Mo = M + (bias ? 1 : 0); g.cbias = cbias;
     const int Kr = bf16_pad(Kp);
     g.nk = Kr / kX3BK; g.accumulate = accumulate;
     g.tiles_m = (g.Mo + kTile - 1) / kTile; g.tiles_n = (N + kTile - 1) / kTile;
@@ -504,15 +526,15 @@
         if (pe != hipSuccess) return pe;
         (void)hipEventRecord(e0, st);
     }
-    hipLaunchKernelGGL(gemm_bf16x3_kernel<TN>, grid, dim3(512), kX3Lds, st, g);
+    hipLaunchKernelGGL(gemm_bf16x3_kernel<FORM>, grid, dim3(512), kX3Lds, st, g);
     if (slabs > 1) {
         const size_t MN = (size_t)g.Mo * N, blocks = (MN + 255) / 256;
         hipLaunchKernelGGL(reduce_slabs_kernel, dim3((unsigned)(blocks < 4096 ? blocks : 4096)), dim3(256), 0, st, (const float*)part, slabs, M, N, C, ldc,
-                           accumulate, g.Mo, bias);
+                           accumulate, g.Mo, bias, cbias);
     }
     if (prof) {
         (void)hipEventRecord(e1, st);
-        prof_record(cls, 16, cls == 2 ? "x3_128x128(dma) pick screen" : cls == 3 ? "x3_128x128(dma) wgrad" : "x3_128x128(dma) dgrad",
+        prof_record(cls, 16, cls == 0 ? "x3_128x128(dma) fwd" : cls == 2 ? "x3_128x128(dma) pick screen" : cls == 3 ? "x3_128x128(dma) wgrad" : "x3_128x128(dma) dgrad",
                     2.0 * M * (double)N * Kp, e0, e1);
     }
     return hipGetLastError();
@@ -522,7 +544,7 @@
 hipError_t launch_gemm_bf16x3_nt(const uint16_t* Ah, const uint16_t* Al, int lda, const uint16_t* Bh, const uint16_t* Bl, int ldb, float* C, int ldc,
                                  int M, int N, int Kp, int accumulate, float* part, size_t part_floats, int cls, hipStream_t st)
 {
-    return launch_x3<false>(Ah, Al, lda, Bh, Bl, ldb, C, ldc, M, N, Kp, accumulate, nullptr, part, part_floats, cls, st);
+    return launch_x3<kX3NT>(Ah, Al, lda, Bh, Bl, ldb, C, ldc, M, N, Kp, accumulate, nullptr, part, part_floats, cls, st);
 }
 
 bool gemm_bf16x3_tn_ok(int lda, int ldb, int K)
@@ -535,7 +557,14 @@
                                  int M, int N, int K, int accumulate, float* bias, float* part, size_t part_floats, int cls, hipStream_t st)
 {
     if (!gemm_bf16x3_tn_ok(lda, ldb, K)) return hipErrorInvalidValue;
-    return launch_x3<true>(Ah, Al, lda, Bh, Bl, ldb, C, ldc, M, N, K, accumulate, bias, part, part_floats, cls, st);
-}
-
-}
+    return launch_x3<kX3TN>(Ah, Al, lda, Bh, Bl, ldb, C, ldc, M, N, K, accumulate, bias, part, part_floats, cls, st);
+}
+
+hipError_t launch_gemm_bf16x3_nn(const uint16_t* Ah, const uint16_t* Al, int lda, const uint16_t* Bh, const uint16_t* Bl, int ldb, float* C, int ldc,
+                                 int M, int N, int K, int accumulate, const float* cbias, float* part, size_t part_floats, int cls, hipStream_t st)
+{
+    if (!gemm_bf16x3_tn_ok(ldb, ldb, K) || lda < bf16_pad(K) || (cbias && accumulate)) return hipErrorInvalidValue;
+    return launch_x3<kX3NN>(Ah, Al, lda, Bh, Bl, ldb, C, ldc, M, N, K, accumulate, nullptr, part, part_floats, cls, st, cbias);
+}
+
+}
diff --git a/multitask-end-to-end-video-captioning_amd/csrc/internal.h b/multitask-end-to-end-video-captioning_amd/csrc/internal.h
--- a/multitask-end-to-end-video-captioning_amd/csrc/internal.h
+++ b/multitask-end-to-end-video-captioning_amd/csrc/internal.h
@@ -272,7 +272,7 @@
     lo = pack2(a - __uint_as_float(hi << 16), b - __uint_as_float(hi & 0xffff0000u));
 }
 hipError_t launch_cast_rows_bf16(const float* src, int ld, const int32_t* rowidx, int R, int K, uint16_t* dst, int ldd, hipStream_t st,
-                                 uint16_t* dst_lo = nullptr, int ones = 0);
+                                 uint16_t* dst_lo = nullptr, int ones = 0, int width = 0);
 struct CastTrArgs {
     const float* src; int ld; const int32_t* rowidx; int R, C;
     uint16_t* dst; int ldd; int Rp;
@@ -290,6 +290,8 @@
 bool gemm_bf16x3_tn_ok(int lda, int ldb, int K);
 hipError_t launch_gemm_bf16x3_tn(const uint16_t* Ah, const uint16_t* Al, int lda, const uint16_t* Bh, const uint16_t* Bl, int ldb, float* C, int ldc,
                                  int M, int N, int K, int accumulate, float* bias, float* part, size_t part_floats, int cls, hipStream_t st);
+hipError_t launch_gemm_bf16x3_nn(const uint16_t* Ah, const uint16_t* Al, int lda, const uint16_t* Bh, const uint16_t* Bl, int ldb, float* C, int ldc,
+                                 int M, int N, int K, int accumulate, const float* cbias, float* part, size_t part_floats, int cls, hipStream_t st);
 bool softmax_nll_split_ok(const float* logits, int ld, int V, const uint16_t* hi, const uint16_t* lo, int ldp);
 hipError_t launch_softmax_nll_split(const float* logits, int ld, int R, int V, const int32_t* target, const float* coef, float smoothing, float* nll,
                                     float* lp_t, uint16_t* hi, uint16_t* lo, int ldp, hipStream_t st, const float* smooth_rows = nullptr);
diff --git a/multitask-end-to-end-video-captioning_amd/csrc/train.hip b/multitask-end-to-end-video-captioning_amd/csrc/train.hip
--- a/multitask-end-to-end-video-captioning_amd/csrc/train.hip
+++ b/multitask-end-to-end-video-captioning_amd/csrc/train.hip
@@ -263,7 +263,7 @@
 
 int unroll_front(const s2vt_dims* d, const s2vt_params* p, const float* video, int B, int N, int T, float keep, uint64_t seed,
                  const int32_t* video_id, const int32_t* sample_id, const TrainWs& w, const void* sampler_workspace,
-                 size_t sampler_workspace_bytes, int sampler_rows, s2vt_stream stream)
+                 size_t sampler_workspace_bytes, int sampler_rows, s2vt_stream stream, bool encode_partials = true)
 {
     const int H = d->lstm_dim, E = d->word_dim, Tv = d->n_video_lstm_step;
     const size_t NH = (size_t)N * H, BH = (size_t)B * H;
@@ -306,7 +306,7 @@
                                 nullptr, 0, B, H, T, 1.0f, none, 0, w.chain_abuf, w.chain_sync, st));
     }
     HIP_TRY(launch_expand_dropout(w.H1 + BH, w.O1, T, B, N, H, keep, seed, 256u, video_id, sample_id, st));
-    {
+    if (encode_partials) {
         ASeg se = make_seg(w.O1, H, H, 0);
         HIP_TRY(store_call(&se, 1, p->lstm2_W, 4 * H, nullptr, w.G2, 4 * H, Tv * N, 4 * H, 0, -1, st));
     }
@@ -530,17 +530,22 @@
                                         workspace, workspace_bytes, sampler_workspace, sampler_workspace_bytes, sampler_rows, stream);
 }
 
-int s2vt_teacher_forced_fwd_live(const s2vt_dims* d, const s2vt_params* p, const float* video, int32_t B, int32_t N,
-                                 const int32_t* caption, int32_t caption_steps, const int32_t* live_rows, int32_t n_live, float keep,
-                                 uint64_t seed, const int32_t* video_id, const int32_t* sample_id, float* logits, void* workspace,
-                                 size_t workspace_bytes, const void* sampler_workspace, size_t sampler_workspace_bytes,
-                                 int32_t sampler_rows, s2vt_stream stream)
+constexpr int kSplitFwdDefault = 1;
+static bool split_mode_on(int N);
+
+static int teacher_forced_fwd_body(const s2vt_dims* d, const s2vt_params* p, const float* video, int32_t B, int32_t N,
+                                   const int32_t* caption, int32_t caption_steps, const int32_t* live_rows, int32_t n_live, float keep,
+                                   uint64_t seed, const int32_t* video_id, const int32_t* sample_id, float* logits, void* workspace,
+                                   size_t workspace_bytes, const void* sampler_workspace, size_t sampler_workspace_bytes,
+                                   int32_t sampler_rows, s2vt_stream stream, void* split_ws, size_t split_ws_bytes, bool split_entry, int stage)
 {
     if ((live_rows == nullptr) != (n_live == 0) || n_live < 0) return S2VT_E_BADARG;
     if (!dims_ok_res(d) || !params_ok(p) || !video || !caption || !logits || !workspace || B <= 0 || N <= 0 || N % B)
         return S2VT_E_BADARG;
     if (!(keep > 0.0f) || (keep < 1.0f && (!video_id || !sample_id))) return S2VT_E_BADARG;
+    if (split_entry && !split_ws) return S2VT_E_BADARG;
     if (reinterpret_cast<uintptr_t>(workspace) & 255u) return S2VT_E_ALIGN;
+    if (split_entry && (reinterpret_cast<uintptr_t>(split_ws) & 255u)) return S2VT_E_ALIGN;
     if (chain_fault()) return S2VT_E_CHAIN_TIMEOUT;
     if (caption_steps < 1 || caption_steps > d->n_caption_lstm_step) return S2VT_E_BADARG;
     if (live_rows && (n_live > caption_steps * N || ((d->lstm_dim | d->word_dim) & 3))) return S2VT_E_BADARG;
@@ -550,24 +555,57 @@
     TrainWs w;
     carve_train(c, d, B, N, &w);
     if (!c.ok()) return S2VT_E_WORKSPACE;
+    Bf16Ws bw{};
+    if (split_entry) {
+        Carver cb(split_ws, split_ws_bytes);
+        carve_bf16(cb, d, B, N, &bw, true);
+        if (!cb.ok()) return S2VT_E_WORKSPACE;
+    }
     hipStream_t st = S(stream);
+    const size_t NH = (size_t)N * H;
+    const int Rd = live_rows ? n_live : Tc * N;
+    const int K4 = bf16_pad(4 * H), Kv = bf16_pad(V), Hp1 = bf16_pad(H + 1), HEp = bf16_pad(H + E);
+    const bool split_on = split_entry && stage >= 1 && split_mode_on(N) && !(H & 7);
+    const size_t bt_cap = split_entry ? (size_t)(bw.AT - bw.BT) : 0, at_cap = split_entry ? (size_t)(bw.L + bw.lo_delta - bw.AT) : 0;
+    uint16_t* const o2p = (size_t)Rd * Hp1 <= at_cap ? bw.AT : (size_t)Rd * Hp1 <= bt_cap ? bw.BT : nullptr;
+    const bool split_logits = split_on && o2p && gemm_bf16x3_tn_ok(Kv, Kv, H);
+    const bool split_g2 = split_on && stage >= 2 && gemm_bf16x3_tn_ok(K4, K4, H + E) && (size_t)(Tv * N > Rd ? Tv * N : Rd) * HEp <= bt_cap;
+    auto lo = [&](uint16_t* hi) { return hi + bw.lo_delta; };
+    auto nn = [&](uint16_t* A, int lda, uint16_t* Bm, int ldb, float* Cm, int ldc, int M, int Nn, int K, const float* cbias) {
+        return launch_gemm_bf16x3_nn(A, lo(A), lda, Bm, lo(Bm), ldb, Cm, ldc, M, Nn, K, 0, cbias, bw.kpart, bw.kpart_floats, 0, st);
+    };
 
     HIP_TRY(launch_prep_caption(caption, w.prev, w.tgt, N, d->n_caption_lstm_step, st));
     {
         const int rc = unroll_front(d, p, video, B, N, T, keep, seed, video_id, sample_id, w, sampler_workspace, sampler_workspace_bytes,
-                                    sampler_rows, stream);
+                                    sampler_rows, stream, !split_g2);
         if (rc != S2VT_OK) return rc;
     }
-    const size_t NH = (size_t)N * H;
     NoiseIds ids{video_id, sample_id, seed};
+    if (split_g2) {
+        HIP_TRY(launch_cast_rows_bf16(p->lstm2_W, 4 * H, nullptr, H + E, 4 * H, bw.W, K4, st, lo(bw.W)));
+        HIP_TRY(launch_cast_rows_bf16(w.O1, H, nullptr, Tv * N, H, bw.BT, bf16_pad(H), st, lo(bw.BT)));
+        HIP_TRY(nn(bw.BT, bf16_pad(H), bw.W, K4, w.G2, 4 * H, Tv * N, 4 * H, H, nullptr));
+        if (live_rows) HIP_TRY(launch_gather_i32(w.prev, live_rows, n_live, w.prevp, st));
+        HIP_TRY(launch_cast_rows_bf16(w.O1 + (size_t)Tv * NH, H, live_rows, Rd, H, bw.BT, HEp, st, lo(bw.BT), 0, H));
+        HIP_TRY(launch_cast_rows_bf16(p->Wemb, E, live_rows ? w.prevp : w.prev, Rd, E, bw.BT + H, HEp, st, lo(bw.BT) + H, 0, HEp - H));
+    }
     {
         if (!live_rows) {
-            ASeg sd[2] = {make_seg(w.O1 + (size_t)Tv * NH, H, H, 0), make_seg(p->Wemb, E, E, H, 0, w.prev)};
-            HIP_TRY(store_call(sd, 2, p->lstm2_W, 4 * H, nullptr, w.G2 + (size_t)Tv * 4 * NH, 4 * H, Tc * N, 4 * H, 0, -1, st));
+            if (split_g2) {
+                HIP_TRY(nn(bw.BT, HEp, bw.W, K4, w.G2 + (size_t)Tv * 4 * NH, 4 * H, Tc * N, 4 * H, H + E, nullptr));
+            } else {
+                ASeg sd[2] = {make_seg(w.O1 + (size_t)Tv * NH, H, H, 0), make_seg(p->Wemb, E, E, H, 0, w.prev)};
+                HIP_TRY(store_call(sd, 2, p->lstm2_W, 4 * H, nullptr, w.G2 + (size_t)Tv * 4 * NH, 4 * H, Tc * N, 4 * H, 0, -1, st));
+            }
         } else {
-            HIP_TRY(launch_gather_i32(w.prev, live_rows, n_live, w.prevp, st));
-            ASeg sd[2] = {make_seg(w.O1 + (size_t)Tv * NH, H, H, 0, 0, live_rows), make_seg(p->Wemb, E, E, H, 0, w.prevp)};
-            HIP_TRY(store_call(sd, 2, p->lstm2_W, 4 * H, nullptr, w.dZ2p, 4 * H, n_live, 4 * H, 0, -1, st));
+            if (split_g2) {
+                HIP_TRY(nn(bw.BT, HEp, bw.W, K4, w.dZ2p, 4 * H, n_live, 4 * H, H + E, nullptr));
+            } else {
+                HIP_TRY(launch_gather_i32(w.prev, live_rows, n_live, w.prevp, st));
+                ASeg sd[2] = {make_seg(w.O1 + (size_t)Tv * NH, H, H, 0, 0, live_rows), make_seg(p->Wemb, E, E, H, 0, w.prevp)};
+                HIP_TRY(store_call(sd, 2, p->lstm2_W, 4 * H, nullptr, w.dZ2p, 4 * H, n_live, 4 * H, 0, -1, st));
+            }
             float* const dec = w.G2 + (size_t)Tv * 4 * NH;
             ZeroList z;
             z.add(dec, (size_t)Tc * N * 4 * H * 4);
@@ -582,9 +620,52 @@
                             w.O2, NH, N, H, T, keep, ids, 512u, w.chain_abuf, w.chain_sync, st, rec_live ? w.perm : nullptr,
                             rec_live ? w.nlive : nullptr));
     if (is_residual(d)) HIP_TRY(launch_add_inplace(w.O2 + (size_t)Tv * NH, w.O1 + (size_t)Tv * NH, (size_t)Tc * NH, st));
+    if (split_logits) {
+        HIP_TRY(launch_cast_rows_bf16(w.O2 + (size_t)Tv * NH, H, live_rows, Rd, H, o2p, Hp1, st, lo(o2p), 1));
+        HIP_TRY(launch_cast_rows_bf16(p->embed_word_W, V, nullptr, H, V, bw.W, Kv, st, lo(bw.W)));
+        HIP_TRY(nn(o2p, Hp1, bw.W, Kv, logits, V, Rd, V, H, p->embed_word_b));
+        return S2VT_OK;
+    }
     ASeg so = make_seg(w.O2 + (size_t)Tv * NH, H, H, 0, 0, live_rows);
-    HIP_TRY(store_call(&so, 1, p->embed_word_W, V, p->embed_word_b, logits, V, live_rows ? n_live : Tc * N, V, 0, -1, st));
-    return S2VT_OK;
+    HIP_TRY(store_call(&so, 1, p->embed_word_W, V, p->embed_word_b, logits, V, Rd, V, 0, -1, st));
+    return S2VT_OK;
+}
+
+int s2vt_teacher_forced_fwd_live(const s2vt_dims* d, const s2vt_params* p, const float* video, int32_t B, int32_t N,
+                                 const int32_t* caption, int32_t caption_steps, const int32_t* live_rows, int32_t n_live, float keep,
+                                 uint64_t seed, const int32_t* video_id, const int32_t* sample_id, float* logits, void* workspace,
+                                 size_t workspace_bytes, const void* sampler_workspace, size_t sampler_workspace_bytes,
+                                 int32_t sampler_rows, s2vt_stream stream)
+{
+    return teacher_forced_fwd_body(d, p, video, B, N, caption, caption_steps, live_rows, n_live, keep, seed, video_id, sample_id, logits,
+                                   workspace, workspace_bytes, sampler_workspace, sampler_workspace_bytes, sampler_rows, stream, nullptr, 0,
+                                   false, 0);
+}
+
+int s2vt_split_fwd_stage(void)
+{
+    static const int stage = [] {
+        const char* e = getenv("S2VT_SPLIT_FWD");
+        if (e && (e[0] == '0' || e[0] == '1' || e[0] == '2') && !e[1]) return e[0] - '0';
+        return kSplitFwdDefault;
+    }();
+    return stage;
+}
+
+int s2vt_split_fwd_active(int32_t N)
+{
+    return split_mode_on(N) ? s2vt_split_fwd_stage() : 0;
+}
+
+int s2vt_teacher_forced_fwd_split(const s2vt_dims* d, const s2vt_params* p, const float* video, int32_t B, int32_t N,
+                                  const int32_t* caption, int32_t caption_steps, const int32_t* live_rows, int32_t n_live, float keep,
+                                  uint64_t seed, const int32_t* video_id, const int32_t* sample_id, float* logits, void* workspace,
+                                  size_t workspace_bytes, const void* sampler_workspace, size_t sampler_workspace_bytes,
+                                  int32_t sampler_rows, void* split_ws, size_t split_ws_bytes, s2vt_stream stream)
+{
+    return teacher_forced_fwd_body(d, p, video, B, N, caption, caption_steps, live_rows, n_live, keep, seed, video_id, sample_id, logits,
+                                   workspace, workspace_bytes, sampler_workspace, sampler_workspace_bytes, sampler_rows, stream, split_ws,
+                                   split_ws_bytes, true, s2vt_split_fwd_stage());
 }
 
 size_t s2vt_scheduled_scratch_bytes(const s2vt_dims* d, int32_t N)
@@ -750,6 +831,7 @@
     static const int on = [] { const char* e = getenv("S2VT_SPLIT_GRADS"); return e ? atoi(e) : 1; }();
     return on && N > 256 ? kGradSplit : kGradFp32;
 }
+static bool split_mode_on(int N) { return split_grad_mode(N) == kGradSplit; }
 static bool split_recurrence()
 {
     static const bool on = [] { const char* e = getenv("S2VT_BCHAIN_SPLIT"); return !(e && e[0] == '0'); }();
@@ -1170,6 +1252,19 @@
     return S2VT_OK;
 }
 
+int s2vt_gemm_bf16x3_nn(const uint16_t* Ah, const uint16_t* Al, int32_t lda, const uint16_t* Bh, const uint16_t* Bl, int32_t ldb, float* C,
+                        int32_t ldc, int32_t M, int32_t N, int32_t K, int32_t accumulate, const float* bias, void* scratch, size_t scratch_bytes,
+                        s2vt_stream stream)
+{
+    if (!Ah || !Al || !Bh || !Bl || !C || M < 0 || N < 0 || K < 0 || lda < bf16_pad(K) || ldb < N || ldc < N || (lda & 7) || (ldb & 7))
+        return S2VT_E_BADARG;
+    if (accumulate < 0 || accumulate > 1 || (bias && accumulate) || (scratch_bytes && !scratch) || !gemm_bf16x3_tn_ok(ldb, ldb, K)) return S2VT_E_BADARG;
+    if ((reinterpret_cast<uintptr_t>(Ah) | reinterpret_cast<uintptr_t>(Al) | reinterpret_cast<uintptr_t>(Bh) | reinterpret_cast<uintptr_t>(Bl)) & 15)
+        return S2VT_E_ALIGN;
+    HIP_TRY(launch_gemm_bf16x3_nn(Ah, Al, lda, Bh, Bl, ldb, C, ldc, M, N, K, accumulate, bias, static_cast<float*>(scratch), scratch_bytes / 4, 0, S(stream)));
+    return S2VT_OK;
+}
+
 int s2vt_cast_bf16(const float* src, int32_t ld, const int32_t* rowidx, int32_t R, int32_t C, int32_t transpose, uint16_t* dst, int32_t ldd,
                    int32_t Rp, float* colsum, uint16_t* row_dst, int32_t row_ldd, void* scratch, size_t scratch_bytes, s2vt_stream stream)
 {
diff --git a/multitask-end-to-end-video-captioning_amd/model.py b/multitask-end-to-end-video-captioning_amd/model.py
--- a/multitask-end-to-end-video-captioning_amd/model.py
+++ b/multitask-end-to-end-video-captioning_amd/model.py
@@ -519,7 +519,8 @@
                                    "weights, as the last sampler call before the update")
             state = (ls[0], ls[1])
         logits, ws = ops.teacher_forced_fwd(self.dims, self.store.params, video, caption, N, keep, seed, vid, sid,
-                                            sampler_state=state, steps=steps, live=live)
+                                            sampler_state=state, steps=steps, live=live,
+                                            split=self.grad_precision == "fp32" and ops.split_fwd_active(N) > 0)
         if callable(coef_tm):
             coef_tm = coef_tm()
         target = caption.t().contiguous().view(-1) if target_tm is None else target_tm
diff --git a/multitask-end-to-end-video-captioning_amd/ops.py b/multitask-end-to-end-video-captioning_amd/ops.py
--- a/multitask-end-to-end-video-captioning_amd/ops.py
+++ b/multitask-end-to-end-video-captioning_amd/ops.py
@@ -472,7 +472,7 @@
 
 
 def teacher_forced_fwd(dims: Dims, params: Params, video, caption, N: int, keep=1.0, seed=0, video_id=None,
-                       sample_id=None, ws=None, logits=None, sampler_state=None, steps=None, live=None):
+                       sample_id=None, ws=None, logits=None, sampler_state=None, steps=None, live=None, split=False):
     _chk_f32(video)
     assert caption.is_cuda and caption.dtype == torch.int32 and caption.is_contiguous() and caption.shape[0] == N
     assert caption.shape[1] == dims.n_caption_lstm_step
@@ -488,6 +488,14 @@
         logits = torch.empty((R, dims.n_words), dtype=torch.float32, device=video.device)
     assert logits.shape[0] == R
     sws, srows = sampler_state if sampler_state is not None else (None, 0)
+    if split:
+        gws = split_grad_workspace(dims, B, N, video.device)
+        check(lib().s2vt_teacher_forced_fwd_split(C.byref(dims), C.byref(params), _ptr(video), B, N, _ptr(caption), steps,
+                                                  _ptr(live), 0 if live is None else live.numel(), float(keep), seed,
+                                                  _ptr(video_id), _ptr(sample_id), _ptr(logits), _ptr(ws), ws.numel(), _ptr(sws),
+                                                  0 if sws is None else sws.numel(), srows, _ptr(gws), gws.numel(), _stream()),
+              "s2vt_teacher_forced_fwd_split")
+        return logits, ws
     check(lib().s2vt_teacher_forced_fwd_live(C.byref(dims), C.byref(params), _ptr(video), B, N, _ptr(caption), steps,
                                              _ptr(live), 0 if live is None else live.numel(), float(keep), seed,
                                               _ptr(video_id), _ptr(sample_id), _ptr(logits), _ptr(ws), ws.numel(), _ptr(sws),
@@ -546,6 +554,14 @@
     return bool(lib().s2vt_split_grad_active(int(N)))
 
 
+def split_fwd_stage() -> int:
+    return int(lib().s2vt_split_fwd_stage())
+
+
+def split_fwd_active(N: int) -> int:
+    return int(lib().s2vt_split_fwd_active(int(N)))
+
+
 def softmax_nll_fwd_bwd_split(logits, target, coef, smoothing, dims: Dims, B: int, N: int):
     _chk_f32(logits, coef)
     R, V = logits.shape
@@ -666,6 +682,25 @@
     check(lib().s2vt_gemm_bf16x3_tn(_ptr(Ah), _ptr(Al), Ah.stride(0), _ptr(Bh), _ptr(Bl), Bh.stride(0), _ptr(out), out.stride(0), M, N, K,
                                     int(bool(accumulate)), _ptr(bias), _ptr(scratch), 0 if scratch is None else scratch.numel(), _stream()),
           "s2vt_gemm_bf16x3_tn")
+    return out
+
+
+def gemm_bf16x3_nn(Ah, Al, Bh, Bl, N=None, K=None, out=None, accumulate=False, split_k=True, bias=None):
+    for t in (Ah, Al, Bh, Bl):
+        assert t.is_cuda and t.dtype == torch.bfloat16 and t.stride(1) == 1
+    assert Ah.shape == Al.shape and Bh.shape == Bl.shape and Ah.stride(0) == Al.stride(0) and Bh.stride(0) == Bl.stride(0)
+    M = Ah.shape[0]
+    K = Bh.shape[0] if K is None else int(K)
+    N = Bh.shape[1] if N is None else int(N)
+    if out is None:
+        assert not accumulate
+        out = torch.empty((M, N), dtype=torch.float32, device=Ah.device)
+    _chk_f32(out, bias)
+    assert out.shape[0] == M and out.shape[1] == N and out.stride(1) == 1
+    scratch = workspace(32 * M * N, Ah.device, "gemm_bf16x3") if split_k and M * N else None
+    check(lib().s2vt_gemm_bf16x3_nn(_ptr(Ah), _ptr(Al), Ah.stride(0), _ptr(Bh), _ptr(Bl), Bh.stride(0), _ptr(out), out.stride(0), M, N, K,
+                                    int(bool(accumulate)), _ptr(bias), _ptr(scratch), 0 if scratch is None else scratch.numel(), _stream()),
+          "s2vt_gemm_bf16x3_nn")
     return out
 
 
```
